# enricobottazzi/zk-fhe

Hardware: AMD Instinct MI355X
Metric: BFV proofs/sec (k=13) (higher is better)
Workload: dtype u32x8 (256-bit Montgomery integers over BN254 Fr/Fq)

## Files before the change

### zk-fhe_amd/csrc/core.hip

```cpp
#include <atomic>
#include <cstdio>
#include <cstdlib>
#include <cstring>

#include <map>
#include <mutex>
#include <utility>

#include "ctx.hpp"
#include "fq29.hip.hpp"
#include "fr29.hip.hpp"
#include "fr9.hip.hpp"

using namespace zk;

static thread_local std::string g_create_err;

int zk_fail(zkfhe_ctx *ctx, int code, const char *what, hipError_t e, const char *file, int line) {
  char buf[512];
  snprintf(buf, sizeof(buf), "%s failed: %s (%s:%d)", what, hipGetErrorString(e), file, line);
  if (ctx) ctx->err = buf; else g_create_err = buf;
  return code;
}
int zk_fail_msg(zkfhe_ctx *ctx, int code, const std::string &msg) {
  if (ctx) ctx->err = msg; else g_create_err = msg;
  return code;
}

int zk_func_max_lds(zkfhe_ctx *ctx, const void *kernel, int bytes) {
  static std::mutex mu;
  static std::map<std::pair<int, const void *>, int> done;
  std::lock_guard<std::mutex> l(mu);
  int &have = done[std::make_pair(ctx->device, kernel)];
  if (have >= bytes) return ZKFHE_OK;
  ZK_HIP(ctx, hipFuncSetAttribute(kernel, hipFuncAttributeMaxDynamicSharedMemorySize, bytes));
  have = bytes;
  return ZKFHE_OK;
}

int zk_scratch(zkfhe_ctx *ctx, int slot, size_t bytes, void **out) {
  if (ctx->scratch_sz[slot] < bytes) {
    if (ctx->scratch[slot]) {
      ZK_HIP(ctx, hipStreamSynchronize(ctx->stream));
      ZK_HIP(ctx, hipFree(ctx->scratch[slot]));
      ctx->scratch[slot] = nullptr;
      ctx->scratch_sz[slot] = 0;
    }
    size_t want = bytes + bytes / 4;
    ZK_HIP(ctx, hipMalloc(&ctx->scratch[slot], want));
    ctx->scratch_sz[slot] = want;
  }
  *out = ctx->scratch[slot];
  return ZKFHE_OK;
}

Fr zk_fr_from_u64(uint64_t v) {
  Fr t = Fr::zero();
  t.l[0] = (u32)v;
  t.l[1] = (u32)(v >> 32);
  return fp_to_mont<FrP>(t);
}

Fr zk_fr_root_of_unity(int log_n) {
  Fr c;
  const u32 w[8] = {0x60c37c9cu, 0xd34f1ed9u, 0xd39329c8u, 0x3215cf6du, 0x3dd31f74u, 0x98865ea9u, 0x166d18b7u, 0x03ddb9f5u};
  for (int i = 0; i < 8; ++i) c.l[i] = w[i];
  Fr r = fp_to_mont<FrP>(c);
  for (int i = 0; i < 28 - log_n; ++i) r = fp_sqr<FrP>(r);
  return r;
}

__global__ void __launch_bounds__(256) k_copy16(const uint4 *__restrict__ src, uint4 *__restrict__ dst, size_t n16) {
  for (size_t i = blockIdx.x * (size_t)blockDim.x + threadIdx.x; i < n16; i += (size_t)gridDim.x * blockDim.x) dst[i] = src[i];
}
int zk_copy_d2d(zkfhe_ctx *ctx, void *dst, const void *src, size_t bytes) {
  if (!bytes) return ZKFHE_OK;
  if (bytes >= ((size_t)1 << 20) && (bytes & 15) == 0 && ((uintptr_t)dst & 15) == 0 && ((uintptr_t)src & 15) == 0) {
    const size_t n16 = bytes / 16;
    size_t blocks = (n16 + 255) / 256;
    const size_t cap = (size_t)ctx->num_cu * 32;
    k_copy16<<<(unsigned)(blocks > cap ? cap : blocks), 256, 0, ctx->stream>>>((const uint4 *)src, (uint4 *)dst, n16);
    ZK_LAUNCH_CHECK(ctx);
    return ZKFHE_OK;
  }
  ZK_HIP(ctx, zk_memcpy_async(ctx, dst, src, bytes, hipMemcpyDeviceToDevice, ctx->stream));
  return ZKFHE_OK;
}

extern "C" {

const char *zkfhe_version(void) { return "zkfhe-mi355x 0.1 (gfx950)"; }

int zkfhe_ctx_create(int device_id, void *hip_stream, zkfhe_ctx **out) {
  setenv("GPU_MAX_HW_QUEUES", "2", 0);
  if (!getenv("ZKFHE_SPIN_WAIT")) {
    (void)hipSetDevice(device_id);
    (void)hipSetDeviceFlags(hipDeviceScheduleBlockingSync);
    (void)hipGetLastError();
  }
  if (!out) return zk_fail_msg(nullptr, ZKFHE_EINVAL, "out is NULL");
  *out = nullptr;
  int count = 0;
  hipError_t e = hipGetDeviceCount(&count);
  if (e != hipSuccess || count == 0)
    return zk_fail_msg(nullptr, ZKFHE_ENODEV, std::string("no HIP device: ") + hipGetErrorString(e));
  if (device_id < 0 || device_id >= count) return zk_fail_msg(nullptr, ZKFHE_EINVAL, "device_id out of range");
  hipDeviceProp_t prop;
  ZK_HIP(nullptr, hipGetDeviceProperties(&prop, device_id));
  if (strncmp(prop.gcnArchName, "gfx950", 6) != 0)
    return zk_fail_msg(nullptr, ZKFHE_ENODEV, std::string("device is ") + prop.gcnArchName + ", this library is built for gfx950 only");
  ZK_HIP(nullptr, hipSetDevice(device_id));
  zkfhe_ctx *ctx = new zkfhe_ctx();
  static std::atomic<uint64_t> next_uid{1};
  ctx->uid = next_uid.fetch_add(1);
  ctx->device = device_id;
  ctx->num_cu = prop.multiProcessorCount;
  if (hip_stream) {
    ctx->stream = (hipStream_t)hip_stream;
  } else {
    e = hipStreamCreateWithFlags(&ctx->stream, hipStreamNonBlocking);
    if (e != hipSuccess) { delete ctx; return zk_fail(nullptr, ZKFHE_EHIP, "hipStreamCreate", e, __FILE__, __LINE__); }
    ctx->own_stream = true;
  }
  if (hipHostMalloc(&ctx->bounce, zkfhe_ctx::BOUNCE_BYTES, hipHostMallocDefault) != hipSuccess) ctx->bounce = nullptr;
  if (hipEventCreateWithFlags(&ctx->wait_ev, hipEventBlockingSync | hipEventDisableTiming) != hipSuccess) ctx->wait_ev = nullptr;
  hipEventCreate(&ctx->ev0);
  hipEventCreate(&ctx->ev1);
  hipEventCreate(&ctx->pe0);
  hipEventCreate(&ctx->pe1);
  *out = ctx;
  return ZKFHE_OK;
}

int zkfhe_ctx_destroy(zkfhe_ctx *ctx) {
  ZK_ENTER(ctx);
  if (!ctx) return ZKFHE_OK;
  hipSetDevice(ctx->device);
  hipStreamSynchronize(ctx->stream);
  if (ctx->bounce) (void)hipHostFree(ctx->bounce);
  for (auto &kv : ctx->domains) {
    hipFree(kv.second.fwd);
    hipFree(kv.second.inv);
    hipFree(kv.second.fwd29);
    hipFree(kv.second.inv29);
    hipFree(kv.second.n_inv29_dev);
  }
  for (auto &kv : ctx->tw13) hipFree(kv.second);
  for (auto &kv : ctx->pre13) hipFree(kv.second);
  for (auto &kv : ctx->dif8) hipFree(kv.second);
  for (int i = 0; i < 4; ++i)
    if (ctx->scratch[i]) hipFree(ctx->scratch[i]);
  if (ctx->tickets) hipFree(ctx->tickets);
  if (ctx->bfv_tw) hipFree(ctx->bfv_tw);
  if (ctx->bfv_work) hipFree(ctx->bfv_work);
  for (auto &kv : ctx->slot_tw) hipFree(kv.second.dev);
  if (ctx->wait_ev) hipEventDestroy(ctx->wait_ev);
  hipEventDestroy(ctx->ev0);
  hipEventDestroy(ctx->ev1);
  if (ctx->own_stream) hipStreamDestroy(ctx->stream);
  delete ctx;
  return ZKFHE_OK;
}

const char *zkfhe_last_error(const zkfhe_ctx *ctx) { return ctx ? ctx->err.c_str() : g_create_err.c_str(); }

int zkfhe_sync(zkfhe_ctx *ctx) {
  ZK_ENTER(ctx);
  ZK_HIP(ctx, zk_wait(ctx));
  return ZKFHE_OK;
}

void *zkfhe_stream(zkfhe_ctx *ctx) { return (void *)ctx->stream; }

int zkfhe_device_info(zkfhe_ctx *ctx, char *arch_name, size_t arch_len, int *num_cu, size_t *hbm_bytes) {
  ZK_ENTER(ctx);
  hipDeviceProp_t prop;
  ZK_HIP(ctx, hipGetDeviceProperties(&prop, ctx->device));
  if (arch_name && arch_len) { strncpy(arch_name, prop.gcnArchName, arch_len - 1); arch_name[arch_len - 1] = 0; }
  if (num_cu) *num_cu = prop.multiProcessorCount;
  if (hbm_bytes) *hbm_bytes = prop.totalGlobalMem;
  return ZKFHE_OK;
}

int zkfhe_dev_alloc(zkfhe_ctx *ctx, size_t bytes, void **dptr) {
  ZK_ENTER(ctx);
  ZK_ARG(ctx, dptr != nullptr);
  ZK_HIP(ctx, hipSetDevice(ctx->device));
  hipError_t e = hipMalloc(dptr, bytes ? bytes : 1);
  if (e == hipErrorOutOfMemory) return zk_fail_msg(ctx, ZKFHE_ENOMEM, "hipMalloc: out of device memory");
  ZK_HIP(ctx, e);
  return ZKFHE_OK;
}
int zkfhe_dev_free(zkfhe_ctx *ctx, void *dptr) {
  ZK_ENTER(ctx);
  if (!dptr) return ZKFHE_OK;
  if (!ctx) {
    (void)hipFree(dptr);
    return ZKFHE_OK;
  }
  ZK_HIP(ctx, hipStreamSynchronize(ctx->stream));
  ZK_HIP(ctx, hipFree(dptr));
  return ZKFHE_OK;
}
int zkfhe_upload(zkfhe_ctx *ctx, void *dst_dev, const void *src_host, size_t bytes) {
  ZK_ENTER(ctx);
  if (!bytes) return ZKFHE_OK;
  if (ctx->bounce && bytes <= zkfhe_ctx::BOUNCE_BYTES) {
    memcpy(ctx->bounce, src_host, bytes);
    ZK_HIP(ctx, zk_memcpy_async(ctx, dst_dev, ctx->bounce, bytes, hipMemcpyHostToDevice, ctx->stream));
  } else {
    ZK_HIP(ctx, zk_memcpy_async(ctx, dst_dev, src_host, bytes, hipMemcpyHostToDevice, ctx->stream));
  }
  ZK_HIP(ctx, zk_wait(ctx));
  return ZKFHE_OK;
}
int zkfhe_download(zkfhe_ctx *ctx, void *dst_host, const void *src_dev, size_t bytes) {
  ZK_ENTER(ctx);
  if (!bytes) return ZKFHE_OK;
  if (ctx->bounce && bytes <= zkfhe_ctx::BOUNCE_BYTES) {
    ZK_HIP(ctx, zk_memcpy_async(ctx, ctx->bounce, src_dev, bytes, hipMemcpyDeviceToHost, ctx->stream));
    ZK_HIP(ctx, zk_wait(ctx));
    memcpy(dst_host, ctx->bounce, bytes);
    return ZKFHE_OK;
  }
  ZK_HIP(ctx, zk_memcpy_async(ctx, dst_host, src_dev, bytes, hipMemcpyDeviceToHost, ctx->stream));
  ZK_HIP(ctx, zk_wait(ctx));
  return ZKFHE_OK;
}
int zkfhe_copy_dev(zkfhe_ctx *ctx, void *dst_dev, const void *src_dev, size_t bytes) {
  ZK_ENTER(ctx);
  return zk_copy_d2d(ctx, dst_dev, src_dev, bytes);
}
int zkfhe_memset_dev(zkfhe_ctx *ctx, void *dst_dev, int byte, size_t bytes) {
  ZK_ENTER(ctx);
  ZK_HIP(ctx, zk_memset_async(ctx, dst_dev, byte, bytes, ctx->stream));
  return ZKFHE_OK;
}

int zkfhe_prof_enable(zkfhe_ctx *ctx, int on) {
  ZK_ENTER(ctx);
  ctx->prof_on = on != 0;
  return ZKFHE_OK;
}
int zkfhe_prof_reset(zkfhe_ctx *ctx) {
  ZK_ENTER(ctx);
  for (int i = 0; i < zkfhe_ctx::PROF_SLOTS; ++i) {
    ctx->prof_ms[i] = ctx->prof_bytes[i] = ctx->prof_ops[i] = 0;
    ctx->prof_launches[i] = 0;
  }
  return ZKFHE_OK;
}
int zkfhe_prof_read(zkfhe_ctx *ctx, int which, double *total_ms, uint64_t *launches, double *algorithmic_bytes) {
  ZK_ENTER(ctx);
  ZK_ARG(ctx, which >= 0 && which < zkfhe_ctx::PROF_SLOTS);
  if (total_ms) *total_ms = ctx->prof_ms[which];
  if (launches) *launches = ctx->prof_launches[which];
  if (algorithmic_bytes) *algorithmic_bytes = ctx->prof_bytes[which];
  return ZKFHE_OK;
}

int zkfhe_prof_read_ops(zkfhe_ctx *ctx, int which, double *ops) {
  ZK_ENTER(ctx);
  ZK_ARG(ctx, which >= 0 && which < zkfhe_ctx::PROF_SLOTS && ops != nullptr);
  *ops = ctx->prof_ops[which];
  return ZKFHE_OK;
}

int zkfhe_ctx_last_proof_marks(zkfhe_ctx *ctx, float marks_ms[3]) {
  ZK_ENTER(ctx);
  ZK_ARG(ctx, marks_ms != nullptr);
  for (int i = 0; i < 3; ++i) marks_ms[i] = ctx->proof_marks[i];
  return ZKFHE_OK;
}

int zkfhe_ctx_last_proof_commands(zkfhe_ctx *ctx, uint64_t counts[3]) {
  ZK_ENTER(ctx);
  ZK_ARG(ctx, counts != nullptr);
  for (int i = 0; i < 3; ++i) counts[i] = ctx->cmd_count[i];
  return ZKFHE_OK;
}

int zkfhe_timer_start(zkfhe_ctx *ctx) {
  ZK_ENTER(ctx);
  ZK_HIP(ctx, hipEventRecord(ctx->ev0, ctx->stream));
  return ZKFHE_OK;
}
int zkfhe_timer_stop_ms(zkfhe_ctx *ctx, float *ms) {
  ZK_ENTER(ctx);
  ZK_HIP(ctx, hipEventRecord(ctx->ev1, ctx->stream));
  ZK_HIP(ctx, hipEventSynchronize(ctx->ev1));
  ZK_HIP(ctx, hipEventElapsedTime(ms, ctx->ev0, ctx->ev1));
  return ZKFHE_OK;
}

}

enum { OP_ADD = 0, OP_SUB = 1, OP_MUL = 2 };

template <int OP>
__global__ void __launch_bounds__(256) k_fr_binop(const Fr *__restrict__ a, const Fr *__restrict__ b, Fr *__restrict__ out, size_t n) {
  for (size_t i = blockIdx.x * (size_t)blockDim.x + threadIdx.x; i < n; i += (size_t)gridDim.x * blockDim.x) {
    Fr x = a[i], y = b[i];
    Fr r = OP == OP_ADD ? x + y : OP == OP_SUB ? x - y : x * y;
    out[i] = r;
  }
}

template <int MODE>
__global__ void __launch_bounds__(256) k_fr_unop(const Fr *__restrict__ a, Fr s, Fr *__restrict__ out, size_t n) {
  for (size_t i = blockIdx.x * (size_t)blockDim.x + threadIdx.x; i < n; i += (size_t)gridDim.x * blockDim.x) {
    Fr x = a[i];
    out[i] = MODE == 0 ? x * s : MODE == 1 ? fr29_to_mont(x) : fp_from_mont<FrP>(x);
  }
}

__global__ void __launch_bounds__(256) k_fr_sqr_chain(const Fr *__restrict__ a, Fr *__restrict__ out, size_t n, int iters) {
  size_t i = blockIdx.x * (size_t)blockDim.x + threadIdx.x;
  if (i >= n) return;
  Fr x = a[i];
  for (int k = 0; k < iters; ++k) x = fp_sqr<FrP>(x);
  out[i] = x;
}

__global__ void __launch_bounds__(256) k_fq29_sqr_chain(const Fq *__restrict__ a, Fq *__restrict__ out, size_t n, int iters) {
  size_t i = blockIdx.x * (size_t)blockDim.x + threadIdx.x;
  if (i >= n) return;
  F29 x = f29_unpack(a[i]);
  for (int k = 0; k < iters; ++k) x = f29_sqr(x);
  out[i] = f29_pack(f29_canonical(x));
}

enum { FR9_MUL = 0, FR9_SQR = 1, FR9_MUL2 = 2, FR9_PERM = 3, FR9_LOOKUP = 4, FR9_CHAIN = 5, FR9_OPS = 6 };
__global__ void __launch_bounds__(256) k_fr9_op(int op, const Fr *__restrict__ in, Fr *__restrict__ out, size_t n) {
  for (size_t i = blockIdx.x * (size_t)blockDim.x + threadIdx.x; i < n; i += (size_t)gridDim.x * blockDim.x) {
    const Fr a = in[i], b = in[n + i], c = in[2 * n + i], d = in[3 * n + i], e = in[4 * n + i];
    Fr r;
    switch (op) {
      case FR9_MUL: r = fr9_store(fr9_mul(fr9_load(a), fr9_load32(b))); break;
      case FR9_SQR: r = fr9_store(fr9_cc(fr9_sqr(fr9_load(a)))); break;
      case FR9_MUL2: r = fr9_store(fr9_mul2(fr9_load(a), fr9_load32(b), fr9_load32(c), fr9_load(d))); break;
      case FR9_PERM: r = fr9_store(fr9_perm_step(fr9_load(a), fr9_perm_factor(fr9_load32(b), fr9_mul(fr9_load(d), fr9_cc(fr9_load32(c))), fr9_load32(e)))); break;
      case FR9_CHAIN: r = fr9_store(fr9_mul(fr9_load(c), fr9_times32(fr9_mul(fr9_load(a), fr9_load32(b))))); break;
      default: r = fr9_store(fr9_lookup_term(fr9_load(a), fr9_load(b), fr9_lookup_sum(fr9_load32(c), fr9_load32(d)))); break;
    }
    out[i] = r;
  }
}

#define BI_CHUNK 8
#define BI_LONG ((size_t)1 << 20)
template <bool NUM>
__global__ void __launch_bounds__(256) k_fr_batch_invert(Fr *__restrict__ a, Fr *__restrict__ num, Fr *__restrict__ tmp, size_t n, size_t T) {
  size_t t = blockIdx.x * (size_t)blockDim.x + threadIdx.x;
  if (t >= T) return;
  Lz<0, 1, 2> acc = lz_widen<0, 1, 2>(fr9_one());
  int cnt = 0;
  for (size_t i = t; i < n; i += T, ++cnt) {
    tmp[i] = fr9_store(acc);
    Fr x = a[i];
    if (!x.is_zero()) acc = fr9_mul(acc, fr9_load32(x));
  }
  acc = lz_widen<0, 1, 2>(fr9_load(fp_inv<FrP>(fr9_store(acc))));
  for (int k = cnt - 1; k >= 0; --k) {
    size_t i = t + (size_t)k * T;
    Fr x = a[i];
    if (x.is_zero()) {
      if (NUM) num[i] = Fr::zero();
      continue;
    }
    const Lz<0, 1, 2> inv = fr9_mul(acc, fr9_load32(tmp[i]));
    acc = fr9_mul(acc, fr9_load32(x));
    if (NUM) num[i] = fr9_store(fr9_mul(inv, fr9_load32(num[i])));
    else a[i] = fr9_store(inv);
  }
}

static unsigned ew_grid(zkfhe_ctx *ctx, size_t n) {
  size_t b = (n + 255) / 256;
  size_t cap = (size_t)ctx->num_cu * 8;
  return (unsigned)(b < 1 ? 1 : (b > cap ? cap : b));
}

extern "C" {

int zkfhe_fr_add(zkfhe_ctx *ctx, const zkfhe_fr *a, const zkfhe_fr *b, zkfhe_fr *out, size_t n) {
  ZK_ENTER(ctx);
  if (!n) return ZKFHE_OK;
  k_fr_binop<OP_ADD><<<ew_grid(ctx, n), 256, 0, ctx->stream>>>((const Fr *)a, (const Fr *)b, (Fr *)out, n);
  ZK_LAUNCH_CHECK(ctx);
  return ZKFHE_OK;
}
int zkfhe_fr_sub(zkfhe_ctx *ctx, const zkfhe_fr *a, const zkfhe_fr *b, zkfhe_fr *out, size_t n) {
  ZK_ENTER(ctx);
  if (!n) return ZKFHE_OK;
  k_fr_binop<OP_SUB><<<ew_grid(ctx, n), 256, 0, ctx->stream>>>((const Fr *)a, (const Fr *)b, (Fr *)out, n);
  ZK_LAUNCH_CHECK(ctx);
  return ZKFHE_OK;
}
int zkfhe_fr_mul(zkfhe_ctx *ctx, const zkfhe_fr *a, const zkfhe_fr *b, zkfhe_fr *out, size_t n) {
  ZK_ENTER(ctx);
  if (!n) return ZKFHE_OK;
  k_fr_binop<OP_MUL><<<ew_grid(ctx, n), 256, 0, ctx->stream>>>((const Fr *)a, (const Fr *)b, (Fr *)out, n);
  ZK_LAUNCH_CHECK(ctx);
  return ZKFHE_OK;
}
int zkfhe_fr_scale(zkfhe_ctx *ctx, const zkfhe_fr *a, const zkfhe_fr *s_host, zkfhe_fr *out, size_t n) {
  ZK_ENTER(ctx);
  if (!n) return ZKFHE_OK;
  ZK_ARG(ctx, s_host != nullptr);
  Fr s;
  memcpy(&s, s_host, 32);
  k_fr_unop<0><<<ew_grid(ctx, n), 256, 0, ctx->stream>>>((const Fr *)a, s, (Fr *)out, n);
  ZK_LAUNCH_CHECK(ctx);
  return ZKFHE_OK;
}
int zkfhe_fr_to_mont(zkfhe_ctx *ctx, const zkfhe_fr *a, zkfhe_fr *out, size_t n) {
  ZK_ENTER(ctx);
  if (!n) return ZKFHE_OK;
  k_fr_unop<1><<<ew_grid(ctx, n), 256, 0, ctx->stream>>>((const Fr *)a, Fr::zero(), (Fr *)out, n);
  ZK_LAUNCH_CHECK(ctx);
  return ZKFHE_OK;
}
int zkfhe_fr_from_mont(zkfhe_ctx *ctx, const zkfhe_fr *a, zkfhe_fr *out, size_t n) {
  ZK_ENTER(ctx);
  if (!n) return ZKFHE_OK;
  k_fr_unop<2><<<ew_grid(ctx, n), 256, 0, ctx->stream>>>((const Fr *)a, Fr::zero(), (Fr *)out, n);
  ZK_LAUNCH_CHECK(ctx);
  return ZKFHE_OK;
}
static int batch_invert(zkfhe_ctx *ctx, Fr *a, Fr *num, size_t n) {
  if (!n) return ZKFHE_OK;
  void *tmp;
  int rc = zk_scratch(ctx, 0, n * sizeof(Fr), &tmp);
  if (rc) return rc;
  static const int forced = getenv("ZKFHE_BI_CHUNK") ? atoi(getenv("ZKFHE_BI_CHUNK")) : 0;
  size_t chunk = forced > 0 ? (size_t)forced : n / ((size_t)ctx->num_cu * 1024);
  if (forced <= 0) chunk = chunk < BI_CHUNK ? BI_CHUNK : (chunk > 32 ? 32 : chunk);
  if (forced <= 0 && n >= BI_LONG && chunk < 16) chunk = 16;
  size_t T = (n + chunk - 1) / chunk;
  if (num)
    k_fr_batch_invert<true><<<zk_blocks(T, 256), 256, 0, ctx->stream>>>(a, num, (Fr *)tmp, n, T);
  else
    k_fr_batch_invert<false><<<zk_blocks(T, 256), 256, 0, ctx->stream>>>(a, nullptr, (Fr *)tmp, n, T);
  ZK_LAUNCH_CHECK(ctx);
  return ZKFHE_OK;
}
int zkfhe_fr_batch_invert(zkfhe_ctx *ctx, zkfhe_fr *a, size_t n) {
  ZK_ENTER(ctx);
  return batch_invert(ctx, (Fr *)a, nullptr, n);
}
int zkfhe_fr_batch_invert_mul(zkfhe_ctx *ctx, const zkfhe_fr *den, zkfhe_fr *num, size_t n) {
  ZK_ENTER(ctx);
  ZK_ARG(ctx, n == 0 || (den != nullptr && num != nullptr && (const void *)den != (const void *)num));
  return batch_invert(ctx, (Fr *)den, (Fr *)num, n);
}
int zkfhe_fr9_op(zkfhe_ctx *ctx, int op, const zkfhe_fr *in, zkfhe_fr *out, size_t n) {
  ZK_ENTER(ctx);
  ZK_ARG(ctx, op >= 0 && op < FR9_OPS);
  if (!n) return ZKFHE_OK;
  ZK_ARG(ctx, in != nullptr && out != nullptr);
  k_fr9_op<<<ew_grid(ctx, n), 256, 0, ctx->stream>>>(op, (const Fr *)in, (Fr *)out, n);
  ZK_LAUNCH_CHECK(ctx);
  return ZKFHE_OK;
}
int zkfhe_fr_sqr_chain(zkfhe_ctx *ctx, const zkfhe_fr *a, zkfhe_fr *out, size_t n, int iters) {
  ZK_ENTER(ctx);
  if (!n) return ZKFHE_OK;
  k_fr_sqr_chain<<<zk_blocks(n, 256), 256, 0, ctx->stream>>>((const Fr *)a, (Fr *)out, n, iters);
  ZK_LAUNCH_CHECK(ctx);
  return ZKFHE_OK;
}

int zkfhe_fq29_sqr_chain(zkfhe_ctx *ctx, const zkfhe_fq *a, zkfhe_fq *out, size_t n, int iters) {
  ZK_ENTER(ctx);
  if (!n) return ZKFHE_OK;
  k_fq29_sqr_chain<<<zk_blocks(n, 256), 256, 0, ctx->stream>>>((const Fq *)a, (Fq *)out, n, iters);
  ZK_LAUNCH_CHECK(ctx);
  return ZKFHE_OK;
}

}
```

### zk-fhe_amd/csrc/ctx.hpp

```cpp
#pragma once
#include <hip/hip_runtime.h>

#include <array>
#include <map>
#include <string>
#include <vector>

#include "../../include/zkfhe.h"
#include "bn254.hip.hpp"

struct NttDomain {
  int log_n = 0;
  zk::Fr *fwd = nullptr;
  zk::Fr *inv = nullptr;
  zk::Fr n_inv;
  zk::Fr omega, omega_inv;
  zk::Fr *fwd29 = nullptr, *inv29 = nullptr;
  zk::Fr n_inv29;
  zk::Fr *n_inv29_dev = nullptr;
};

struct zkfhe_ctx {
  uint64_t uid = 0;
  int device = 0;
  hipStream_t stream = nullptr;
  bool own_stream = false;
  hipEvent_t ev0 = nullptr, ev1 = nullptr;
  std::string err;
  int num_cu = 0;
  std::map<int, NttDomain> domains;
  std::map<const void *, void *> tw13;
  std::map<std::array<uint64_t, 6>, void *> pre13;
  std::map<std::array<uint64_t, 8>, void *> dif8;
  bool prof_on = false;
  hipEvent_t pe0 = nullptr, pe1 = nullptr;
  hipEvent_t wait_ev = nullptr;
  static constexpr int PROF_SLOTS = 26;
  double prof_ms[PROF_SLOTS] = {}, prof_bytes[PROF_SLOTS] = {}, prof_ops[PROF_SLOTS] = {};
  uint64_t prof_launches[PROF_SLOTS] = {};
  void *bounce = nullptr;
  static constexpr size_t BOUNCE_BYTES = (size_t)1 << 20;
  void *scratch[4] = {nullptr, nullptr, nullptr, nullptr};
  size_t scratch_sz[4] = {0, 0, 0, 0};
  float proof_marks[3] = {0, 0, 0};
  uint64_t cmd_count[3] = {0, 0, 0};
  zkfhe_ctx *cmd_owner = nullptr;
  unsigned *tickets = nullptr;
  uint32_t *bfv_tw = nullptr;
  void *bfv_work = nullptr;
  size_t bfv_work_sz = 0;
  struct SlotTables {
    uint32_t *dev = nullptr;
    uint32_t pinv = 0, n_inv = 0;
  };
  std::map<std::pair<uint64_t, uint64_t>, SlotTables> slot_tw;
};

struct zkfhe_basis {
  size_t n = 0;
  int c = 0;
  int windows = 0;
  zk::G1Affine *table = nullptr;
  zk::G1Affine *mult = nullptr;
  int mc = 0, mw = 0;
  size_t mult_bytes = 0;
  bool narrowed = false;
};

int zk_fail(zkfhe_ctx *ctx, int code, const char *what, hipError_t e, const char *file, int line);
int zk_fail_msg(zkfhe_ctx *ctx, int code, const std::string &msg);

#define ZK_HIP(ctx, expr)                                                             \
  do {                                                                                \
    hipError_t _e = (expr);                                                           \
    if (_e != hipSuccess) return zk_fail((ctx), ZKFHE_EHIP, #expr, _e, __FILE__, __LINE__); \
  } while (0)

enum { ZK_CMD_KERNEL = 0, ZK_CMD_COPY = 1, ZK_CMD_FILL = 2 };
static inline void zk_count(zkfhe_ctx *ctx, int which) { ++(ctx->cmd_owner ? ctx->cmd_owner : ctx)->cmd_count[which]; }

#define ZK_LAUNCH_CHECK(ctx)         \
  do {                               \
    zk_count((ctx), ZK_CMD_KERNEL);  \
    ZK_HIP(ctx, hipGetLastError());  \
  } while (0)

static inline hipError_t zk_memcpy_async(zkfhe_ctx *ctx, void *dst, const void *src, size_t bytes, hipMemcpyKind kind, hipStream_t stream) {
  zk_count(ctx, ZK_CMD_COPY);
  return hipMemcpyAsync(dst, src, bytes, kind, stream);
}
static inline hipError_t zk_memset_async(zkfhe_ctx *ctx, void *dst, int value, size_t bytes, hipStream_t stream) {
  zk_count(ctx, ZK_CMD_FILL);
  return hipMemsetAsync(dst, value, bytes, stream);
}

#define ZK_ENTER(ctx)                                   \
  do {                                                  \
    if (ctx) (void)hipSetDevice((ctx)->device);         \
  } while (0)

#define ZK_ARG(ctx, cond)                                                        \
  do {                                                                           \
    if (!(cond)) return zk_fail_msg((ctx), ZKFHE_EINVAL, std::string("bad argument: ") + #cond); \
  } while (0)

inline void zk_prof_begin(zkfhe_ctx *ctx) {
  if (ctx->prof_on) (void)hipEventRecord(ctx->pe0, ctx->stream);
}
inline void zk_prof_end(zkfhe_ctx *ctx, int which, double bytes) {
  if (!ctx->prof_on) return;
  (void)hipEventRecord(ctx->pe1, ctx->stream);
  (void)hipEventSynchronize(ctx->pe1);
  float ms = 0;
  (void)hipEventElapsedTime(&ms, ctx->pe0, ctx->pe1);
  ctx->prof_ms[which] += ms;
  ctx->prof_bytes[which] += bytes;
  ctx->prof_launches[which] += 1;
}

inline hipError_t zk_wait(zkfhe_ctx *ctx) {
  static const bool spin = getenv("ZKFHE_SPIN_WAIT") != nullptr;
  if (spin || !ctx->wait_ev) return hipStreamSynchronize(ctx->stream);
  hipError_t e = hipEventRecord(ctx->wait_ev, ctx->stream);
  if (e != hipSuccess) return e;
  return hipEventSynchronize(ctx->wait_ev);
}

int zk_dif8_pass(zkfhe_ctx *ctx, const zk::Fr *src, zk::Fr *dst, size_t n_cols, int log_n, int S, int inverse, const zk::Fr *shifts_host, unsigned rows);
int zk_msm_batch_strided(zkfhe_ctx *ctx, const zkfhe_basis *basis, const zkfhe_fr *scalars_dev, size_t col_stride, size_t n_cols, zkfhe_g1_affine *out_dev);
int zk_msm_batch_strided_form(zkfhe_ctx *ctx, const zkfhe_basis *basis, const zkfhe_fr *scalars_dev, size_t col_stride, size_t n_cols, void *out_dev, bool xyzz);
#define ZK_CK(x)             \
  do {                       \
    const int rc__ = (x);    \
    if (rc__) return rc__;   \
  } while (0)

int zk_func_max_lds(zkfhe_ctx *ctx, const void *kernel, int bytes);
int zk_scratch(zkfhe_ctx *ctx, int slot, size_t bytes, void **out);
int zk_basis_create_scaled(zkfhe_ctx *ctx, const zkfhe_g1_affine *bases_host, size_t n, int window_bits, double table_budget_scale, zkfhe_basis **out);
int zk_copy_d2d(zkfhe_ctx *ctx, void *dst, const void *src, size_t bytes);
int zk_domain(zkfhe_ctx *ctx, int log_n, const NttDomain **out);
int zk_pre13(zkfhe_ctx *ctx, const zk::Fr &g, int lef, int rows, bool scaled, const void **out);
int zk_coset_ntt_rows(zkfhe_ctx *ctx, const zk::Fr *in_dev, zk::Fr *out_dev, size_t n_cols, int log_n, int lef, const zk::Fr &g, int rows);
int zk_extend_lagrange(zkfhe_ctx *ctx, const zk::Fr *lagr_dev, zk::Fr *tmp_dev, zk::Fr *out_dev, size_t n_cols, int log_n, int lef, const zk::Fr &g, int rows);

zk::Fr zk_fr_from_u64(uint64_t v);
zk::Fr zk_fr_root_of_unity(int log_n);

static inline unsigned zk_blocks(size_t n, unsigned threads) { return (unsigned)((n + threads - 1) / threads); }
```

### zk-fhe_amd/host/keygen.hip

```cpp
#include "prover_internal.hpp"

std::vector<BigInt> GpuPolyMul::mul_u64(const std::vector<uint64_t> &a, const std::vector<uint64_t> &b) {
  const U256 *host = mul_u64_raw(a, b);
  std::vector<BigInt> out(2 * a.size() - 1);
  for (size_t i = 0; i < out.size(); ++i) out[i] = fe::to_bigint(host[i]);
  return out;
}

const U256 *GpuPolyMul::mul_u64_raw(const std::vector<uint64_t> &a, const std::vector<uint64_t> &b) {
  const size_t n = a.size();
  if (ws->polyio.bytes < 2 * n * 8 + 2 * n * 32) throw std::runtime_error("polynomial too long for the prover workspace");
  uint64_t *da = (uint64_t *)ws->polyio.p, *db = da + n;
  Fr *dout = (Fr *)(db + n);
  const U256 *host = ws->host_poly;
  int rc = up(ctx, ws, da, a.data(), n * 8);
  if (!rc) rc = up(ctx, ws, db, b.data(), n * 8);
  if (!rc) rc = zkfhe_witness_poly_mul_u64(ctx, da, db, n, (zkfhe_fr *)dout);
  if (!rc) rc = zkfhe_fr_from_mont(ctx, (const zkfhe_fr *)dout, (zkfhe_fr *)dout, 2 * n - 1);
  if (!rc && ws->host_poly && 2 * n - 1 <= ws->host_poly_len) {
    if (zk_memcpy_async(ctx, ws->host_poly, dout, (2 * n - 1) * 32, hipMemcpyDeviceToHost, ctx->stream) != hipSuccess) rc = ZKFHE_EHIP;
    if (!rc) rc = zkfhe_sync(ctx);
  } else if (!rc) {
    pageable.resize(2 * n - 1);
    host = pageable.data();
    rc = zkfhe_download(ctx, pageable.data(), dout, (2 * n - 1) * 32);
  }
  if (rc) throw std::runtime_error(std::string("GPU poly mul failed: ") + zkfhe_last_error(ctx));
  return host;
}

int up(zkfhe_ctx *ctx, Workspace *ws, void *dst, const void *src, size_t bytes) {
  if (!bytes) return ZKFHE_OK;
  const size_t need = (bytes + 63) & ~(size_t)63;
  if (!ws->ring || ws->ring_off + need > Workspace::RING_BYTES) return zkfhe_upload(ctx, dst, src, bytes);
  uint8_t *slot = ws->ring + ws->ring_off;
  ws->ring_off += need;
  memcpy(slot, src, bytes);
  ZK_HIP(ctx, zk_memcpy_async(ctx, dst, slot, bytes, hipMemcpyHostToDevice, ctx->stream));
  return ZKFHE_OK;
}

int alloc_workspace(zkfhe_ctx *ctx, const CircuitConfig &c, Workspace *ws, int ext_rows) {
  const size_t n = c.n(), ne = (size_t)ext_rows * n, col = n * 32, ecol = ne * 32;
  const size_t n_all = (size_t)c.n_advice() + 3 * c.n_lookup + c.n_chunks() + 1;
  ws->n_all = n_all;
  CK(ws->all_l.alloc(ctx, n_all * col));
  CK(ws->all_ext.alloc(ctx, n_all * ecol));
  {
    size_t o = 0;
    auto take = [&](View &l, View &e, size_t cols) {
      l.p = (char *)ws->all_l.p + o * col;
      e.p = (char *)ws->all_ext.p + o * ecol;
      o += cols;
    };
    take(ws->adv_l, ws->adv_ext, c.n_advice());
    take(ws->la_l, ws->la_ext, c.n_lookup);
    take(ws->ls_l, ws->ls_ext, c.n_lookup);
    take(ws->pz_l, ws->pz_ext, c.n_chunks());
    take(ws->lz_l, ws->lz_ext, c.n_lookup);
    take(ws->inst_l, ws->inst_ext, 1);
  }
  ZK_HIP(ctx, zk_memset_async(ctx, ws->inst_l.p, 0, col, ctx->stream));
  ws->inst_count = 0;
  CK(ws->tmp_c.alloc(ctx, std::max<size_t>(n_all, c.n_perm()) * col));
  {
    const size_t groups = ((size_t)c.n_gate() + 7) / 8 + 1 + 2 + ((size_t)c.n_chunks() + 31) / 32 + ((size_t)c.n_chunks() + 3) / 4 + ((size_t)c.n_lookup + 2) / 3 + 8;
    CK(ws->partials.alloc(ctx, std::max<size_t>(groups * (size_t)ext_rows, 96) * col));
  }
  CK(ws->h_ext.alloc(ctx, 4 * col));
  CK(ws->h_c.alloc(ctx, 4 * col));
  CK(ws->misc.alloc(ctx, 32 * col));
  CK(ws->points.alloc(ctx, std::max<size_t>(n_all, c.n_perm()) * 64 + 64));
  CK(ws->num.alloc(ctx, std::max<size_t>(c.n_chunks(), c.n_lookup) * col));
  CK(ws->den.alloc(ctx, std::max<size_t>(c.n_chunks(), c.n_lookup) * col));
  if ((size_t)c.n_perm() > 4096 || (size_t)c.n_chunks() + c.n_lookup > 4096)
    return zk_fail_msg(ctx, ZKFHE_EINVAL, "configuration too wide for the prover workspace (more than 4096 permutation columns)");
  CK(ws->small.alloc(ctx, 1 << 20));
  const size_t max_items = (size_t)c.n_advice() + c.n_fixed() + 2 + c.n_perm() + c.n_chunks() + 3 * c.n_lookup;
  CK(ws->jobs.alloc(ctx, max_items * sizeof(zkp::EvalJob) + max_items * (sizeof(void *) + 32) + 256));
  CK(ws->evout.alloc(ctx, (max_items + 64) * 4 * 32));
  CK(ws->polyio.alloc(ctx, 4 * c.n() * 32));
  ZK_HIP(ctx, hipHostMalloc((void **)&ws->host_adv, (size_t)c.n_advice() * col, hipHostMallocDefault));
  memset(ws->host_adv, 0, (size_t)c.n_advice() * col);
  ZK_HIP(ctx, hipHostMalloc((void **)&ws->host_blind, std::max<size_t>(2 * c.n_lookup, 2) * col, hipHostMallocDefault));
  return ZKFHE_OK;
}

void free_workspace(Workspace *ws) {
  (void)hipSetDevice(ws->all_l.device);
  for (DevBuf *b : ws->all()) b->release();
  for (void *h : {(void *)ws->host_adv, (void *)ws->host_blind, (void *)ws->host_pool, (void *)ws->host_poly, (void *)ws->host_pts, (void *)ws->ring, (void *)ws->host_rand_pt,
                  (void *)ws->host_early, (void *)ws->host_early_err, (void *)ws->host_out})
    if (h) (void)hipHostFree(h);
  if (ws->ev_pts) (void)hipEventDestroy(ws->ev_pts);
  if (ws->ev_rand) (void)hipEventDestroy(ws->ev_rand);
  if (ws->ev_early) (void)hipEventDestroy(ws->ev_early);
  if (ws->aux) (void)zkfhe_ctx_destroy(ws->aux);
  delete ws;
}

int get_workspace(zkfhe_ctx *ctx, zkfhe_bfv_pk *pk, Workspace **out) {
  std::lock_guard<std::mutex> lock(pk->mu);
  auto it = pk->workspaces.find(ctx->uid);
  if (it == pk->workspaces.end()) {
    Workspace *ws = new Workspace();
    int rc = alloc_workspace(ctx, pk->cfg, ws, pk->ext_rows);
    if (rc) {
      for (DevBuf *b : ws->all()) b->release();
      delete ws;
      return rc;
    }
    it = pk->workspaces.emplace(ctx->uid, ws).first;
  }
  if (it->second->all_l.device != ctx->device) return zk_fail_msg(ctx, ZKFHE_EINVAL, "prover workspace belongs to another device");
  *out = it->second;
  return ZKFHE_OK;
}

int extend_cols(zkfhe_ctx *ctx, zkfhe_bfv_pk *pk, Workspace *ws, const Fr *lagr, size_t count, Fr *ext) {
  if (!count) return ZKFHE_OK;
  const int rows = pk->ext_rows;
  const size_t n = pk->cfg.n();
  const Fr g = mont_u64(COSET_G);
  (void)n;
  return zk_extend_lagrange(ctx, lagr, ws->tmp_c.fr(), ext, count, (int)pk->cfg.k, 2, g, rows);
}

static int build_resident_tables(zkfhe_ctx *ctx, zkfhe_bfv_pk *pk, Workspace *ws) {
  const CircuitConfig &cfg = pk->cfg;
  const size_t n = cfg.n(), cells = (size_t)cfg.n_perm() * n;
  const NttDomain *dom;
  CK(zk_domain(ctx, (int)cfg.k, &dom));
  const size_t R = (size_t)pk->ext_rows;
  CK(pk->fixed_ext.alloc(ctx, (size_t)cfg.n_fixed() * R * n * 32));
  CK(pk->sigma_ext.alloc(ctx, cells * R * 32));
  CK(pk->l_ext.alloc(ctx, 3 * R * n * 32));
  CK(pk->xs_ext.alloc(ctx, R * n * 32));
  CK(extend_cols(ctx, pk, ws, pk->fixed_l.fr(), cfg.n_fixed(), pk->fixed_ext.fr()));
  CK(extend_cols(ctx, pk, ws, pk->sigma_l.fr(), cfg.n_perm(), pk->sigma_ext.fr()));
  {
    std::vector<U256> l(3 * n, fe::zero());
    const size_t u = cfg.u();
    l[0] = fe::one();
    l[n + u] = fe::one();
    for (size_t i = 0; i < u; ++i) l[2 * n + i] = fe::one();
    CK(upload_canon(ctx, ws->misc.fr(), l.data(), 3 * n));
    CK(extend_cols(ctx, pk, ws, ws->misc.fr(), 3, pk->l_ext.fr()));
  }
  {
    const Fr wext = zk_fr_root_of_unity((int)cfg.k + 2);
    Fr shift = mont_u64(COSET_G);
    for (int k1 = 0; k1 < pk->ext_rows; ++k1) {
      zkp::k_powers<<<(unsigned)((n + 255) / 256), 256, 0, ctx->stream>>>(shift, dom->omega, pk->xs_ext.fr() + (size_t)k1 * n, n);
      ZK_LAUNCH_CHECK(ctx);
      shift = shift * wext;
    }
    if (pk->ext_rows == 3) {
      CK(pk->ext3_pw.alloc(ctx, 3 * n * 32));
      Fr gk = mont_u64(COSET_G);
      for (int t = 0; t < 3; ++t) {
        zkp::k_powers<<<(unsigned)((n + 255) / 256), 256, 0, ctx->stream>>>(Fr::one(), fr_inv(gk), pk->ext3_pw.fr() + (size_t)t * n, n);
        ZK_LAUNCH_CHECK(ctx);
        gk = gk * wext;
      }
    }
  }
  return ZKFHE_OK;
}

static U256 vk_digest_of(const zkfhe_bfv_pk *pk) { return vk_digest(pk->cfg, pk->fixed_commit, pk->sigma_commit); }

static int keygen_impl(zkfhe_ctx *ctx, const zkfhe_srs *srs, const char *input_json, const BfvParams &prm, CircuitConfig cfg, bool replay,
                zkfhe_bfv_pk **out) {
  const size_t n = cfg.n();
  ZK_ARG(ctx, srs->k == cfg.k);
  const CircuitInput in = CircuitInput::parse_json(input_json);
  Context ctx0(CTX_PHASE0, false, true), ctx_gate(CTX_GATE1, false, true), ctx_rlc(CTX_RLC1, true, true);
  std::vector<Cell> make_public;
  BfvState st = bfv_phase0(ctx0, in, prm, make_public);
  bfv_phase1(st, prm, ctx_gate, ctx_rlc, fe::zero());
  Assigner as(cfg, true);
  as.place(ctx0, replay);
  as.place(ctx_gate, replay);
  as.place(ctx_rlc, replay);
  as.place_lookups(ctx_gate);
  as.finish_structure(ctx0, ctx_gate, ctx_rlc, make_public);
  cfg.bp_gate0 = as.t.bp_gate0;
  cfg.bp_gate1 = as.t.bp_gate1;
  cfg.bp_rlc = as.t.bp_rlc;
  zkfhe_bfv_pk *pk = new zkfhe_bfv_pk();
  pk->cfg = cfg;
  pk->prm = prm;
  pk->ext_rows = getenv("ZKFHE_CHECK_QUOTIENT") ? 4 : 3;
  {
    pk->gate1_cells = ctx_gate.advice.size();
    pk->n_lookup_cells = ctx_gate.lookup.size();
    pk->n_inv_slots = ctx_gate.inv_slots.size();
    std::vector<uint32_t> lsrc(ctx_gate.lookup.size());
    for (size_t i = 0; i < lsrc.size(); ++i) {
      ZK_ASSERT(ctx_gate.lookup[i].ctx == CTX_GATE1, "lookup cell outside the phase-1 gate context");
      lsrc[i] = ctx_gate.lookup[i].off;
    }
    std::vector<uint32_t> start(cfg.n_gate1, 0), len(cfg.n_gate1, 0);
    size_t s = 0;
    for (unsigned c = 0; c < cfg.n_gate1 && s < pk->gate1_cells; ++c) {
      start[c] = (uint32_t)s;
      if (c < cfg.bp_gate1.size()) {
        len[c] = cfg.bp_gate1[c] + 1;
        s += cfg.bp_gate1[c];
      } else {
        len[c] = (uint32_t)(pk->gate1_cells - s);
        s = pk->gate1_cells;
      }
    }
    CK(pk->lookup_src.alloc(ctx, (lsrc.size() + 1) * 4));
    CK(pk->inv_slots.alloc(ctx, (ctx_gate.inv_slots.size() + 1) * 4));
    CK(pk->place_start.alloc(ctx, (start.size() + 1) * 4));
    CK(pk->place_len.alloc(ctx, (len.size() + 1) * 4));
    if (!lsrc.empty()) CK(zkfhe_upload(ctx, pk->lookup_src.p, lsrc.data(), lsrc.size() * 4));
    if (!ctx_gate.inv_slots.empty()) CK(zkfhe_upload(ctx, pk->inv_slots.p, ctx_gate.inv_slots.data(), ctx_gate.inv_slots.size() * 4));
    CK(zkfhe_upload(ctx, pk->place_start.p, start.data(), start.size() * 4));
    CK(zkfhe_upload(ctx, pk->place_len.p, len.data(), len.size() * 4));
  }
  const size_t cells = (size_t)cfg.n_perm() * n;
  std::vector<uint32_t> parent(cells);
  for (size_t i = 0; i < cells; ++i) parent[i] = (uint32_t)i;
  auto find = [&](uint32_t x) {
    uint32_t root = x;
    while (parent[root] != root) root = parent[root];
    while (parent[x] != root) {
      uint32_t nx = parent[x];
      parent[x] = root;
      x = nx;
    }
    return root;
  };
  for (const auto &cp : as.t.copies) {
    uint32_t ra = find((uint32_t)cp.first), rb = find((uint32_t)cp.second);
    if (ra != rb) {
      if (ra < rb) parent[rb] = ra;
      else parent[ra] = rb;
    }
  }
  std::vector<uint32_t> target(cells), last_of(cells, 0xffffffffu), first_of(cells);
  for (size_t i = 0; i < cells; ++i) target[i] = (uint32_t)i;
  for (size_t i = 0; i < cells; ++i) {
    const uint32_t r = find((uint32_t)i);
    if (last_of[r] == 0xffffffffu) first_of[r] = (uint32_t)i;
    else target[last_of[r]] = (uint32_t)i;
    last_of[r] = (uint32_t)i;
  }
  for (size_t i = 0; i < cells; ++i)
    if (parent[i] == i && last_of[i] != 0xffffffffu) target[last_of[i]] = first_of[i];
  const NttDomain *dom;
  CK(zk_domain(ctx, (int)cfg.k, &dom));
  CK(pk->fixed_l.alloc(ctx, (size_t)cfg.n_fixed() * n * 32));
  CK(pk->sigma_l.alloc(ctx, cells * 32));
  CK(pk->dpow.alloc(ctx, (size_t)cfg.n_perm() * 32));
  for (unsigned c = 0; c < cfg.n_fixed(); ++c) {
    ZK_HIP(ctx, zk_memcpy_async(ctx, pk->fixed_l.fr() + (size_t)c * n, as.t.fixed[c].data(), n * 32, hipMemcpyHostToDevice, ctx->stream));
  }
  CK(zkfhe_fr_to_mont(ctx, (const zkfhe_fr *)pk->fixed_l.p, (zkfhe_fr *)pk->fixed_l.p, (size_t)cfg.n_fixed() * n));
  U256 dcan;
  memcpy(dcan.l, DELTA_CANON, 32);
  zkp::k_powers<<<1, 256, 0, ctx->stream>>>(Fr::one(), mont(dcan), pk->dpow.fr(), cfg.n_perm());
  ZK_LAUNCH_CHECK(ctx);
  DevBuf tgt;
  CK(tgt.alloc(ctx, cells * 4));
  CK(zkfhe_upload(ctx, tgt.p, target.data(), cells * 4));
  zkp::k_sigma_values<<<(unsigned)((cells + 255) / 256), 256, 0, ctx->stream>>>((const uint32_t *)tgt.p, pk->dpow.fr(), dom->fwd, pk->sigma_l.fr(),
                                                                                 cells, (int)cfg.k);
  ZK_LAUNCH_CHECK(ctx);
  Workspace *ws;
  CK(get_workspace(ctx, pk, &ws));
  CK(commit_cols(ctx, srs, srs->g_lagrange, pk->fixed_l.fr(), cfg.n_fixed(), (G1Affine *)ws->points.p, pk->fixed_commit));
  CK(commit_cols(ctx, srs, srs->g_lagrange, pk->sigma_l.fr(), cfg.n_perm(), (G1Affine *)ws->points.p, pk->sigma_commit));
  CK(build_resident_tables(ctx, pk, ws));
  CK(zkfhe_sync(ctx));
  tgt.release();
  pk->vk_digest = vk_digest_of(pk);
  *out = pk;
  return ZKFHE_OK;
}


extern "C" {

int zkfhe_bfv_keygen(zkfhe_ctx *ctx, const zkfhe_srs *srs, const char *input_json, const zkfhe_bfv_params *params,
                     const zkfhe_bfv_config *config, zkfhe_bfv_pk **out) {
  ZK_ENTER(ctx);
  ZK_ARG(ctx, srs && input_json && params && config && out);
  try {
    return keygen_impl(ctx, srs, input_json, params_from_c(params), config_from_c(config), config->replay != 0, out);
  } catch (const std::exception &e) {
    return zk_fail_msg(ctx, ZKFHE_EINVAL, e.what());
  }
}

int zkfhe_bfv_pk_destroy(zkfhe_ctx *ctx, zkfhe_bfv_pk *pk) {
  ZK_ENTER(ctx);
  if (!pk) return ZKFHE_OK;
  zkfhe_sync(ctx);
  DevBuf *bufs[] = {&pk->fixed_l, &pk->sigma_l, &pk->fixed_ext, &pk->sigma_ext, &pk->l_ext, &pk->xs_ext, &pk->dpow, &pk->ext3_pw,
                    &pk->lookup_src, &pk->inv_slots, &pk->place_start, &pk->place_len};
  for (DevBuf *b : bufs) b->release();
  for (auto &kv : pk->workspaces) free_workspace(kv.second);
  delete pk;
  return ZKFHE_OK;
}

int zkfhe_bfv_pk_release_ctx(zkfhe_ctx *ctx, zkfhe_bfv_pk *pk) {
  ZK_ENTER(ctx);
  ZK_ARG(ctx, pk != nullptr);
  zkfhe_sync(ctx);
  std::lock_guard<std::mutex> lock(pk->mu);
  auto it = pk->workspaces.find(ctx->uid);
  if (it != pk->workspaces.end()) {
    free_workspace(it->second);
    pk->workspaces.erase(it);
  }
  return ZKFHE_OK;
}

namespace {
struct FileW {
  FILE *f;
  bool ok = true;
  void raw(const void *p, size_t n) { ok = ok && fwrite(p, 1, n, f) == n; }
  void u32(uint32_t v) { raw(&v, 4); }
  void u64(uint64_t v) { raw(&v, 8); }
  void vec32(const std::vector<uint32_t> &v) {
    u64(v.size());
    if (!v.empty()) raw(v.data(), v.size() * 4);
  }
};
struct FileR {
  FILE *f;
  bool ok = true;
  void raw(void *p, size_t n) { ok = ok && fread(p, 1, n, f) == n; }
  uint32_t u32() {
    uint32_t v = 0;
    raw(&v, 4);
    return v;
  }
  uint64_t u64() {
    uint64_t v = 0;
    raw(&v, 8);
    return v;
  }
  std::vector<uint32_t> vec32(size_t limit) {
    const uint64_t n = u64();
    std::vector<uint32_t> v;
    if (!ok || n > limit) {
      ok = false;
      return v;
    }
    v.resize(n);
    if (n) raw(v.data(), n * 4);
    return v;
  }
};
int download_u32(zkfhe_ctx *ctx, const DevBuf &b, size_t count, std::vector<uint32_t> &out) {
  out.resize(count);
  if (count) CK(zkfhe_download(ctx, out.data(), b.p, count * 4));
  return ZKFHE_OK;
}
int upload_u32(zkfhe_ctx *ctx, DevBuf &b, const std::vector<uint32_t> &v) {
  CK(b.alloc(ctx, (v.size() + 1) * 4));
  if (!v.empty()) CK(zkfhe_upload(ctx, b.p, v.data(), v.size() * 4));
  return ZKFHE_OK;
}
}

int zkfhe_bfv_pk_save(zkfhe_ctx *ctx, const zkfhe_bfv_pk *pk, const char *path) {
  ZK_ENTER(ctx);
  ZK_ARG(ctx, pk != nullptr && path != nullptr);
  const CircuitConfig &cfg = pk->cfg;
  const size_t n = cfg.n();
  std::vector<uint32_t> lookup_src, inv_slots, place_start, place_len;
  CK(download_u32(ctx, pk->lookup_src, pk->n_lookup_cells, lookup_src));
  CK(download_u32(ctx, pk->inv_slots, pk->n_inv_slots, inv_slots));
  CK(download_u32(ctx, pk->place_start, cfg.n_gate1, place_start));
  CK(download_u32(ctx, pk->place_len, cfg.n_gate1, place_len));
  std::vector<uint8_t> cols((size_t)(cfg.n_fixed() + cfg.n_perm()) * n * 32);
  CK(zkfhe_download(ctx, cols.data(), pk->fixed_l.p, (size_t)cfg.n_fixed() * n * 32));
  CK(zkfhe_download(ctx, cols.data() + (size_t)cfg.n_fixed() * n * 32, pk->sigma_l.p, (size_t)cfg.n_perm() * n * 32));
  FILE *f = fopen(path, "wb");
  if (!f) return zk_fail_msg(ctx, ZKFHE_EINVAL, std::string("cannot write ") + path);
  FileW w{f};
  w.raw("ZKFHEPK2", 8);
  const uint32_t hdr[8] = {cfg.k, cfg.n_gate0, cfg.n_gate1, cfg.n_lookup, cfg.n_rlc, cfg.unusable_rows, cfg.lookup_bits, cfg.transcript};
  w.raw(hdr, sizeof(hdr));
  w.vec32(cfg.bp_gate0), w.vec32(cfg.bp_gate1), w.vec32(cfg.bp_rlc);
  w.u64(pk->prm.N), w.u64(pk->prm.Q), w.u64(pk->prm.T), w.u64(pk->prm.B);
  w.u64(pk->gate1_cells);
  w.vec32(lookup_src), w.vec32(inv_slots), w.vec32(place_start), w.vec32(place_len);
  w.u64(pk->fixed_commit.size()), w.u64(pk->sigma_commit.size());
  for (const auto &pt : pk->fixed_commit) w.raw(&pt, sizeof(AffinePoint));
  for (const auto &pt : pk->sigma_commit) w.raw(&pt, sizeof(AffinePoint));
  w.raw(pk->vk_digest.l, 32);
  w.u64(cols.size());
  w.raw(cols.data(), cols.size());
  const bool ok = w.ok && fclose(f) == 0;
  if (!ok) return zk_fail_msg(ctx, ZKFHE_EINVAL, std::string("short write to ") + path);
  return ZKFHE_OK;
}

int zkfhe_bfv_pk_load(zkfhe_ctx *ctx, const zkfhe_srs *srs, const char *path, zkfhe_bfv_pk **out) {
  ZK_ENTER(ctx);
  ZK_ARG(ctx, srs != nullptr && path != nullptr && out != nullptr);
  FILE *f = fopen(path, "rb");
  if (!f) return zk_fail_msg(ctx, ZKFHE_EINVAL, std::string("cannot read ") + path);
  FileR r{f};
  char magic[8];
  r.raw(magic, 8);
  if (!r.ok || memcmp(magic, "ZKFHEPK2", 8) != 0) {
    fclose(f);
    return zk_fail_msg(ctx, ZKFHE_EINVAL, std::string(path) + " is not a ZKFHEPK2 proving key");
  }
  zkfhe_bfv_pk *pk = new zkfhe_bfv_pk();
  pk->ext_rows = getenv("ZKFHE_CHECK_QUOTIENT") ? 4 : 3;
  auto fail = [&](const std::string &why) {
    fclose(f);
    zkfhe_bfv_pk_destroy(ctx, pk);
    return zk_fail_msg(ctx, ZKFHE_EINVAL, std::string(path) + ": " + why);
  };
  try {
    uint32_t hdr[8];
    r.raw(hdr, sizeof(hdr));
    CircuitConfig &cfg = pk->cfg;
    cfg.k = hdr[0], cfg.n_gate0 = hdr[1], cfg.n_gate1 = hdr[2], cfg.n_lookup = hdr[3], cfg.n_rlc = hdr[4], cfg.unusable_rows = hdr[5], cfg.lookup_bits = hdr[6];
    cfg.transcript = hdr[7];
    if (!r.ok || cfg.transcript > TR_BLAKE2B || cfg.k < 3 || cfg.k > 20 || cfg.n_gate0 + cfg.n_gate1 > 4096 || cfg.n_lookup > 4096 || cfg.n_rlc > 4096) return fail("bad header");
    if (cfg.n_gate() == 0 || cfg.unusable_rows < 4 || cfg.unusable_rows >= cfg.n()) return fail("bad header (unusable_rows)");
    if (cfg.lookup_bits == 0 || cfg.lookup_bits > 20 || ((size_t)1 << cfg.lookup_bits) > cfg.max_rows()) return fail("bad header (lookup_bits)");
    if (cfg.k != srs->k) return fail("proving key and SRS have different k");
    cfg.bp_gate0 = r.vec32(1 << 16), cfg.bp_gate1 = r.vec32(1 << 16), cfg.bp_rlc = r.vec32(1 << 16);
    pk->prm.N = r.u64(), pk->prm.Q = r.u64(), pk->prm.T = r.u64(), pk->prm.B = r.u64();
    pk->gate1_cells = r.u64();
    if (!r.ok || pk->prm.N < 2 || (pk->prm.N & (pk->prm.N - 1)) || 5 * (uint64_t)pk->prm.N + 1 > cfg.u() || pk->prm.Q < 2 ||
        pk->prm.Q >= ((uint64_t)1 << 63) || pk->prm.T < 1 || pk->prm.T >= pk->prm.Q || pk->prm.B >= pk->prm.Q)
      return fail("BFV parameters do not fit the recorded layout");
    const size_t n = cfg.n(), max_cells = (size_t)cfg.n_gate1 * n;
    const std::vector<uint32_t> lookup_src = r.vec32(max_cells), inv_slots = r.vec32(max_cells), place_start = r.vec32(cfg.n_gate1), place_len = r.vec32(cfg.n_gate1);
    if (!r.ok || pk->gate1_cells > max_cells || place_start.size() != cfg.n_gate1 || place_len.size() != cfg.n_gate1) return fail("bad structure lists");
    for (uint32_t o : lookup_src)
      if (o >= pk->gate1_cells) return fail("lookup offset outside the gate stream");
    for (uint32_t o : inv_slots)
      if (o >= pk->gate1_cells) return fail("inverse slot outside the gate stream");
    for (unsigned c = 0; c < cfg.n_gate1; ++c)
      if ((size_t)place_start[c] + place_len[c] > pk->gate1_cells || place_len[c] > n) return fail("column range outside the gate stream");
    pk->n_lookup_cells = lookup_src.size();
    pk->n_inv_slots = inv_slots.size();
    const uint64_t nf = r.u64(), ns = r.u64();
    if (!r.ok || nf != cfg.n_fixed() || ns != cfg.n_perm()) return fail("commitment counts do not match the configuration");
    pk->fixed_commit.resize(nf), pk->sigma_commit.resize(ns);
    for (auto &pt : pk->fixed_commit) r.raw(&pt, sizeof(AffinePoint));
    for (auto &pt : pk->sigma_commit) r.raw(&pt, sizeof(AffinePoint));
    r.raw(pk->vk_digest.l, 32);
    const uint64_t col_bytes = r.u64();
    if (!r.ok || col_bytes != (uint64_t)(cfg.n_fixed() + cfg.n_perm()) * n * 32) return fail("column block has the wrong size");
    if (!(vk_digest_of(pk) == pk->vk_digest)) return fail("verifying-key digest does not match the stored commitments");
    std::vector<uint8_t> cols(col_bytes);
    r.raw(cols.data(), cols.size());
    if (!r.ok) return fail("truncated file");
    fclose(f);
    f = nullptr;
    int rc;
    if ((rc = upload_u32(ctx, pk->lookup_src, lookup_src)) || (rc = upload_u32(ctx, pk->inv_slots, inv_slots)) ||
        (rc = upload_u32(ctx, pk->place_start, place_start)) || (rc = upload_u32(ctx, pk->place_len, place_len)) ||
        (rc = pk->fixed_l.alloc(ctx, (size_t)cfg.n_fixed() * n * 32)) || (rc = pk->sigma_l.alloc(ctx, (size_t)cfg.n_perm() * n * 32)) ||
        (rc = pk->dpow.alloc(ctx, (size_t)cfg.n_perm() * 32)) ||
        (rc = zkfhe_upload(ctx, pk->fixed_l.p, cols.data(), (size_t)cfg.n_fixed() * n * 32)) ||
        (rc = zkfhe_upload(ctx, pk->sigma_l.p, cols.data() + (size_t)cfg.n_fixed() * n * 32, (size_t)cfg.n_perm() * n * 32))) {
      zkfhe_bfv_pk_destroy(ctx, pk);
      return rc;
    }
    U256 dcan;
    memcpy(dcan.l, DELTA_CANON, 32);
    zkp::k_powers<<<1, 256, 0, ctx->stream>>>(Fr::one(), mont(dcan), pk->dpow.fr(), cfg.n_perm());
    Workspace *ws;
    if ((rc = get_workspace(ctx, pk, &ws)) || (rc = build_resident_tables(ctx, pk, ws)) || (rc = zkfhe_sync(ctx))) {
      zkfhe_bfv_pk_destroy(ctx, pk);
      return rc;
    }
    std::vector<AffinePoint> chk_f, chk_s;
    if ((rc = commit_cols(ctx, srs, srs->g_lagrange, pk->fixed_l.fr() + (size_t)cfg.fix_table() * n, 1, (G1Affine *)ws->points.p, chk_f)) ||
        (rc = commit_cols(ctx, srs, srs->g_lagrange, pk->sigma_l.fr(), 1, (G1Affine *)ws->points.p, chk_s))) {
      zkfhe_bfv_pk_destroy(ctx, pk);
      return rc;
    }
    if (!(chk_f[0].x == pk->fixed_commit[cfg.fix_table()].x) || !(chk_f[0].y == pk->fixed_commit[cfg.fix_table()].y) ||
        !(chk_s[0].x == pk->sigma_commit[0].x) || !(chk_s[0].y == pk->sigma_commit[0].y)) {
      zkfhe_bfv_pk_destroy(ctx, pk);
      return zk_fail_msg(ctx, ZKFHE_EINVAL, std::string(path) + ": proving key was generated with a different SRS");
    }
  } catch (const std::exception &e) {
    if (f) fclose(f);
    zkfhe_bfv_pk_destroy(ctx, pk);
    return zk_fail_msg(ctx, ZKFHE_EINVAL, e.what());
  }
  *out = pk;
  return ZKFHE_OK;
}

int zkfhe_bfv_pk_info(const zkfhe_bfv_pk *pk, uint8_t vk_digest[32], uint32_t *n_fixed, uint32_t *n_sigma) {
  if (!pk) return ZKFHE_EINVAL;
  if (vk_digest) memcpy(vk_digest, pk->vk_digest.l, 32);
  if (n_fixed) *n_fixed = (uint32_t)pk->fixed_commit.size();
  if (n_sigma) *n_sigma = (uint32_t)pk->sigma_commit.size();
  return ZKFHE_OK;
}

int zkfhe_bfv_pk_prefix_cache(const zkfhe_bfv_pk *pk_c, int capacity, uint64_t *hits, uint64_t *misses, uint64_t *entries) {
  if (!pk_c) return ZKFHE_EINVAL;
  zkfhe_bfv_pk *pk = const_cast<zkfhe_bfv_pk *>(pk_c);
  if (capacity >= 0) pk->prefix.set_capacity((size_t)capacity);
  pk->prefix.stats(hits, misses, entries);
  return ZKFHE_OK;
}

int zkfhe_bfv_pk_commitments(const zkfhe_bfv_pk *pk, uint8_t *fixed_out, uint8_t *sigma_out) {
  if (!pk) return ZKFHE_EINVAL;
  for (size_t i = 0; i < pk->fixed_commit.size() && fixed_out; ++i) {
    memcpy(fixed_out + 64 * i, pk->fixed_commit[i].x.l, 32);
    memcpy(fixed_out + 64 * i + 32, pk->fixed_commit[i].y.l, 32);
  }
  for (size_t i = 0; i < pk->sigma_commit.size() && sigma_out; ++i) {
    memcpy(sigma_out + 64 * i, pk->sigma_commit[i].x.l, 32);
    memcpy(sigma_out + 64 * i + 32, pk->sigma_commit[i].y.l, 32);
  }
  return ZKFHE_OK;
}

int zkfhe_bfv_pk_export_vk(const zkfhe_bfv_pk *pk, uint8_t *out, size_t cap, size_t *len) {
  if (!pk || !len) return ZKFHE_EINVAL;
  const size_t nf = pk->fixed_commit.size(), ns = pk->sigma_commit.size();
  const size_t need = 8 + 40 + 32 + 64 * (nf + ns);
  *len = need;
  if (!out || cap < need) return out ? ZKFHE_EINVAL : ZKFHE_OK;
  memcpy(out, "ZKFHEVK2", 8);
  const uint32_t hdr[10] = {pk->cfg.k, pk->cfg.n_gate0, pk->cfg.n_gate1, pk->cfg.n_lookup, pk->cfg.n_rlc, pk->cfg.unusable_rows,
                            pk->cfg.lookup_bits, pk->cfg.transcript, (uint32_t)nf, (uint32_t)ns};
  memcpy(out + 8, hdr, 40);
  memcpy(out + 48, pk->vk_digest.l, 32);
  uint8_t *p = out + 80;
  for (const auto &c : pk->fixed_commit) {
    memcpy(p, c.x.l, 32);
    memcpy(p + 32, c.y.l, 32);
    p += 64;
  }
  for (const auto &c : pk->sigma_commit) {
    memcpy(p, c.x.l, 32);
    memcpy(p + 32, c.y.l, 32);
    p += 64;
  }
  return ZKFHE_OK;
}

int zkfhe_bfv_pk_break_points(const zkfhe_bfv_pk *pk, int which, uint32_t *out, uint32_t *count) {
  if (!pk || !count) return ZKFHE_EINVAL;
  const auto &v = which == 0 ? pk->cfg.bp_gate0 : which == 1 ? pk->cfg.bp_gate1 : pk->cfg.bp_rlc;
  if (out && *count >= v.size()) memcpy(out, v.data(), v.size() * 4);
  *count = (uint32_t)v.size();
  return ZKFHE_OK;
}

}
```

### zk-fhe_amd/host/prove.hip

```cpp
#include "prover_internal.hpp"

int alloc_witness_buffers(zkfhe_ctx *ctx, const zkfhe_bfv_pk *pk, Workspace *ws) {
  if (ws->stream.p) return ZKFHE_OK;
  const size_t N = pk->prm.N;
  CK(ws->stream.alloc(ctx, (pk->gate1_cells + 8) * 32));
  CK(ws->pool.alloc(ctx, 40 * (2 * N + 8) * 32));
  CK(ws->invtmp.alloc(ctx, (pk->n_inv_slots + 8) * 32));
  ZK_HIP(ctx, hipHostMalloc((void **)&ws->host_pool, 24 * (2 * N + 8) * 32, hipHostMallocDefault));
  ws->host_poly_len = 2 * N + 8;
  ZK_HIP(ctx, hipHostMalloc((void **)&ws->host_poly, ws->host_poly_len * 32, hipHostMallocDefault));
  CK(ws->wblind.alloc(ctx, 256));
  ZK_HIP(ctx, hipHostMalloc((void **)&ws->ring, Workspace::RING_BYTES, hipHostMallocDefault));
  CK(ws->dev_ring.alloc(ctx, Workspace::RING_BYTES));
  {
    const CircuitConfig &c = pk->cfg;
    const size_t max_items = (size_t)c.n_advice() + c.n_fixed() + 2 + c.n_perm() + c.n_chunks() + 3 * c.n_lookup;
    ws->out_pts_cap = std::max<size_t>(ws->n_all, c.n_perm()) + 16;
    ws->out_ev_off = ws->out_pts_cap * PT_SLOT;
    ws->out_ev_cap = max_items * 4;
    ws->out_flag_off = ws->out_ev_off + ws->out_ev_cap * 32;
    ZK_HIP(ctx, hipHostMalloc((void **)&ws->host_out, ws->out_flag_off + 256, hipHostMallocDefault));
    memset(ws->host_out, 0, ws->out_flag_off + 256);
  }
  ZK_HIP(ctx, hipHostMalloc((void **)&ws->host_pts, ((size_t)pk->cfg.n_gate0 + 1) * PT_SLOT, hipHostMallocDefault));
  ZK_HIP(ctx, hipEventCreateWithFlags(&ws->ev_pts, hipEventDisableTiming | hipEventBlockingSync));
  ZK_HIP(ctx, hipEventCreateWithFlags(&ws->ev_rand, hipEventDisableTiming | hipEventBlockingSync));
  ZK_HIP(ctx, hipEventCreateWithFlags(&ws->ev_early, hipEventDisableTiming | hipEventBlockingSync));
  ZK_HIP(ctx, hipHostMalloc((void **)&ws->host_early, ((size_t)pk->cfg.n_advice() + 2 * pk->cfg.n_lookup + 16) * PT_SLOT, hipHostMallocDefault));
  ZK_HIP(ctx, hipHostMalloc((void **)&ws->host_early_err, 64, hipHostMallocDefault));
  ZK_HIP(ctx, hipHostMalloc((void **)&ws->host_rand_pt, PT_SLOT, hipHostMallocDefault));
  if (zkfhe_ctx_create(ctx->device, nullptr, &ws->aux)) return zk_fail_msg(ctx, ZKFHE_EHIP, std::string("auxiliary context: ") + zkfhe_last_error(nullptr));
  return ZKFHE_OK;
}

namespace {

void permute_lookup(const std::vector<U256> &input, size_t u, unsigned table_size, std::vector<U256> &a_perm, std::vector<U256> &s_perm) {
  std::vector<size_t> cnt(table_size, 0);
  for (size_t i = 0; i < u; ++i) {
    const U256 &v = input[i];
    if (v.l[1] | v.l[2] | v.l[3] || v.l[0] >= table_size) throw std::runtime_error("lookup input not in table");
    ++cnt[v.l[0]];
  }
  std::vector<size_t> left(table_size, 1);
  left[0] = u - (table_size - 1);
  a_perm.assign(u, fe::zero());
  s_perm.assign(u, fe::zero());
  std::vector<size_t> holes;
  size_t pos = 0;
  for (unsigned v = 0; v < table_size; ++v)
    for (size_t k = 0; k < cnt[v]; ++k, ++pos) {
      a_perm[pos] = fe::from_u64(v);
      if (k == 0) {
        if (!left[v]) throw std::runtime_error("lookup input not in table");
        --left[v];
        s_perm[pos] = fe::from_u64(v);
      } else {
        holes.push_back(pos);
      }
    }
  size_t hi = 0;
  for (unsigned v = 0; v < table_size; ++v)
    for (size_t k = 0; k < left[v]; ++k) s_perm[holes[hi++]] = fe::from_u64(v);
}

struct DevPoly {
  Fr *d = nullptr;
  size_t len = 0;
  uint64_t bits = 0;
};

class GpuPhase1 {
 public:
  GpuPhase1(zkfhe_ctx *c, const zkfhe_bfv_pk *k, Workspace *w) : ctx(c), pk(k), ws(w) {}

  int launch(const BfvState &st) {
    const uint64_t Q = pk->prm.Q, T = pk->prm.T, B = pk->prm.B;
    stream = ws->stream.fr();
    pool_used = 0;
    off = 0;
    calls.clear();
    call_level.clear();
    produced.clear();
    h_used = 0;
    {
      const PolyChip *ins[14] = {&st.e0, &st.e1, &st.u, &st.m, &st.pk0_u, &st.quotient_0, &st.remainder_0, &st.quotient_0_times_cyclo, &st.expected_c0,
                                 &st.pk1_u, &st.quotient_1, &st.remainder_1, &st.quotient_1_times_cyclo, &st.expected_c1};
      size_t cells = 1 + 16;
      for (const PolyChip *pc : ins) cells += pc->assigned_coefficients.size();
      in_host = ws->host_pool;
      in_dev = ws->pool.fr();
      in_ring = false;
      void *h = nullptr;
      if (cells * 32 <= ((size_t)1 << 20)) {
        void *d = stage_reserve(ws, cells * 32, &h);
        if (d) {
          in_host = (U256 *)h;
          in_dev = (Fr *)d;
          in_ring = true;
        }
      }
    }
    DevPoly e0 = stage(st.e0), e1 = stage(st.e1), u = stage(st.u), m = stage(st.m);
    DevPoly pk0_u = stage(st.pk0_u), q0 = stage(st.quotient_0), r0 = stage(st.remainder_0), q0c = stage(st.quotient_0_times_cyclo), xc0 = stage(st.expected_c0);
    DevPoly pk1_u = stage(st.pk1_u), q1 = stage(st.quotient_1), r1 = stage(st.remainder_1), q1c = stage(st.quotient_1_times_cyclo), xc1 = stage(st.expected_c1);
    in_host[h_used] = st.delta.value;
    const Fr *delta = in_dev + h_used;
    const uint64_t delta_bits = st.delta.value.bits();
    ++h_used;
    mg_slot = h_used;
    n_mg = 0;
    h_used += 16;
    pool_used = h_used;
    if (!in_ring) ZK_HIP(ctx, zk_memcpy_async(ctx, ws->pool.p, ws->host_pool, mg_slot * 32, hipMemcpyHostToDevice, ctx->stream));

    CK(in_range(e0, B, Q));
    CK(in_range(e1, B, Q));
    CK(gadget(zkw::G_CHI_KEY, u, nullptr, nullptr, zkw::cpc_chi_key(), Q - 1, 0, Fr::zero()));
    CK(in_range(m, T / 2, Q));
    const int n_side = 2;
    for (int side = 0; side < n_side; ++side) {
      const DevPoly &pku = side ? pk1_u : pk0_u, &q = side ? q1 : q0, &r = side ? r1 : r0, &qc = side ? q1c : q0c;
      CK(mul_gate());
      DevPoly pku_r;
      CK(reduce_by_modulo(pku, Q, pku_r));
      CK(in_field(q, Q));
      CK(in_field(r, Q));
      CK(mul_gate());
      DevPoly sum, sum_mod;
      CK(add(qc, r, sum));
      CK(reduce_by_modulo(sum, Q, sum_mod));
      if (sum_mod.len < pku_r.len) return zk_fail_msg(ctx, ZKFHE_EINVAL, "degree <= self.degree (src/poly_chip.rs:375)");
      DevPoly trimmed{sum_mod.d + (sum_mod.len - pku_r.len), pku_r.len, sum_mod.bits};
      CK(equal(trimmed, pku_r));
      const size_t N = pk->prm.N;
      if (r.len < N) return zk_fail_msg(ctx, ZKFHE_EINVAL, "degree <= self.degree (src/poly_chip.rs:375)");
      DevPoly acc{r.d + (r.len - N), N, r.bits};
      if (side == 0) {
        DevPoly m_delta, t;
        CK(scalar_mul(m, delta, delta_bits, m_delta));
        CK(add(acc, m_delta, t));
        CK(add(t, e0, acc));
      } else {
        DevPoly t;
        CK(add(acc, e1, t));
        acc = t;
      }
      DevPoly c_red;
      CK(reduce_by_modulo(acc, Q, c_red));
      CK(equal(c_red, side ? xc1 : xc0));
    }
    if (off != pk->gate1_cells) return zk_fail_msg(ctx, ZKFHE_EINVAL, "GPU witness stream length differs from the keygen circuit shape");
    CK(launch_levels());
    if (pk->n_inv_slots) {
      const unsigned g = (unsigned)((pk->n_inv_slots + 255) / 256);
      zkw::k_gather<<<g, 256, 0, ctx->stream>>>(stream, (const unsigned *)pk->inv_slots.p, pk->n_inv_slots, ws->invtmp.fr());
      ZK_LAUNCH_CHECK(ctx);
      CK(zkfhe_fr_batch_invert(ctx, (zkfhe_fr *)ws->invtmp.p, pk->n_inv_slots));
      zkw::k_scatter<<<g, 256, 0, ctx->stream>>>(stream, (const unsigned *)pk->inv_slots.p, pk->n_inv_slots, ws->invtmp.fr());
      ZK_LAUNCH_CHECK(ctx);
    }
    return ZKFHE_OK;
  }

  int place_early(const zkp::RngRows &blind, unsigned zero_cols) {
    zkw::ZeroRuns z{};
    z.count = n_mg;
    for (unsigned i = 0; i < n_mg; ++i) z.at[i] = stream + mg_off[i];
    zkw::k_zero_runs<<<1, 64, 0, ctx->stream>>>(z);
    ZK_LAUNCH_CHECK(ctx);
    return place(blind, zero_cols);
  }
  struct PatchPlan {
    std::vector<unsigned> columns;
    struct Cell {
      unsigned col_slot, row, value;
    };
    std::vector<Cell> cells;
  };
  PatchPlan patch_plan() const {
    PatchPlan p;
    const CircuitConfig &cfg = pk->cfg;
    std::vector<size_t> start(cfg.n_gate1, 0), len(cfg.n_gate1, 0);
    size_t s = 0;
    for (unsigned c = 0; c < cfg.n_gate1 && s < pk->gate1_cells; ++c) {
      start[c] = s;
      if (c < cfg.bp_gate1.size()) {
        len[c] = (size_t)cfg.bp_gate1[c] + 1;
        s += cfg.bp_gate1[c];
      } else {
        len[c] = pk->gate1_cells - s;
        s = pk->gate1_cells;
      }
    }
    for (unsigned i = 0; i < n_mg; ++i)
      for (unsigned j = 0; j < 4; ++j) {
        const size_t o = mg_off[i] + j;
        for (unsigned c = 0; c < cfg.n_gate1; ++c)
          if (len[c] && o >= start[c] && o < start[c] + len[c]) {
            size_t slot = std::find(p.columns.begin(), p.columns.end(), c) - p.columns.begin();
            if (slot == p.columns.size()) p.columns.push_back(c);
            p.cells.push_back({(unsigned)slot, (unsigned)(o - start[c]), 4 * i + j});
          }
      }
    return p;
  }
  int patch(const U256 evals[12], const PatchPlan &plan, Fr *patch_cols, std::vector<zkfhe_sparse_term> *terms = nullptr) {
    const CircuitConfig &cfg = pk->cfg;
    const size_t n = cfg.n();
    Fr mg[16];
    for (int i = 0; i < 4; ++i) {
      mg[4 * i] = Fr::zero();
      for (int j = 0; j < 3; ++j) mg[4 * i + 1 + j] = mont(evals[3 * i + j]);
    }
    if (terms) {
      terms->clear();
      for (const auto &c : plan.cells) {
        if ((c.value & 3) == 0) continue;
        zkfhe_sparse_term t;
        memcpy(&t.scalar, &mg[c.value], 32);
        t.row = c.row;
        t.slot = c.col_slot;
        terms->push_back(t);
      }
    }
    if (plan.cells.size() > 64) return zk_fail_msg(ctx, ZKFHE_EINVAL, "too many challenge-dependent gate cells");
    zkw::PatchList list{};
    for (size_t t = 0; t < plan.cells.size(); ++t) {
      const auto &c = plan.cells[t];
      list.cells[t].dst_adv = ws->adv_l.fr() + ((size_t)cfg.n_gate0 + plan.columns[c.col_slot]) * n + c.row;
      list.cells[t].dst_patch = terms ? nullptr : patch_cols + (size_t)c.col_slot * n + c.row;
      list.cells[t].value = c.value;
    }
    memcpy(list.values, mg, sizeof(mg));
    if (!terms) ZK_HIP(ctx, zk_memset_async(ctx, patch_cols, 0, plan.columns.size() * n * 32, ctx->stream));
    zkw::k_patch_cells<<<1, 64, 0, ctx->stream>>>(list, (unsigned)plan.cells.size());
    ZK_LAUNCH_CHECK(ctx);
    return ZKFHE_OK;
  }

  int finish(const U256 evals[12], const zkp::RngRows &blind) {
    Fr mg[16];
    for (int i = 0; i < 4; ++i) {
      mg[4 * i] = Fr::zero();
      for (int j = 0; j < 3; ++j) mg[4 * i + 1 + j] = mont(evals[3 * i + j]);
    }
    zkw::PatchList list{};
    unsigned nc = 0;
    for (unsigned i = 0; i < n_mg; ++i)
      for (unsigned j = 0; j < 4; ++j) {
        list.cells[nc].dst_adv = stream + mg_off[i] + j;
        list.cells[nc].dst_patch = nullptr;
        list.cells[nc].value = 4 * i + j;
        ++nc;
      }
    memcpy(list.values, mg, sizeof(mg));
    if (nc) {
      zkw::k_patch_cells<<<1, 64, 0, ctx->stream>>>(list, nc);
      ZK_LAUNCH_CHECK(ctx);
    }
    return place(blind, 0);
  }

 private:
  int place(const zkp::RngRows &blind, unsigned zero_cols) {
    const CircuitConfig &cfg = pk->cfg;
    const size_t n = cfg.n();
    const unsigned u = (unsigned)cfg.u();
    const unsigned g_place = grid_for(ctx, (size_t)cfg.n_gate1 * n);
    zkw::k_place<<<g_place + zkp::rng_tail_grid(blind, (size_t)cfg.n_gate1 * (n - u), 256), 256, 0, ctx->stream>>>(
        stream, (const unsigned *)pk->place_start.p, (const unsigned *)pk->place_len.p, cfg.n_gate1, n, ws->adv_l.fr() + (size_t)cfg.n_gate0 * n, blind, u, g_place);
    ZK_LAUNCH_CHECK(ctx);
    if (cfg.n_lookup) {
      if (pk->n_lookup_cells > (size_t)cfg.n_lookup * cfg.max_rows()) return zk_fail_msg(ctx, ZKFHE_EINVAL, "lookup cells do not fit the configured lookup columns");
      zkp::RngRows blind_lk = blind;
      blind_lk.ctr0 += (unsigned long long)(cfg.adv_lookup0() - cfg.n_gate0) * blind.ctr_col_stride;
      const unsigned g_lk = grid_for(ctx, (size_t)(cfg.n_lookup + zero_cols) * n);
      zkw::k_place_lookups<<<g_lk + zkp::rng_tail_grid(blind_lk, (size_t)cfg.n_lookup * (n - u), 256), 256, 0, ctx->stream>>>(
          stream, (const unsigned *)pk->lookup_src.p, pk->n_lookup_cells, (unsigned)cfg.max_rows(), n, cfg.n_lookup, ws->adv_l.fr() + (size_t)cfg.adv_lookup0() * n, blind_lk, u,
          zero_cols, g_lk);
      ZK_LAUNCH_CHECK(ctx);
    } else if (zero_cols) {
      ZK_HIP(ctx, zk_memset_async(ctx, ws->adv_l.fr() + (size_t)cfg.adv_rlc0() * n, 0, (size_t)zero_cols * n * 32, ctx->stream));
    }
    return ZKFHE_OK;
  }

  zkfhe_ctx *ctx;
  const zkfhe_bfv_pk *pk;
  Workspace *ws;
  Fr *stream = nullptr;
  size_t off = 0, pool_used = 0, h_used = 0, mg_slot = 0, mg_off[4] = {0, 0, 0, 0};
  unsigned n_mg = 0;
  U256 *in_host = nullptr;
  Fr *in_dev = nullptr;
  bool in_ring = false;

  DevPoly stage(const PolyChip &p) {
    DevPoly d;
    d.len = p.assigned_coefficients.size();
    d.bits = p.max_num_bits;
    d.d = in_dev + h_used;
    for (size_t i = 0; i < d.len; ++i) in_host[h_used + i] = p.assigned_coefficients[i].value;
    h_used += d.len;
    return d;
  }
  Fr *take(size_t len) {
    Fr *p = ws->pool.fr() + pool_used;
    pool_used += len;
    return p;
  }
  int gadget(int type, const DevPoly &a, const Fr *b, Fr *out, size_t cpc, uint64_t p0, uint64_t p1, const Fr &bound) {
    if (pool_used * 32 > ws->pool.bytes || (off + a.len * cpc) > pk->gate1_cells)
      return zk_fail_msg(ctx, ZKFHE_EINVAL, "GPU witness stream exceeds the keygen circuit shape");
    zkw::GadgetArgs g;
    g.type = type;
    g.a = a.d;
    g.b = b;
    g.out = out;
    g.stream = stream;
    g.base = off;
    g.cpc = cpc;
    g.count = a.len;
    g.p0 = p0;
    g.p1 = p1;
    g.bound = bound;
    calls.push_back(g);
    call_level.push_back(level_of(a.d, a.len, b));
    if (out) produced.push_back({out, out + a.len, call_level.back()});
    off += a.len * cpc;
    return ZKFHE_OK;
  }
  struct Produced {
    const Fr *lo, *hi;
    int level;
  };
  std::vector<zkw::GadgetArgs> calls;
  std::vector<int> call_level;
  std::vector<Produced> produced;
  int level_of(const Fr *a, size_t len, const Fr *b) const {
    int lv = 0;
    for (const Produced &p : produced) {
      if (a < p.hi && a + len > p.lo) lv = std::max(lv, p.level + 1);
      if (b && b < p.hi && b + 1 > p.lo) lv = std::max(lv, p.level + 1);
      if (b && b + len > p.lo && b < p.hi) lv = std::max(lv, p.level + 1);
    }
    return lv;
  }
  int launch_levels() {
    int max_level = 0;
    for (int l : call_level) max_level = std::max(max_level, l);
    std::vector<zkw::GadgetArgs> ordered;
    std::vector<size_t> first(max_level + 2, 0);
    for (int l = 0; l <= max_level; ++l) {
      first[l] = ordered.size();
      for (size_t i = 0; i < calls.size(); ++i)
        if (call_level[i] == l) ordered.push_back(calls[i]);
    }
    first[max_level + 1] = ordered.size();
    STAGE(dev, zkw::GadgetArgs, ws, ordered.data(), ordered.size() * sizeof(zkw::GadgetArgs));
    CK(flush_staged(ctx, ws));
    for (int l = 0; l <= max_level; ++l) {
      size_t longest = 0;
      for (size_t i = first[l]; i < first[l + 1]; ++i) longest = std::max(longest, ordered[i].count);
      if (first[l + 1] == first[l]) continue;
      zkw::k_gadget<<<dim3((unsigned)((longest + 255) / 256), (unsigned)(first[l + 1] - first[l])), 256, 0, ctx->stream>>>(dev + first[l]);
      ZK_LAUNCH_CHECK(ctx);
    }
    return ZKFHE_OK;
  }
  int in_range(const DevPoly &a, uint64_t z, uint64_t y) {
    if (!(z < y)) return zk_fail_msg(ctx, ZKFHE_EINVAL, "z < y (src/poly_chip.rs:278)");
    return gadget(zkw::G_IN_RANGE, a, nullptr, nullptr, zkw::cpc_in_range(z, y), z, y, Fr::zero());
  }
  int in_field(const DevPoly &a, uint64_t q) { return gadget(zkw::G_IN_FIELD, a, nullptr, nullptr, zkw::cpc_in_field(q), q, 0, Fr::zero()); }
  int mul_gate() {
    if (off + 4 > pk->gate1_cells || n_mg >= 4) return zk_fail_msg(ctx, ZKFHE_EINVAL, "GPU witness stream exceeds the keygen circuit shape");
    mg_off[n_mg++] = off;
    off += 4;
    return ZKFHE_OK;
  }
  int reduce_by_modulo(const DevPoly &a, uint64_t q, DevPoly &out) {
    if (a.bits >= 192 || (q >> 63)) return zk_fail_msg(ctx, ZKFHE_EINVAL, "reduce_by_modulo: operands too wide for the device divider (a < 2^192, q < 2^63)");
    Fr bound;
    zkw::u64 rem;
    zkw::c_divmod(zkw::c_pow2((unsigned)a.bits), q, bound, rem);
    bound = zkw::c_add(bound, zkw::c_u64(1));
    out.d = take(a.len);
    out.len = a.len;
    out.bits = bits_u64(q);
    return gadget(zkw::G_DIV_MOD, a, nullptr, out.d, zkw::cpc_div_mod(q, bound), q, 0, bound);
  }
  int add(const DevPoly &a, const DevPoly &b, DevPoly &out) {
    if (b.len < a.len) return zk_fail_msg(ctx, ZKFHE_EINVAL, "add: operand lengths differ");
    out.d = take(a.len);
    out.len = a.len;
    out.bits = std::max(a.bits, b.bits) + 1;
    return gadget(zkw::G_ADD, a, b.d, out.d, 4, 0, 0, Fr::zero());
  }
  int scalar_mul(const DevPoly &a, const Fr *scalar, uint64_t scalar_bits, DevPoly &out) {
    out.d = take(a.len);
    out.len = a.len;
    out.bits = a.bits + scalar_bits;
    return gadget(zkw::G_SCALAR_MUL, a, scalar, out.d, 4, 0, 0, Fr::zero());
  }
  int equal(const DevPoly &a, const DevPoly &b) {
    if (b.len < a.len) return zk_fail_msg(ctx, ZKFHE_EINVAL, "constrain_equality: operand lengths differ");
    return gadget(zkw::G_EQUAL, a, b.d, nullptr, zkw::cpc_equal(), 0, 0, Fr::zero());
  }
};

struct OpenItem {
  zkp::EvalJob job;
  U256 ev[4];
};

class HeavyGate {
 public:
  static HeavyGate &get() {
    static HeavyGate g;
    return g;
  }
  bool enter() {
    std::unique_lock<std::mutex> l(mu);
    if (slots <= 0) return false;
    const uint64_t my = next_ticket++;
    cv.wait(l, [&] { return slots <= 0 || my < serving + (uint64_t)slots; });
    return true;
  }
  void leave() {
    {
      std::lock_guard<std::mutex> l(mu);
      ++serving;
    }
    cv.notify_all();
  }
  int set(int n) {
    int old;
    {
      std::lock_guard<std::mutex> l(mu);
      old = slots;
      if (n >= 0) slots = n;
    }
    cv.notify_all();
    return old;
  }

 private:
  HeavyGate() {
    if (const char *e = getenv("ZKFHE_GATE")) slots = atoi(e);
  }
  std::mutex mu;
  std::condition_variable cv;
  int slots = 0;
  uint64_t next_ticket = 0, serving = 0;
};
struct GateHold {
  bool held = false;
  void enter() { held = HeavyGate::get().enter(); }
  void leave() {
    if (held) HeavyGate::get().leave();
    held = false;
  }
  ~GateHold() { leave(); }
};

struct Trace {
  bool on;
  double t0, last, cpu_last;
  unsigned long tid;
  static double thread_cpu_ms() {
    timespec ts;
    clock_gettime(CLOCK_THREAD_CPUTIME_ID, &ts);
    return ts.tv_sec * 1e3 + ts.tv_nsec * 1e-6;
  }
  Trace() : on(getenv("ZKFHE_TRACE") != nullptr), t0(now_ms()), last(t0), cpu_last(on ? thread_cpu_ms() : 0), tid((unsigned long)std::hash<std::thread::id>()(std::this_thread::get_id()) % 10000) {}
  void mark(const char *what) {
    if (!on) return;
    const double t = now_ms(), c = thread_cpu_ms();
    fprintf(stderr, "[zkfhe trace %04lu] %8.3f ms (+%7.3f, cpu %6.3f) %s @%.3f\n", tid, t - t0, t - last, c - cpu_last, what, t);
    last = t;
    cpu_last = c;
  }
};

struct BackendGuard {
  GpuPolyMul gpu_mul;
  BackendGuard(zkfhe_ctx *ctx, Workspace *ws) : gpu_mul(ctx, ws) { poly_mul_backend() = &gpu_mul; }
  ~BackendGuard() { poly_mul_backend() = nullptr; }
};

zkp::Mat3 vandermonde3_inverse(const Fr c[3]) {
  zkp::Mat3 vinv;
  for (int k1 = 0; k1 < 3; ++k1) {
    const Fr &a = c[(k1 + 1) % 3], &b = c[(k1 + 2) % 3];
    const Fr den = fr_inv((c[k1] - a) * (c[k1] - b));
    vinv.v[0 * 3 + k1] = a * b * den;
    vinv.v[1 * 3 + k1] = (Fr::zero() - (a + b)) * den;
    vinv.v[2 * 3 + k1] = den;
  }
  return vinv;
}

void interpolate4(const Fr *pts, const Fr *vals, size_t np, Fr rc[4]) {
  for (int q = 0; q < 4; ++q) rc[q] = Fr::zero();
  for (size_t i = 0; i < np; ++i) {
    Fr num[4] = {Fr::one(), Fr::zero(), Fr::zero(), Fr::zero()};
    Fr den = Fr::one();
    size_t deg = 0;
    for (size_t t = 0; t < np; ++t) {
      if (t == i) continue;
      for (size_t q = ++deg; q > 0; --q) num[q] = num[q - 1] - pts[t] * num[q];
      num[0] = Fr::zero() - pts[t] * num[0];
      den = den * (pts[i] - pts[t]);
    }
    const Fr scl = vals[i] * fr_inv(den);
    for (size_t q = 0; q <= deg; ++q) rc[q] = rc[q] + num[q] * scl;
  }
}

void split_permuted(std::vector<AffinePoint> &pts, size_t n_adv, std::vector<AffinePoint> &permuted) {
  const size_t nl = (pts.size() - n_adv) / 2;
  permuted.resize(2 * nl);
  for (size_t i = 0; i < nl; ++i) permuted[2 * i] = pts[n_adv + i], permuted[2 * i + 1] = pts[n_adv + nl + i];
  pts.resize(n_adv);
}

struct Proof {
  zkfhe_ctx *const ctx;
  const zkfhe_srs *const srs;
  zkfhe_bfv_pk *const pk;
  const CircuitConfig &cfg;
  std::vector<U256> &instances;
  Trace &trace;
  Workspace *const ws;
  const NttDomain *const dom;
  const size_t n = cfg.n(), u = cfg.u(), nbl = n - u;
  const unsigned k = cfg.k;
  zkp::RngSeed rseed;
  const uint64_t ctr_adv = 0, ctr_lk = (uint64_t)cfg.n_advice() * nbl, ctr_pz = ctr_lk + 2 * (uint64_t)cfg.n_lookup * nbl,
                 ctr_lz = ctr_pz + (uint64_t)cfg.n_chunks() * (nbl - 1), ctr_rand = ctr_lz + (uint64_t)cfg.n_lookup * (nbl - 1);
  Transcript tr{cfg.transcript};
  bool host_witness = false, early_p1 = false, early_rand = false, inst_via_ring = false;
  const unsigned W_sh = srs->sharded() ? (unsigned)zkfhe_comm_world(srs->comm) : 1u, r_sh = srs->sharded() ? (unsigned)zkfhe_comm_rank(srs->comm) : 0u;
  const size_t c_lo = (size_t)cfg.n_chunks() * r_sh / W_sh, c_hi = (size_t)cfg.n_chunks() * (r_sh + 1) / W_sh;
  BfvState st;
  Assigner as{cfg, false, ws->host_adv};
  GpuPhase1 g1{ctx, pk, ws};
  std::vector<AffinePoint> permuted;
  U256 gamma_rlc;
  Fr beta, gamma, y, x;
  Fr *beta_delta_dev = nullptr;
  Fr pts_rot[6];
  std::vector<OpenItem> items;
  size_t idx_H = 0;
  double t_wit = 0;

  int rng_fill(hipStream_t stream, uint64_t ctr0, uint64_t ctr_col_stride, Fr *dst, size_t per_col, size_t col_stride, size_t n_cols) {
    if (!per_col || !n_cols) return ZKFHE_OK;
    zkp::k_rng_fill<<<grid_for(ctx, per_col * n_cols), 256, 0, stream>>>(rseed, ctr0, ctr_col_stride, dst, per_col, col_stride, n_cols);
    ZK_LAUNCH_CHECK(ctx);
    return ZKFHE_OK;
  }
  zkp::RngRows blind_rows(uint64_t ctr0, uint64_t ctr_col_stride) const {
    return zkp::RngRows{rseed, ctr0, ctr_col_stride, 1};
  }
  const zkfhe_basis *small_basis() const { return srs->g_lagrange_small ? srs->g_lagrange_small : srs->g_lagrange; }
  bool owns_chunk(size_t j) const { return j >= c_lo && j < c_hi; }
  bool owns_col(size_t perm_col) const { return owns_chunk(perm_col / cfg.chunk()); }
  int setup() {
    CK(zkfhe_sync(ctx));
    CK(alloc_witness_buffers(ctx, pk, ws));
    ws->aux->cmd_owner = ctx;
    ws->ring_off = ws->ring_flushed = 0;
    ws->inst_pending = false;
    trace.mark("setup (workspace)");
    early_rand = !srs->sharded();
    if (!early_rand) return ZKFHE_OK;
    zkfhe_ctx *aux = ws->aux;
    Fr *rand_c = ws->misc.fr() + 8 * n, *rand_l = ws->misc.fr() + 9 * n;
    CK(rng_fill(aux->stream, ctr_rand, 0, rand_c, n, n, 1));
    if (int rc = zkfhe_msm_batch_xyzz(aux, srs->g, (const zkfhe_fr *)rand_c, 1, (zkfhe_g1_xyzz *)ws->host_rand_pt))
      return zk_fail_msg(ctx, rc, std::string("random polynomial commitment (auxiliary stream): ") + zkfhe_last_error(aux));
    if (int rc = zkfhe_ntt_batch_to(aux, (const zkfhe_fr *)rand_c, (zkfhe_fr *)rand_l, 1, (int)k, 0))
      return zk_fail_msg(ctx, rc, std::string("random polynomial, Lagrange form (auxiliary stream): ") + zkfhe_last_error(aux));
    ZK_HIP(ctx, hipEventRecord(ws->ev_rand, aux->stream));
    return ZKFHE_OK;
  }
  int phase0(const char *input_json, const FastInput *words, std::vector<AffinePoint> &pts) {
    Context ctx0(CTX_PHASE0, false, false);
    std::vector<Cell> make_public;
    instances.clear();
    tr.common_scalar(pk->vk_digest);
    const auto on_public = [&](const std::vector<Cell> &pub) {
      instances.reserve(pub.size());
      for (const Cell &c : pub) instances.push_back(c.value);
      const size_t n_key = std::min<size_t>(instances.size(), 2 * (size_t)pk->prm.N);
      Transcript::State mid;
      if (input_json && pk->prehash.take(input_json, strlen(input_json), instances.data(), instances.size(), mid)) {
        tr.restore(mid);
      } else if (!n_key || !pk->prefix.capacity()) {
        tr.common_scalars_async(instances);
      } else if (pk->prefix.lookup(instances.data(), n_key, mid)) {
        tr.restore(mid);
        tr.common_scalars_async(std::vector<U256>(instances.begin() + (long)n_key, instances.end()));
      } else {
        PrefixCache *cache = &pk->prefix;
        std::vector<U256> key(instances.begin(), instances.begin() + (long)n_key);
        tr.common_scalars_async_marked(instances, n_key, [cache, key](const Transcript::State &st) { cache->insert(key.data(), key.size(), st); });
      }
    };
    std::string rendered;
    if (words ? !bfv_phase0_fast_values(ctx0, *words, pk->prm, make_public, st, on_public)
              : !bfv_phase0_fast(ctx0, input_json, strlen(input_json), pk->prm, make_public, st, on_public)) {
      if (words) {
        rendered = render_input_json(*words);
        input_json = rendered.c_str();
      }
      const CircuitInput in = CircuitInput::parse_json(input_json);
      trace.mark("parse_json");
      st = bfv_phase0(ctx0, in, pk->prm, make_public, on_public);
    }
    trace.mark("bfv_phase0");
    as.place(ctx0, true);
    trace.mark("place phase 0");
    if (instances.size() > n) return zk_fail_msg(ctx, ZKFHE_EINVAL, "more public inputs than rows");
    inst_via_ring = instances.size() * 32 <= ((size_t)1 << 20);
    if (inst_via_ring) {
      STAGE(staged, U256, ws, instances.data(), instances.size() * 32);
      ws->inst_src = (const Fr *)(ws->ring + ((const uint8_t *)staged - (const uint8_t *)ws->dev_ring.p));
      ws->inst_n = instances.size();
      ws->inst_pending = true;
    }
    trace.mark("transcript: instances");
    CK(blind_and_upload(0, cfg.n_gate0));
    trace.mark("blind + upload phase 0");
    const char *witness_env = getenv("ZKFHE_WITNESS");
    host_witness = witness_env && strcmp(witness_env, "host") == 0;
    const char *early_env = getenv("ZKFHE_EARLY_P1");
    const bool early_want = early_env ? early_env[0] == '1' : (cfg.transcript == TR_POSEIDON || k >= 18);
    early_p1 = early_want && !host_witness && cfg.n_lookup > 0 && cfg.lookup_bits == 8;
    if (host_witness) return commit_cols(ctx, srs, small_basis(), ws->adv_l.fr(), cfg.n_gate0, (G1Affine *)ws->points.p, pts);
    CK(srs_msm_pts(ctx, srs, small_basis(), ws->adv_l.fr(), cfg.n_gate0, ws->host_pts));
    CK(srs_record(ctx, srs, ws->ev_pts));
    CK(g1.launch(st));
    if (early_p1) {
      CK(g1.place_early(blind_rows(ctr_adv + (uint64_t)cfg.n_gate0 * nbl, nbl), cfg.n_rlc));
      CK(permute_lookups(ws->host_early_err));
      CK(srs_msm_pts(ctx, srs, small_basis(), ws->adv_l.fr() + (size_t)cfg.n_gate0 * n, cfg.n_advice() - cfg.n_gate0 + 2 * cfg.n_lookup, ws->host_early));
      CK(srs_record(ctx, srs, ws->ev_early));
    }
    ZK_HIP(ctx, hipEventSynchronize(ws->ev_pts));
    pts.resize(cfg.n_gate0);
    points_canon(srs, ws->host_pts, cfg.n_gate0, pts.data());
    return ZKFHE_OK;
  }
  int blind_and_upload(unsigned col_lo, unsigned col_hi) {
    const char *upload_env = getenv("ZKFHE_UPLOAD");
    const bool upload_by_copy = upload_env && !strcmp(upload_env, "copy");
    Fr *dst = ws->adv_l.fr() + (size_t)col_lo * n;
    if (!upload_by_copy) {
      zkp::k_to_mont_blind<<<grid_for(ctx, (size_t)(col_hi - col_lo) * n), 256, 0, ctx->stream>>>((const Fr *)as.t.advice[col_lo], dst, n, (unsigned)u, col_hi - col_lo,
                                                                                                   blind_rows(ctr_adv + (uint64_t)col_lo * nbl, nbl));
      ZK_LAUNCH_CHECK(ctx);
      return ZKFHE_OK;
    }
    ZK_HIP(ctx, zk_memcpy_async(ctx, dst, as.t.advice[col_lo], (size_t)(col_hi - col_lo) * n * 32, hipMemcpyHostToDevice, ctx->stream));
    CK(zkfhe_fr_to_mont(ctx, (const zkfhe_fr *)dst, (zkfhe_fr *)dst, (size_t)(col_hi - col_lo) * n));
    return rng_fill(ctx->stream, ctr_adv + (uint64_t)col_lo * nbl, nbl, dst + u, nbl, n, col_hi - col_lo);
  }
  int permute_lookups(int *err) {
    *err = 0;
    const zkp::RngRows blind_lk = blind_rows(ctr_lk, 2 * nbl);
    return zkw::lookup_permute(ctx, ws->adv_l.fr() + (size_t)cfg.adv_lookup0() * n, n, (unsigned)u, cfg.n_lookup, ws->la_l.fr(), ws->ls_l.fr(), err, nullptr, &blind_lk);
  }
  int phase1_host(std::vector<AffinePoint> &pts) {
    Context ctx_gate(CTX_GATE1, false, false), ctx_rlc(CTX_RLC1, true, false);
    bfv_phase1(st, pk->prm, ctx_gate, ctx_rlc, gamma_rlc);
    as.place(ctx_gate, true);
    as.place(ctx_rlc, true);
    as.place_lookups(ctx_gate);
    t_wit = now_ms();
    CK(blind_and_upload(cfg.n_gate0, cfg.n_advice()));
    trace.mark("blind + upload phase 1");
    return commit_cols_out(ctx, srs, small_basis(), ws->adv_l.fr() + (size_t)cfg.n_gate0 * n, cfg.n_advice() - cfg.n_gate0, ws, pts);
  }
  int phase1_device(std::vector<AffinePoint> &pts) {
    const size_t n_adv1 = cfg.n_advice() - cfg.n_gate0;
    Context ctx_rlc(CTX_RLC1, true, false);
    U256 evals[12];
    bfv_phase1_rlc(st, ctx_rlc, gamma_rlc, evals);
    trace.mark("rlc context");
    as.place(ctx_rlc, true);
    trace.mark("place rlc");
    if (early_p1) return phase1_early_finish(evals, n_adv1, pts);
    CK(g1.finish(evals, blind_rows(ctr_adv + (uint64_t)cfg.n_gate0 * nbl, nbl)));
    trace.mark("gpu phase 1 (enqueue)");
    t_wit = now_ms();
    CK(blind_and_upload(cfg.adv_rlc0(), cfg.n_advice()));
    trace.mark("blind + upload phase 1");
    if (!cfg.n_lookup) return commit_cols_out(ctx, srs, small_basis(), ws->adv_l.fr() + (size_t)cfg.n_gate0 * n, n_adv1, ws, pts);
    if (cfg.lookup_bits != 8) return zk_fail_msg(ctx, ZKFHE_EINVAL, "the device lookup permutation is built for lookup_bits = 8");
    int *lookup_err = ws->out_flags() + 2;
    CK(permute_lookups(lookup_err));
    CK(commit_cols_out(ctx, srs, small_basis(), ws->adv_l.fr() + (size_t)cfg.n_gate0 * n, n_adv1 + 2 * cfg.n_lookup, ws, pts));
    if (*lookup_err) return zk_fail_msg(ctx, ZKFHE_EINVAL, "lookup input not in table: a range check of the witness fails");
    split_permuted(pts, n_adv1, permuted);
    return ZKFHE_OK;
  }
  int phase1_early_finish(const U256 evals[12], size_t n_adv1, std::vector<AffinePoint> &pts) {
    const GpuPhase1::PatchPlan plan = g1.patch_plan();
    const size_t np = plan.columns.size();
    Fr *patch_cols = ws->tmp_c.fr();
    std::vector<zkfhe_sparse_term> terms;
    const bool sparse = !srs->sharded() && zkfhe_basis_has_multiples(srs->g_lagrange);
    CK(g1.patch(evals, plan, patch_cols, sparse ? &terms : nullptr));
    CK(blind_and_upload(cfg.adv_rlc0(), cfg.n_advice()));
    if (np + cfg.n_rlc > ws->out_pts_cap)
      return zk_fail_msg(ctx, ZKFHE_EINVAL, "early phase-1 commitment: correction points do not fit the workspace (set ZKFHE_EARLY_P1=0)");
    uint8_t *fix_dev = ws->out_pts();
    const size_t ps = pt_stride(srs);
    if (np && sparse) {
      STAGE(terms_dev, zkfhe_sparse_term, ws, terms.data(), terms.size() * sizeof(zkfhe_sparse_term));
      CK(flush_staged(ctx, ws));
      CK(zkfhe_msm_sparse_xyzz(ctx, srs->g_lagrange, terms_dev, terms.size(), np, (zkfhe_g1_xyzz *)fix_dev));
    } else if (np) {
      CK(srs_msm_pts(ctx, srs, srs->g_lagrange, patch_cols, np, fix_dev));
    }
    if (cfg.n_rlc) CK(srs_msm_pts(ctx, srs, srs->g_lagrange, ws->adv_l.fr() + (size_t)cfg.adv_rlc0() * n, cfg.n_rlc, fix_dev + np * ps));
    CK(srs_join(ctx, srs, false));
    ZK_HIP(ctx, zk_wait(ctx));
    if (*ws->host_early_err) return zk_fail_msg(ctx, ZKFHE_EINVAL, "lookup input not in table: a range check of the witness fails");
    for (size_t t = 0; t < np; ++t) {
      if (srs->sharded()) {
        G1Affine &e = ((G1Affine *)ws->host_early)[plan.columns[t]];
        zk::G1X acc = zk::g1x_from_affine(e);
        zk::g1x_add_affine(acc, ((const G1Affine *)fix_dev)[t], false);
        e = zk::g1x_to_affine(acc);
      } else {
        zk::g1x_add(((zk::G1X *)ws->host_early)[plan.columns[t]], ((const zk::G1X *)fix_dev)[t]);
      }
    }
    for (unsigned j = 0; j < cfg.n_rlc; ++j) memcpy(ws->host_early + (size_t)(cfg.adv_rlc0() - cfg.n_gate0 + j) * ps, fix_dev + (np + j) * ps, ps);
    trace.mark("gpu phase 1 (enqueue)");
    t_wit = now_ms();
    trace.mark("blind + upload phase 1");
    pts.resize(n_adv1 + 2 * (size_t)cfg.n_lookup);
    points_canon(srs, ws->host_early, pts.size(), pts.data());
    split_permuted(pts, n_adv1, permuted);
    return ZKFHE_OK;
  }
  int lookup_columns() {
    if (!cfg.n_lookup) return ZKFHE_OK;
    if (host_witness) {
      std::vector<U256> input, ap, sp;
      U256 *stA = ws->host_blind, *stS = ws->host_blind + (size_t)cfg.n_lookup * n;
      for (unsigned i = 0; i < cfg.n_lookup; ++i) {
        input.assign(as.t.advice[cfg.adv_lookup0() + i], as.t.advice[cfg.adv_lookup0() + i] + u);
        permute_lookup(input, u, 1u << cfg.lookup_bits, ap, sp);
        U256 *colA = stA + (size_t)i * n, *colS = stS + (size_t)i * n;
        std::copy(ap.begin(), ap.end(), colA);
        std::copy(sp.begin(), sp.end(), colS);
        for (size_t r = u; r < n; ++r) colA[r] = colS[r] = fe::zero();
      }
      ZK_HIP(ctx, zk_memcpy_async(ctx, ws->la_l.p, ws->host_blind, 2 * (size_t)cfg.n_lookup * n * 32, hipMemcpyHostToDevice, ctx->stream));
      CK(zkfhe_fr_to_mont(ctx, (const zkfhe_fr *)ws->la_l.p, (zkfhe_fr *)ws->la_l.p, 2 * (size_t)cfg.n_lookup * n));
      CK(rng_fill(ctx->stream, ctr_lk, 2 * nbl, ws->la_l.fr() + u, nbl, n, cfg.n_lookup));
      CK(rng_fill(ctx->stream, ctr_lk + nbl, 2 * nbl, ws->ls_l.fr() + u, nbl, n, cfg.n_lookup));
      std::vector<AffinePoint> pts;
      CK(commit_cols_out(ctx, srs, small_basis(), ws->la_l.fr(), 2 * cfg.n_lookup, ws, pts));
      split_permuted(pts, 0, permuted);
    }
    tr.write_points(permuted);
    return ZKFHE_OK;
  }
  zkp::PermArgs perm_args() const {
    zkp::PermArgs pa;
    pa.adv = ws->adv_l.fr();
    pa.constcol = pk->fixed_l.fr() + (size_t)cfg.fix_const() * n;
    pa.inst = ws->inst_l.fr();
    pa.sigma = pk->sigma_l.fr();
    pa.wpow = dom->fwd;
    pa.beta_delta = beta_delta_dev;
    pa.beta = beta;
    pa.gamma = gamma;
    pa.n_advice = cfg.n_advice();
    pa.n_perm = cfg.n_perm();
    pa.chunk = cfg.chunk();
    pa.n_chunks = cfg.n_chunks();
    pa.n = n;
    return pa;
  }
  int prefix_products(const Fr *ratio, Fr *z, size_t n_cols, const zkp::RngRows &blind, Fr *totals_dev) {
    const size_t nb_z = nbl - 1;
    if (n <= 65536) {
      zkp::k_prefix_product<<<(unsigned)n_cols + zkp::rng_tail_grid(blind, n_cols * nb_z, 1024), 1024, 0, ctx->stream>>>(ratio, z, totals_dev, n, (unsigned)u, (unsigned)n_cols, blind);
      ZK_LAUNCH_CHECK(ctx);
      return ZKFHE_OK;
    }
    CK(rng_fill(ctx->stream, blind.ctr0, blind.ctr_col_stride, z + (u + 1), nb_z, n, n_cols));
    const unsigned seg_len = 32768, segs = (unsigned)(n / seg_len);
    Fr *seg = ws->den.fr();
    if ((size_t)n_cols * segs * 32 > ws->den.bytes) return zk_fail_msg(ctx, ZKFHE_EINVAL, "prefix products: segment buffer too small");
    zkp::k_prefix_seg_totals<<<dim3(segs, (unsigned)n_cols), 1024, 0, ctx->stream>>>(ratio, seg, n, (unsigned)u, seg_len);
    ZK_LAUNCH_CHECK(ctx);
    zkp::k_prefix_seg_scan<<<(unsigned)((n_cols + 63) / 64), 64, 0, ctx->stream>>>(seg, segs, (unsigned)n_cols, totals_dev);
    ZK_LAUNCH_CHECK(ctx);
    zkp::k_prefix_seg_apply<<<dim3(segs, (unsigned)n_cols), 1024, 0, ctx->stream>>>(ratio, seg, z, n, (unsigned)u, seg_len);
    ZK_LAUNCH_CHECK(ctx);
    return ZKFHE_OK;
  }
  int grand_products() {
    if (inst_via_ring) {
      CK(flush_staged(ctx, ws));
    } else {
      if (instances.size() < ws->inst_count)
        ZK_HIP(ctx, zk_memset_async(ctx, ws->inst_l.fr() + instances.size(), 0, (ws->inst_count - instances.size()) * 32, ctx->stream));
      CK(upload_canon(ctx, ws->inst_l.fr(), instances.data(), instances.size()));
      ws->inst_count = instances.size();
    }
    U256 dcan;
    memcpy(dcan.l, DELTA_CANON, 32);
    beta_delta_dev = (Fr *)ws->small.p;
    zkp::k_powers<<<1, 256, 0, ctx->stream>>>(beta, mont(dcan), beta_delta_dev, cfg.n_perm());
    ZK_LAUNCH_CHECK(ctx);
    const size_t nch = cfg.n_chunks(), nb_z = nbl - 1;
    zkp::k_perm_num_den<<<grid_for(ctx, nch * n), 256, 0, ctx->stream>>>(perm_args(), ws->num.fr(), ws->den.fr());
    ZK_LAUNCH_CHECK(ctx);
    CK(zkfhe_fr_batch_invert_mul(ctx, (const zkfhe_fr *)ws->den.p, (zkfhe_fr *)ws->num.p, nch * n));
    Fr *totals_dev = (Fr *)ws->small.p + 4096;
    CK(prefix_products(ws->num.fr(), ws->pz_l.fr(), nch, blind_rows(ctr_pz, nb_z), totals_dev));
    int *const closes = ws->out_flags();
    closes[0] = closes[1] = 1;
    zkp::k_chunk_carry<<<1, 1024, 0, ctx->stream>>>(totals_dev, (unsigned)nch, 0, closes);
    ZK_LAUNCH_CHECK(ctx);
    zkp::k_scale_rows<<<grid_for(ctx, nch * (u + 1)), 256, 0, ctx->stream>>>(ws->pz_l.fr(), totals_dev, n, (unsigned)(u + 1), (unsigned)nch);
    ZK_LAUNCH_CHECK(ctx);
    if (cfg.n_lookup) {
      const size_t nl = cfg.n_lookup;
      zkp::k_lookup_num_den<<<grid_for(ctx, nl * n), 256, 0, ctx->stream>>>(ws->adv_l.fr() + (size_t)cfg.adv_lookup0() * n,
                                                                            pk->fixed_l.fr() + (size_t)cfg.fix_table() * n, ws->la_l.fr(), ws->ls_l.fr(),
                                                                            beta, gamma, (unsigned)nl, n, ws->num.fr(), ws->den.fr());
      ZK_LAUNCH_CHECK(ctx);
      CK(zkfhe_fr_batch_invert_mul(ctx, (const zkfhe_fr *)ws->den.p, (zkfhe_fr *)ws->num.p, nl * n));
      CK(prefix_products(ws->num.fr(), ws->lz_l.fr(), nl, blind_rows(ctr_lz, nb_z), totals_dev));
      zkp::k_chunk_carry<<<1, 1024, 0, ctx->stream>>>(totals_dev, (unsigned)nl, 1, closes + 1);
      ZK_LAUNCH_CHECK(ctx);
    }
    std::vector<AffinePoint> pz_commit;
    CK(commit_cols_out(ctx, srs, srs->g_lagrange, ws->pz_l.fr(), nch + cfg.n_lookup, ws, pz_commit));
    if (!closes[0]) return zk_fail_msg(ctx, ZKFHE_EINVAL, "permutation argument does not close: a copy constraint is violated");
    if (!closes[1]) return zk_fail_msg(ctx, ZKFHE_EINVAL, "lookup argument does not close");
    tr.write_points(pz_commit);
    return ZKFHE_OK;
  }
  int random_poly() {
    Fr *rand_c = ws->misc.fr() + 8 * n;
    if (early_rand) {
      ZK_HIP(ctx, hipEventSynchronize(ws->ev_rand));
      ZK_HIP(ctx, hipStreamWaitEvent(ctx->stream, ws->ev_rand, 0));
      AffinePoint rp;
      points_canon(srs, ws->host_rand_pt, 1, &rp);
      tr.write_point(rp);
    } else {
      CK(rng_fill(ctx->stream, ctr_rand, 0, rand_c, n, n, 1));
      std::vector<AffinePoint> rand_commit;
      CK(commit_cols_out(ctx, srs, srs->g, rand_c, 1, ws, rand_commit));
      tr.write_point(rand_commit[0]);
    }
    return ZKFHE_OK;
  }
  int grow_qgather(size_t bytes) {
    if (ws->qgather.bytes >= bytes) return ZKFHE_OK;
    CK(zkfhe_sync(ctx));
    ws->qgather.release();
    return ws->qgather.alloc(ctx, bytes);
  }
  int sum_shares(size_t slots, Fr *dst) {
    CK(zkfhe_comm_join(ctx, srs->comm, 0));
    for (size_t j = 0; j < slots; ++j) {
      zkp::k_sum_rows<<<grid_for(ctx, n), 256, 0, ctx->stream>>>(ws->qgather.fr() + j * (size_t)W_sh * n, W_sh, n, dst + j * n);
      ZK_LAUNCH_CHECK(ctx);
    }
    return ZKFHE_OK;
  }
  zkp::QArgs quotient_args(const zkp::QGroup *groups_dev, int q_rows) const {
    zkp::QArgs qa;
    qa.adv = ws->adv_ext.fr();
    qa.fix = pk->fixed_ext.fr();
    qa.sig = pk->sigma_ext.fr();
    qa.pz = ws->pz_ext.fr();
    qa.lz = ws->lz_ext.fr();
    qa.la = ws->la_ext.fr();
    qa.ls = ws->ls_ext.fr();
    qa.inst = ws->inst_ext.fr();
    qa.lext = pk->l_ext.fr();
    qa.xs = pk->xs_ext.fr();
    qa.beta_delta = beta_delta_dev;
    qa.groups = groups_dev;
    qa.partials = ws->partials.fr();
    qa.y = y;
    qa.beta = beta;
    qa.gamma = gamma;
    qa.gamma_rlc = mont(gamma_rlc);
    qa.log_n = k;
    qa.u = (unsigned)u;
    qa.n_gate = cfg.n_gate();
    qa.n_rlc = cfg.n_rlc;
    qa.adv_rlc0 = cfg.adv_rlc0();
    qa.fix_qrlc0 = cfg.fix_qrlc0();
    qa.fix_const = cfg.fix_const();
    qa.fix_table = cfg.fix_table();
    qa.adv_lookup0 = cfg.adv_lookup0();
    qa.n_lookup = cfg.n_lookup;
    qa.n_advice = cfg.n_advice();
    qa.n_perm = cfg.n_perm();
    qa.chunk = cfg.chunk();
    qa.n_chunks = cfg.n_chunks();
    qa.rows = (unsigned)q_rows;
    return qa;
  }
  int launch_quotient(zkp::QArgs &qa, size_t pt0, size_t count, size_t G, const Fr *ypow_dev, const Fr *zinv_dev) {
    qa.pt0 = pt0;
    qa.pt_count = count;
    const unsigned blocks = (unsigned)((count + 255) / 256);
    if (G) {
      zkp::k_quotient_partials<<<dim3(blocks, (unsigned)G), 256, 0, ctx->stream>>>(qa);
      ZK_LAUNCH_CHECK(ctx);
    }
    zkp::k_quotient_combine<<<blocks, 256, 0, ctx->stream>>>(ws->partials.fr(), ypow_dev, (unsigned)G, zinv_dev, k, qa.rows, pt0, count, ws->h_ext.fr());
    ZK_LAUNCH_CHECK(ctx);
    return ZKFHE_OK;
  }
  int quotient(std::vector<AffinePoint> &h_commit) {
    const int q_rows = pk->ext_rows;
    const Fr wext = zk_fr_root_of_unity((int)k + 2);
    if (W_sh == 1) {
      CK(extend_cols(ctx, pk, ws, ws->all_l.fr(), ws->n_all, ws->all_ext.fr()));
    } else {
      const size_t ecol = n * (size_t)q_rows;
      auto ext_range = [&](const View &l, const View &e, size_t lo, size_t hi) -> int {
        if (hi <= lo) return ZKFHE_OK;
        return extend_cols(ctx, pk, ws, l.fr() + lo * n, hi - lo, e.fr() + lo * ecol);
      };
      const size_t a_lo = std::min<size_t>(c_lo * cfg.chunk(), cfg.n_advice()), a_hi = std::min<size_t>(c_hi * cfg.chunk(), cfg.n_advice());
      CK(ext_range(ws->adv_l, ws->adv_ext, a_lo, a_hi));
      const size_t l_lo = a_lo > cfg.adv_lookup0() ? std::min<size_t>(a_lo - cfg.adv_lookup0(), cfg.n_lookup) : 0;
      const size_t l_hi = a_hi > cfg.adv_lookup0() ? std::min<size_t>(a_hi - cfg.adv_lookup0(), cfg.n_lookup) : 0;
      CK(ext_range(ws->la_l, ws->la_ext, l_lo, l_hi));
      CK(ext_range(ws->ls_l, ws->ls_ext, l_lo, l_hi));
      CK(ext_range(ws->lz_l, ws->lz_ext, l_lo, l_hi));
      CK(ext_range(ws->pz_l, ws->pz_ext, c_lo ? c_lo - 1 : 0, c_hi));
      if (owns_col(cfg.perm_inst())) CK(ext_range(ws->inst_l, ws->inst_ext, 0, 1));
    }
    const size_t nch = cfg.n_chunks();
    std::vector<zkp::QGroup> groups;
    std::vector<size_t> last_e;
    size_t e = 0;
    auto run = [&](int type, size_t first, size_t count, size_t max_group, size_t expr_per_unit, const std::function<bool(size_t)> &owned) {
      size_t j = first;
      while (j < first + count) {
        if (!owned(j)) {
          e += expr_per_unit;
          ++j;
          continue;
        }
        size_t len = 0;
        while (j + len < first + count && len < max_group && owned(j + len)) ++len;
        groups.push_back(zkp::QGroup{type, (int)j, (int)len, 0});
        e += len * expr_per_unit;
        last_e.push_back(e - 1);
        j += len;
      }
    };
    run(zkp::QG_GATE, 0, cfg.n_gate(), 8, 1, [&](size_t j) { return owns_col(j); });
    run(zkp::QG_RLC, 0, cfg.n_rlc, cfg.n_rlc ? cfg.n_rlc : 1, 1, [&](size_t j) { return owns_col(cfg.adv_rlc0() + j); });
    run(zkp::QG_PERM_FIRST, 0, 1, 1, 1, [&](size_t) { return owns_chunk(0); });
    run(zkp::QG_PERM_LAST, 0, 1, 1, 1, [&](size_t) { return owns_chunk(nch - 1); });
    run(zkp::QG_PERM_C, 1, nch - 1, 32, 1, [&](size_t j) { return owns_chunk(j); });
    run(zkp::QG_PERM_D, 0, nch, 4, 1, [&](size_t j) { return owns_chunk(j); });
    run(zkp::QG_LOOKUP, 0, cfg.n_lookup, 3, 5, [&](size_t i) { return owns_col(cfg.adv_lookup0() + i); });
    const size_t E = e, G = groups.size();
    if (G > 96 || G * n * (size_t)q_rows * 32 > ws->partials.bytes) return zk_fail_msg(ctx, ZKFHE_EINVAL, "too many quotient groups for the workspace");
    std::vector<Fr> ypow(G);
    for (size_t g = 0; g < G; ++g) ypow[g] = zk::zk_fr_to_29(fr_pow(y, E - 1 - last_e[g]));
    if (groups.empty()) groups.push_back(zkp::QGroup{});
    if (ypow.empty()) ypow.push_back(Fr::zero());
    STAGE(groups_dev, zkp::QGroup, ws, groups.data(), groups.size() * sizeof(zkp::QGroup));
    STAGE(ypow_dev, Fr, ws, ypow.data(), ypow.size() * 32);
    const Fr gn = fr_pow(mont_u64(COSET_G), n), i4 = fr_pow(wext, n);
    Fr zinv[4], cur = gn;
    for (int t = 0; t < 4; ++t) {
      zinv[t] = zk::zk_fr_to_29(fr_inv(cur - Fr::one()));
      cur = cur * i4;
    }
    STAGE(zinv_dev, Fr, ws, zinv, 4 * 32);
    CK(flush_staged(ctx, ws));
    zkp::QArgs qa = quotient_args(groups_dev, q_rows);
    const size_t npts = n * (size_t)q_rows;
    if (W_sh == 1) {
      CK(launch_quotient(qa, 0, npts, G, ypow_dev, zinv_dev));
    } else {
      CK(grow_qgather((size_t)W_sh * npts * 32));
      for (int k1 = 0; k1 < q_rows; ++k1) {
        CK(launch_quotient(qa, (size_t)k1 * n, n, G, ypow_dev, zinv_dev));
        CK(zkfhe_comm_all_gather_async(ctx, srs->comm, ws->h_ext.fr() + (size_t)k1 * n, ws->qgather.fr() + (size_t)k1 * W_sh * n, n * 32));
      }
      CK(sum_shares((size_t)q_rows, ws->h_ext.fr()));
    }
    const Fr g = mont_u64(COSET_G);
    if (q_rows == 4) {
      CK(zkfhe_coset_ntt_batch(ctx, (const zkfhe_fr *)ws->h_ext.p, (zkfhe_fr *)ws->h_c.p, 1, (int)k, 2, (const zkfhe_fr *)&g, 1));
    } else {
      Fr *rows3 = ws->partials.fr();
      const Fr *pw = pk->ext3_pw.fr();
      CK(zkfhe_ntt_batch_to(ctx, (const zkfhe_fr *)ws->h_ext.p, (zkfhe_fr *)rows3, 3, (int)k, 1));
      const Fr c[3] = {fr_pow(g, n), fr_pow(g * wext, n), fr_pow(g * wext * wext, n)};
      zkp::k_ext3_combine<<<(unsigned)((n + 255) / 256), 256, 0, ctx->stream>>>(rows3, pw, vandermonde3_inverse(c), n, ws->h_c.fr());
      ZK_LAUNCH_CHECK(ctx);
    }
    CK(commit_cols_out(ctx, srs, srs->g, ws->h_c.fr(), 3, ws, h_commit));
    if (q_rows == 4) {
      std::vector<U256> top(8);
      CK(zkfhe_download(ctx, top.data(), ws->h_c.fr() + 3 * n, 8 * 32));
      for (const auto &v : top)
        if (!v.is_zero()) return zk_fail_msg(ctx, ZKFHE_EINVAL, "quotient degree too high: a constraint is violated");
    }
    return ZKFHE_OK;
  }
  void add_item(const Fr *lagr, std::initializer_list<int> rots) {
    OpenItem it{{lagr, 0, {0, 0, 0, 0}}};
    for (int r : rots) it.job.rot[it.job.n_rot++] = r;
    items.push_back(it);
  }
  int lincomb(const Fr *const *pp, const Fr *pw, unsigned msz, Fr *dst) {
    const unsigned per = 48, chunks = (msz + per - 1) / per;
    if (chunks > 1 && (size_t)chunks * n * 32 <= ws->partials.bytes) {
      dim3 lg(grid_for(ctx, n), chunks);
      zkp::k_lincomb_ptrs_chunked<<<lg, 256, 0, ctx->stream>>>(pp, pw, msz, per, n, ws->partials.fr());
      ZK_LAUNCH_CHECK(ctx);
      zkp::k_sum_rows<<<grid_for(ctx, n), 256, 0, ctx->stream>>>(ws->partials.fr(), chunks, n, dst);
    } else {
      zkp::k_lincomb_ptrs<<<grid_for(ctx, n), 256, 0, ctx->stream>>>(pp, pw, msz, n, dst);
    }
    ZK_LAUNCH_CHECK(ctx);
    return ZKFHE_OK;
  }
  int evaluations() {
    Fr *rand_c = ws->misc.fr() + 8 * n, *rand_l = ws->misc.fr() + 9 * n, *H_c = ws->misc.fr() + 10 * n, *H_l = ws->misc.fr() + 11 * n;
    const Fr xn = fr_pow(x, n);
    const Fr w = dom->omega;
    pts_rot[0] = x;
    pts_rot[1] = x * w;
    pts_rot[2] = pts_rot[1] * w;
    pts_rot[3] = pts_rot[2] * w;
    pts_rot[4] = x * fr_pow(w, u);
    pts_rot[5] = x * dom->omega_inv;
    const size_t nch = cfg.n_chunks();
    for (unsigned c = 0; c < cfg.n_advice(); ++c) {
      const Fr *p = ws->adv_l.fr() + (size_t)c * n;
      if (c < cfg.n_gate()) add_item(p, {0, 1, 2, 3});
      else if (c < cfg.adv_rlc0()) add_item(p, {0});
      else add_item(p, {0, 1, 2});
    }
    for (unsigned c = 0; c < cfg.n_fixed(); ++c) add_item(pk->fixed_l.fr() + (size_t)c * n, {0});
    idx_H = items.size();
    add_item(H_l, {0});
    add_item(rand_l, {0});
    for (unsigned c = 0; c < cfg.n_perm(); ++c) add_item(pk->sigma_l.fr() + (size_t)c * n, {0});
    for (unsigned j = 0; j < nch; ++j) {
      if (j + 1 != nch) add_item(ws->pz_l.fr() + (size_t)j * n, {0, 1, 4});
      else add_item(ws->pz_l.fr() + (size_t)j * n, {0, 1});
    }
    for (unsigned i = 0; i < cfg.n_lookup; ++i) {
      add_item(ws->lz_l.fr() + (size_t)i * n, {0, 1});
      add_item(ws->la_l.fr() + (size_t)i * n, {0, 5});
      add_item(ws->ls_l.fr() + (size_t)i * n, {0});
    }
    std::vector<zkp::EvalJob> jobs(items.size());
    for (size_t i = 0; i < items.size(); ++i) jobs[i] = items[i].job;
    const Fr sc[3] = {zk::zk_fr_to_29(Fr::one()), zk::zk_fr_to_29(xn), zk::zk_fr_to_29(xn * xn)};
    const Fr *ptrs[3] = {ws->h_c.fr(), ws->h_c.fr() + n, ws->h_c.fr() + 2 * n};
    STAGE(ptrs_dev, const Fr *, ws, ptrs, sizeof(ptrs));
    STAGE(sc_dev, Fr, ws, sc, sizeof(sc));
    STAGE(pts_dev, Fr, ws, pts_rot, sizeof(pts_rot));
    STAGE(jobs_dev, zkp::EvalJob, ws, jobs.data(), jobs.size() * sizeof(zkp::EvalJob));
    CK(flush_staged(ctx, ws));
    CK(lincomb(ptrs_dev, sc_dev, 3, H_c));
    CK(zkfhe_ntt_batch_to(ctx, (const zkfhe_fr *)H_c, (zkfhe_fr *)H_l, 1, (int)k, 0));
    if (!early_rand) CK(zkfhe_ntt_batch_to(ctx, (const zkfhe_fr *)rand_c, (zkfhe_fr *)rand_l, 1, (int)k, 0));
    Fr *bw = ws->misc.fr();
    zkp::k_bary_den<<<grid_for(ctx, 6 * n), 256, 0, ctx->stream>>>(dom->fwd, pts_dev, 6, n, bw);
    ZK_LAUNCH_CHECK(ctx);
    CK(zkfhe_fr_batch_invert(ctx, (zkfhe_fr *)bw, 6 * n));
    const Fr c = zk::zk_fr_to_29((xn - Fr::one()) * dom->n_inv);
    zkp::k_bary_weights<<<grid_for(ctx, 6 * n), 256, 0, ctx->stream>>>(dom->fwd, c, 6 * n, n, bw);
    ZK_LAUNCH_CHECK(ctx);
    DevBuf &od = ws->evout;
    const bool shard_open = W_sh > 1 && k >= 14;
    const size_t per_rank = shard_open ? (jobs.size() + W_sh - 1) / W_sh : jobs.size();
    const size_t j_lo = shard_open ? std::min(jobs.size(), per_rank * r_sh) : 0, j_hi = shard_open ? std::min(jobs.size(), j_lo + per_rank) : jobs.size();
    if (shard_open && (per_rank * W_sh * 4 * 32 > od.bytes || per_rank * (W_sh + 1) * 4 * 32 > ws->h_ext.bytes))
      return zk_fail_msg(ctx, ZKFHE_EINVAL, "too many ranks for the evaluation gather buffers");
    Fr *ev_dst = shard_open ? ws->h_ext.fr() : od.fr();
    const unsigned slices = (n > 32768 && (size_t)16 * jobs.size() * 4 * 32 <= ws->partials.bytes) ? 16u : 1u;
    if (j_hi > j_lo) {
      const zkp::EvalJob *jp = jobs_dev + j_lo;
      const unsigned nj = (unsigned)(j_hi - j_lo);
      if (slices == 1) {
        zkp::k_eval_jobs<<<nj, 256, 0, ctx->stream>>>(jp, bw, n, ev_dst + (shard_open ? 0 : j_lo * 4));
      } else {
        zkp::k_eval_jobs<<<dim3(nj, slices), 256, 0, ctx->stream>>>(jp, bw, n, ws->partials.fr());
        ZK_LAUNCH_CHECK(ctx);
        zkp::k_sum_rows<<<grid_for(ctx, (size_t)nj * 4), 256, 0, ctx->stream>>>(ws->partials.fr(), slices, (size_t)nj * 4, ev_dst + (shard_open ? 0 : j_lo * 4));
      }
      ZK_LAUNCH_CHECK(ctx);
    }
    if (shard_open) CK(zkfhe_comm_all_gather(ctx, srs->comm, ev_dst, od.p, per_rank * 4 * 32));
    if (jobs.size() * 4 > ws->out_ev_cap) return zk_fail_msg(ctx, ZKFHE_EINVAL, "more evaluations than the result block holds");
    CK(zkfhe_fr_from_mont(ctx, (const zkfhe_fr *)od.p, (zkfhe_fr *)ws->out_ev(), jobs.size() * 4));
    ZK_HIP(ctx, zk_wait(ctx));
    trace.mark("evaluations (GPU)");
    const U256 *ev = ws->out_ev();
    for (size_t i = 0; i < items.size(); ++i)
      for (int r = 0; r < items[i].job.n_rot; ++r) items[i].ev[r] = ev[i * 4 + r];
    return ZKFHE_OK;
  }
  int shplonk() {
    const OpenLayout layout(cfg);
    if (items.size() != layout.count || idx_H != layout.H) return zk_fail_msg(ctx, ZKFHE_EINVAL, "opening layout mismatch");
    std::vector<U256> evs;
    evs.reserve(items.size() * 2);
    for (size_t i = 0; i < items.size(); ++i) {
      if (i == idx_H) continue;
      for (int r = 0; r < items[i].job.n_rot; ++r) evs.push_back(items[i].ev[r]);
    }
    tr.write_scalars(evs);
    const Fr yq = mont(tr.squeeze());
    trace.mark("transcript: evaluations");
    std::vector<int> all_rots;
    const std::vector<OpenSet> sets = intermediate_sets(layout, open_queries(cfg, layout), all_rots);
    const size_t ns = sets.size();
    Fr *F = ws->misc.fr() + 12 * n;
    if (ns > 8) return zk_fail_msg(ctx, ZKFHE_EINVAL, "too many rotation sets");
    std::vector<zkp::ShSet> shsets(ns);
    std::vector<const Fr *const *> set_ptrs(ns);
    std::vector<const Fr *> set_pw(ns);
    for (size_t j = 0; j < ns; ++j) {
      const auto &mem = sets[j].members;
      std::vector<const Fr *> ptrs(mem.size());
      std::vector<Fr> pw(mem.size());
      Fr cur = Fr::one();
      const size_t np = sets[j].rots.size();
      if (np > 4) return zk_fail_msg(ctx, ZKFHE_EINVAL, "too many points in a rotation set");
      Fr comb[4] = {Fr::zero(), Fr::zero(), Fr::zero(), Fr::zero()};
      for (size_t m = 0; m < mem.size(); ++m) {
        ptrs[m] = items[mem[m]].job.col;
        pw[m] = zk::zk_fr_to_29(cur);
        for (size_t t = 0; t < np; ++t) comb[t] = comb[t] + cur * mont(items[mem[m]].ev[layout.eval_slot(mem[m], sets[j].rots[t])]);
        cur = cur * yq;
      }
      STAGE(pd, const Fr *, ws, ptrs.data(), mem.size() * sizeof(void *));
      STAGE(sd, Fr, ws, pw.data(), mem.size() * 32);
      set_ptrs[j] = pd;
      set_pw[j] = sd;
      zkp::ShSet &S = shsets[j];
      S.n_pts = (int)np;
      for (size_t t = 0; t < 4; ++t) S.pts[t] = t < np ? pts_rot[sets[j].rots[t]] : Fr::zero();
      interpolate4(S.pts, comb, np, S.rc);
    }
    const Fr v = mont(tr.squeeze());
    Fr vj = Fr::one();
    for (size_t j = 0; j < ns; ++j) {
      shsets[j].vj = vj;
      shsets[j].coef = Fr::zero();
      shsets[j].r_u = Fr::zero();
      vj = vj * v;
    }
    STAGE(sets_dev, zkp::ShSet, ws, shsets.data(), ns * sizeof(zkp::ShSet));
    CK(flush_staged(ctx, ws));
    const bool shard_sets = W_sh > 1 && k >= 14;
    if (shard_sets) CK(grow_qgather((size_t)W_sh * ns * n * 32));
    for (size_t j = 0; j < ns; ++j) {
      const size_t all = sets[j].members.size();
      const size_t m_lo = shard_sets ? all * r_sh / W_sh : 0, m_hi = shard_sets ? all * (r_sh + 1) / W_sh : all;
      CK(lincomb(set_ptrs[j] + m_lo, set_pw[j] + m_lo, (unsigned)(m_hi - m_lo), F + j * n));
      if (shard_sets) CK(zkfhe_comm_all_gather_async(ctx, srs->comm, F + j * n, ws->qgather.fr() + j * (size_t)W_sh * n, n * 32));
    }
    if (shard_sets) CK(sum_shares(ns, F));
    Fr *zs = ws->misc.fr() + 20 * n;
    Fr *hq = ws->misc.fr() + 28 * n;
    Fr *Wq = ws->misc.fr() + 29 * n;
    Fr *dinv = ws->misc.fr() + 30 * n;
    zkp::k_sh_zs<<<grid_for(ctx, ns * n), 256, 0, ctx->stream>>>(sets_dev, (unsigned)ns, dom->fwd, n, zs);
    ZK_LAUNCH_CHECK(ctx);
    CK(zkfhe_fr_batch_invert(ctx, (zkfhe_fr *)zs, ns * n));
    zkp::k_sh_h<<<grid_for(ctx, n), 256, 0, ctx->stream>>>(sets_dev, (unsigned)ns, F, zs, dom->fwd, n, hq);
    ZK_LAUNCH_CHECK(ctx);
    std::vector<AffinePoint> hq_commit, w_commit;
    CK(commit_cols_out(ctx, srs, srs->g_lagrange, hq, 1, ws, hq_commit));
    tr.write_point(hq_commit[0]);
    const Fr uu = mont(tr.squeeze());
    trace.mark("shplonk h (GPU)");
    Fr ztu = Fr::one();
    for (int r : all_rots) ztu = ztu * (uu - pts_rot[r]);
    Fr z0_diff_inv = Fr::one();
    zkp::ShW shw{};
    for (size_t j = 0; j < ns; ++j) {
      Fr zdiff = Fr::one();
      for (int r : all_rots)
        if (std::find(sets[j].rots.begin(), sets[j].rots.end(), r) == sets[j].rots.end()) zdiff = zdiff * (uu - pts_rot[r]);
      if (j == 0) z0_diff_inv = fr_inv(zdiff);
      shsets[j].coef = shsets[j].vj * zdiff * z0_diff_inv;
      Fr ru = shsets[j].rc[3];
      for (int q = 2; q >= 0; --q) ru = ru * uu + shsets[j].rc[q];
      shsets[j].r_u = ru;
      shw.coef[j] = shsets[j].coef;
      shw.r_u[j] = ru;
    }
    ztu = ztu * z0_diff_inv;
    zkp::k_sh_den<<<(unsigned)((n + 255) / 256), 256, 0, ctx->stream>>>(dom->fwd, uu, n, dinv);
    ZK_LAUNCH_CHECK(ctx);
    CK(zkfhe_fr_batch_invert(ctx, (zkfhe_fr *)dinv, n));
    zkp::k_sh_w<<<grid_for(ctx, n), 256, 0, ctx->stream>>>(shw, (unsigned)ns, F, hq, ztu, dinv, n, Wq);
    ZK_LAUNCH_CHECK(ctx);
    CK(commit_cols_out(ctx, srs, srs->g_lagrange, Wq, 1, ws, w_commit));
    tr.write_point(w_commit[0]);
    return ZKFHE_OK;
  }
};

int prove_impl(zkfhe_ctx *ctx, const zkfhe_srs *srs, zkfhe_bfv_pk *pk, const char *input_json, const FastInput *words, const uint8_t seed[32],
               std::vector<uint8_t> &proof, std::vector<U256> &instances, float *timings) {
  const double t_start = now_ms();
  ctx->cmd_count[ZK_CMD_KERNEL] = ctx->cmd_count[ZK_CMD_COPY] = ctx->cmd_count[ZK_CMD_FILL] = 0;
  Trace trace;
  const NttDomain *dom;
  CK(zk_domain(ctx, (int)pk->cfg.k, &dom));
  Workspace *ws;
  CK(get_workspace(ctx, pk, &ws));
  BackendGuard guard(ctx, ws);
  Proof P{ctx, srs, pk, pk->cfg, instances, trace, ws, dom};
  memcpy(P.rseed.w, seed, 32);
  CK(P.setup());
  std::vector<AffinePoint> pts;
  CK(P.phase0(input_json, words, pts));
  trace.mark("commit phase 0 (GPU)");
  ctx->proof_marks[0] = (float)(now_ms() - t_start);
  for (const auto &p : pts) P.tr.write_point(p);
  P.gamma_rlc = P.tr.squeeze();
  ctx->proof_marks[1] = (float)(now_ms() - t_start);
  CK(P.host_witness ? P.phase1_host(pts) : P.phase1_device(pts));
  trace.mark("commit phase 1 (GPU)");
  P.tr.write_points(pts);
  P.tr.squeeze();
  CK(P.lookup_columns());
  trace.mark("lookup permute + commit");
  P.beta = mont(P.tr.squeeze());
  P.gamma = mont(P.tr.squeeze());
  GateHold gate;
  if (!srs->sharded()) gate.enter();
  CK(P.grand_products());
  CK(P.random_poly());
  P.y = mont(P.tr.squeeze());
  const double t_commit = now_ms();
  trace.mark("grand products + commits");
  CK(P.quotient(pts));
  gate.leave();
  for (const auto &p : pts) P.tr.write_point(p);
  P.x = mont(P.tr.squeeze());
  const double t_quot = now_ms();
  trace.mark("quotient");
  CK(P.evaluations());
  CK(P.shplonk());
  proof = P.tr.out;
  const double t_end = now_ms();
  trace.mark("evaluations + shplonk");
  ctx->proof_marks[2] = (float)(t_end - t_start);
  if (timings) {
    timings[0] = (float)(P.t_wit - t_start);
    timings[1] = (float)(t_commit - P.t_wit);
    timings[2] = (float)(t_quot - t_commit);
    timings[3] = (float)(t_end - t_quot);
    timings[4] = (float)(t_end - t_start);
  }
  return ZKFHE_OK;
}

int prove_out(zkfhe_ctx *ctx, const zkfhe_srs *srs, const zkfhe_bfv_pk *pk, const char *input_json, const FastInput *words, const uint8_t seed[32],
              uint8_t *proof_out, size_t proof_cap, size_t *proof_len, uint8_t *instances_out, size_t *n_instances, float *timings_ms) {
  std::vector<uint8_t> proof;
  std::vector<U256> inst;
  CK(prove_impl(ctx, srs, const_cast<zkfhe_bfv_pk *>(pk), input_json, words, seed, proof, inst, timings_ms));
  if (proof.size() > proof_cap) return zk_fail_msg(ctx, ZKFHE_EINVAL, "proof buffer too small");
  memcpy(proof_out, proof.data(), proof.size());
  *proof_len = proof.size();
  if (n_instances) {
    const size_t have = *n_instances;
    *n_instances = inst.size();
    if (instances_out) {
      if (have < inst.size()) return zk_fail_msg(ctx, ZKFHE_EINVAL, "instance buffer too small (the required count is returned in *n_instances)");
      memcpy(instances_out, inst.data(), inst.size() * 32);
    }
  }
  return ZKFHE_OK;
}

}

extern "C" {

int zkfhe_bfv_prove(zkfhe_ctx *ctx, const zkfhe_srs *srs, const zkfhe_bfv_pk *pk, const char *input_json, const uint8_t seed[32],
                    uint8_t *proof_out, size_t proof_cap, size_t *proof_len, uint8_t *instances_out, size_t *n_instances, float *timings_ms) {
  ZK_ENTER(ctx);
  ZK_ARG(ctx, srs && pk && input_json && seed && proof_out && proof_len);
  try {
    pos::BulkClientScope in_flight;
    return prove_out(ctx, srs, pk, input_json, nullptr, seed, proof_out, proof_cap, proof_len, instances_out, n_instances, timings_ms);
  } catch (const std::exception &e) {
    return zk_fail_msg(ctx, ZKFHE_EINVAL, e.what());
  }
}

int zkfhe_bfv_prove_words(zkfhe_ctx *ctx, const zkfhe_srs *srs, const zkfhe_bfv_pk *pk, const zkfhe_bfv_words *words, const uint8_t seed[32],
                          uint8_t *proof_out, size_t proof_cap, size_t *proof_len, uint8_t *instances_out, size_t *n_instances, float *timings_ms) {
  ZK_ENTER(ctx);
  ZK_ARG(ctx, srs && pk && words && seed && proof_out && proof_len);
  const uint64_t *src[8] = {words->pk0, words->pk1, words->m, words->u, words->e0, words->e1, words->c0, words->c1};
  for (const uint64_t *p : src) ZK_ARG(ctx, p != nullptr);
  try {
    pos::BulkClientScope in_flight;
    const size_t N = pk->prm.N;
    FastInput in;
    for (int k = 0; k < 8; ++k) in.a[k].assign(src[k], src[k] + N);
    in.a[8].assign(N + 1, 0);
    in.a[8][0] = in.a[8][N] = 1;
    return prove_out(ctx, srs, pk, nullptr, &in, seed, proof_out, proof_cap, proof_len, instances_out, n_instances, timings_ms);
  } catch (const std::exception &e) {
    return zk_fail_msg(ctx, ZKFHE_EINVAL, e.what());
  }
}

int zkfhe_prover_gate(int n) { return HeavyGate::get().set(n); }

int zkfhe_lookup_permute(zkfhe_ctx *ctx, const zkfhe_fr *cols_dev, size_t n_cols, size_t n, uint32_t usable_rows, zkfhe_fr *a_dev, zkfhe_fr *s_dev, int *not_in_table) {
  ZK_ENTER(ctx);
  ZK_ARG(ctx, cols_dev && a_dev && s_dev && not_in_table && n_cols > 0 && n_cols < 65536 && usable_rows <= n && usable_rows >= 256);
  void *flag;
  CK(zk_scratch(ctx, 3, 64 + n_cols * 256 * sizeof(unsigned), &flag));
  ZK_HIP(ctx, zk_memset_async(ctx, flag, 0, 4, ctx->stream));
  CK(zkw::lookup_permute(ctx, (const Fr *)cols_dev, n, usable_rows, (unsigned)n_cols, (Fr *)a_dev, (Fr *)s_dev, (int *)flag, (unsigned *)((char *)flag + 64)));
  return zkfhe_download(ctx, not_in_table, flag, 4);
}

int zkfhe_bfv_pk_prehash(const zkfhe_bfv_pk *pk_c, const char *input_json, uint64_t *started, uint64_t *taken, uint64_t *pending) {
  if (!pk_c) return ZKFHE_EINVAL;
  zkfhe_bfv_pk *pk = const_cast<zkfhe_bfv_pk *>(pk_c);
  int rc = ZKFHE_OK;
  if (input_json) {
    const uint32_t kind = pk->cfg.transcript;
    const U256 digest = pk->vk_digest;
    const BfvParams prm = pk->prm;
    PrefixCache *cache = &pk->prefix;
    const bool ok = pk->prehash.start(input_json, strlen(input_json), [kind, digest, prm, cache](const std::string &text, std::vector<U256> &inst, Transcript::State &out) {
      struct PublicInputsKnown {};
      try {
        Context ctx0(CTX_PHASE0, false, false);
        std::vector<Cell> make_public;
        BfvState st;
        const auto on_public = [&](const std::vector<Cell> &pub) {
          inst.reserve(pub.size());
          for (const Cell &c : pub) inst.push_back(c.value);
          throw PublicInputsKnown{};
        };
        if (!bfv_phase0_fast(ctx0, text.c_str(), text.size(), prm, make_public, st, on_public))
          (void)bfv_phase0(ctx0, CircuitInput::parse_json(text.c_str()), prm, make_public, on_public);
        throw std::runtime_error("phase 0 ended without public inputs");
      } catch (const PublicInputsKnown &) {
      }
      const size_t n_key = std::min<size_t>(inst.size(), 2 * (size_t)prm.N);
      Transcript tr(kind);
      tr.common_scalar(digest);
      Transcript::State mid;
      size_t from = 0;
      if (n_key && cache->capacity()) {
        if (cache->lookup(inst.data(), n_key, mid)) {
          tr.restore(mid);
        } else {
          tr.common_scalars_async(std::vector<U256>(inst.begin(), inst.begin() + (long)n_key));
          mid = tr.snapshot();
          cache->insert(inst.data(), n_key, mid);
        }
        from = n_key;
      }
      tr.common_scalars_async(std::vector<U256>(inst.begin() + (long)from, inst.end()));
      out = tr.snapshot();
    });
    if (!ok) rc = ZKFHE_EINVAL;
  }
  pk->prehash.stats(started, taken, pending);
  return rc;
}

int zkfhe_bfv_witness_stream(zkfhe_ctx *ctx, const zkfhe_bfv_pk *pk_c, const char *input_json, const uint8_t gamma_le[32], uint8_t *cells_out,
                             size_t cap_cells, size_t *n_cells) {
  ZK_ENTER(ctx);
  ZK_ARG(ctx, pk_c && input_json && gamma_le && n_cells);
  zkfhe_bfv_pk *pk = const_cast<zkfhe_bfv_pk *>(pk_c);
  *n_cells = pk->gate1_cells;
  if (!cells_out) return ZKFHE_OK;
  ZK_ARG(ctx, cap_cells >= pk->gate1_cells);
  try {
    Workspace *ws;
    CK(get_workspace(ctx, pk, &ws));
    CK(zkfhe_sync(ctx));
    BackendGuard guard(ctx, ws);
    Context ctx0(CTX_PHASE0, false, false), ctx_rlc(CTX_RLC1, true, false);
    std::vector<Cell> make_public;
    BfvState st;
    if (!bfv_phase0_fast(ctx0, input_json, strlen(input_json), pk->prm, make_public, st)) st = bfv_phase0(ctx0, CircuitInput::parse_json(input_json), pk->prm, make_public);
    U256 gamma, evals[12];
    memcpy(gamma.l, gamma_le, 32);
    if (!(gamma < fe::MOD)) return zk_fail_msg(ctx, ZKFHE_EINVAL, "gamma is not a canonical Fr value");
    CK(alloc_witness_buffers(ctx, pk, ws));
    ws->ring_off = ws->ring_flushed = 0;
    GpuPhase1 g1(ctx, pk, ws);
    CK(g1.launch(st));
    bfv_phase1_rlc(st, ctx_rlc, gamma, evals);
    CK(g1.finish(evals, zkp::RngRows{}));
    CK(zkfhe_fr_from_mont(ctx, (const zkfhe_fr *)ws->stream.p, (zkfhe_fr *)ws->stream.p, pk->gate1_cells));
    ZK_HIP(ctx, zk_memcpy_async(ctx, cells_out, ws->stream.p, pk->gate1_cells * 32, hipMemcpyDeviceToHost, ctx->stream));
    CK(zkfhe_sync(ctx));
    return ZKFHE_OK;
  } catch (const std::exception &e) {
    return zk_fail_msg(ctx, ZKFHE_EINVAL, e.what());
  }
}

}
```

### zk-fhe_amd/host/prover_kernels.hip.hpp

```cpp
#pragma once
#include "../csrc/ctx.hpp"
#include "../csrc/fr9.hip.hpp"

namespace zkp {

using zk::Fr;

static __global__ void __launch_bounds__(256) k_powers(Fr start, Fr base, Fr *__restrict__ out, size_t n) {
  for (size_t i = blockIdx.x * (size_t)blockDim.x + threadIdx.x; i < n; i += (size_t)gridDim.x * blockDim.x) {
    Fr r = start, b = base;
    for (size_t e = i; e; e >>= 1) {
      if (e & 1) r = r * b;
      b = zk::fp_sqr<zk::FrP>(b);
    }
    out[i] = r;
  }
}

__device__ __forceinline__ unsigned long long rotr64(unsigned long long x, int n) { return (x >> n) | (x << (64 - n)); }
__device__ __forceinline__ Fr rng_draw(const unsigned long long seed[4], unsigned long long ctr) {
  typedef unsigned long long u64;
  const u64 IV[8] = {0x6a09e667f3bcc908ULL, 0xbb67ae8584caa73bULL, 0x3c6ef372fe94f82bULL, 0xa54ff53a5f1d36f1ULL,
                     0x510e527fade682d1ULL, 0x9b05688c2b3e6c1fULL, 0x1f83d9abfb41bd6bULL, 0x5be0cd19137e2179ULL};
  const unsigned char S[12][16] = {
      {0, 1, 2, 3, 4, 5, 6, 7, 8, 9, 10, 11, 12, 13, 14, 15}, {14, 10, 4, 8, 9, 15, 13, 6, 1, 12, 0, 2, 11, 7, 5, 3},
      {11, 8, 12, 0, 5, 2, 15, 13, 10, 14, 3, 6, 7, 1, 9, 4}, {7, 9, 3, 1, 13, 12, 11, 14, 2, 6, 5, 10, 4, 0, 15, 8},
      {9, 0, 5, 7, 2, 4, 10, 15, 14, 1, 11, 12, 6, 8, 3, 13}, {2, 12, 6, 10, 0, 11, 8, 3, 4, 13, 7, 5, 15, 14, 1, 9},
      {12, 5, 1, 15, 14, 13, 4, 10, 0, 7, 6, 3, 9, 2, 8, 11}, {13, 11, 7, 14, 12, 1, 3, 9, 5, 0, 15, 4, 8, 6, 2, 10},
      {6, 15, 14, 9, 11, 3, 0, 8, 12, 2, 13, 7, 1, 4, 10, 5}, {10, 2, 8, 4, 7, 6, 1, 5, 15, 11, 9, 14, 3, 12, 13, 0},
      {0, 1, 2, 3, 4, 5, 6, 7, 8, 9, 10, 11, 12, 13, 14, 15}, {14, 10, 4, 8, 9, 15, 13, 6, 1, 12, 0, 2, 11, 7, 5, 3}};
  u64 h[8], m[16], v[16];
#pragma unroll
  for (int i = 0; i < 8; ++i) h[i] = IV[i];
  h[0] ^= 0x01010040ULL;
  h[6] ^= 0x6e722d6568666b7aULL;
  h[7] ^= 0x0000000000000067ULL;
#pragma unroll
  for (int i = 0; i < 16; ++i) m[i] = 0;
  m[0] = seed[0], m[1] = seed[1], m[2] = seed[2], m[3] = seed[3], m[4] = ctr;
#pragma unroll
  for (int i = 0; i < 8; ++i) {
    v[i] = h[i];
    v[i + 8] = IV[i];
  }
  v[12] ^= 40;
  v[14] = ~v[14];
#define ZK_B2G(a, b, c, d, x, y)          \
  v[a] = v[a] + v[b] + (x);               \
  v[d] = rotr64(v[d] ^ v[a], 32);         \
  v[c] = v[c] + v[d];                     \
  v[b] = rotr64(v[b] ^ v[c], 24);         \
  v[a] = v[a] + v[b] + (y);               \
  v[d] = rotr64(v[d] ^ v[a], 16);         \
  v[c] = v[c] + v[d];                     \
  v[b] = rotr64(v[b] ^ v[c], 63);
#pragma unroll
  for (int r = 0; r < 12; ++r) {
    ZK_B2G(0, 4, 8, 12, m[S[r][0]], m[S[r][1]])
    ZK_B2G(1, 5, 9, 13, m[S[r][2]], m[S[r][3]])
    ZK_B2G(2, 6, 10, 14, m[S[r][4]], m[S[r][5]])
    ZK_B2G(3, 7, 11, 15, m[S[r][6]], m[S[r][7]])
    ZK_B2G(0, 5, 10, 15, m[S[r][8]], m[S[r][9]])
    ZK_B2G(1, 6, 11, 12, m[S[r][10]], m[S[r][11]])
    ZK_B2G(2, 7, 8, 13, m[S[r][12]], m[S[r][13]])
    ZK_B2G(3, 4, 9, 14, m[S[r][14]], m[S[r][15]])
  }
#undef ZK_B2G
#pragma unroll
  for (int i = 0; i < 8; ++i) h[i] ^= v[i] ^ v[i + 8];
  Fr lo, hi;
#pragma unroll
  for (int i = 0; i < 4; ++i) {
    lo.l[2 * i] = (zk::u32)h[i];
    lo.l[2 * i + 1] = (zk::u32)(h[i] >> 32);
    hi.l[2 * i] = (zk::u32)h[4 + i];
    hi.l[2 * i + 1] = (zk::u32)(h[4 + i] >> 32);
  }
#pragma unroll
  for (int k = 0; k < 5; ++k) {
    zk::fp_reduce_once<zk::FrP>(lo.l);
    zk::fp_reduce_once<zk::FrP>(hi.l);
  }
  const Fr r2 = Fr::r2();
  const Fr lom = zk::fp_mul<zk::FrP>(lo, r2);
  const Fr him = zk::fp_mul<zk::FrP>(zk::fp_mul<zk::FrP>(hi, r2), r2);
  return zk::fp_add<zk::FrP>(lom, him);
}
struct RngSeed {
  unsigned long long w[4];
};
struct RngRows {
  RngSeed seed;
  unsigned long long ctr0, ctr_col_stride;
  int on;
};
__device__ __forceinline__ Fr rng_row(const RngRows &b, size_t col, size_t j) { return rng_draw(b.seed.w, b.ctr0 + col * b.ctr_col_stride + j); }
__device__ __forceinline__ void rng_tail_blocks(const RngRows &b, unsigned first_block, Fr *__restrict__ dst, size_t per_col, size_t col_stride, size_t n_cols) {
  const size_t total = per_col * n_cols, T = (size_t)(gridDim.x - first_block) * blockDim.x;
  for (size_t g = (size_t)(blockIdx.x - first_block) * blockDim.x + threadIdx.x; g < total; g += T) {
    const size_t c = g / per_col, j = g - c * per_col;
    dst[c * col_stride + j] = rng_row(b, c, j);
  }
}
static inline unsigned rng_tail_grid(const RngRows &b, size_t draws, unsigned threads) { return b.on ? (unsigned)((draws + threads - 1) / threads) : 0u; }
static __global__ void __launch_bounds__(256) k_rng_fill(RngSeed seed, unsigned long long ctr0, unsigned long long ctr_col_stride, Fr *__restrict__ dst,
                                                  size_t per_col, size_t col_stride, size_t n_cols) {
  const size_t total = per_col * n_cols;
  for (size_t g = blockIdx.x * (size_t)blockDim.x + threadIdx.x; g < total; g += (size_t)gridDim.x * blockDim.x) {
    const size_t c = g / per_col, j = g - c * per_col;
    dst[c * col_stride + j] = rng_draw(seed.w, ctr0 + c * ctr_col_stride + j);
  }
}

static __global__ void __launch_bounds__(256) k_to_mont_blind(const Fr *__restrict__ src, Fr *__restrict__ dst, size_t n, unsigned u, size_t n_cols, RngRows blind) {
  const size_t total = n_cols * n;
  for (size_t g = blockIdx.x * (size_t)blockDim.x + threadIdx.x; g < total; g += (size_t)gridDim.x * blockDim.x) {
    const size_t c = g / n, r = g - c * n;
    dst[g] = r >= u ? rng_row(blind, c, r - u) : zk::fr29_to_mont(src[g]);
  }
}
static __global__ void __launch_bounds__(256) k_ring_flush(const uint4 *__restrict__ src, uint4 *__restrict__ dst, size_t n16, const Fr *__restrict__ inst_src,
                                                    Fr *__restrict__ inst_dst, size_t inst_n, size_t inst_zero) {
  const size_t total = n16 + inst_n + inst_zero;
  for (size_t g = blockIdx.x * (size_t)blockDim.x + threadIdx.x; g < total; g += (size_t)gridDim.x * blockDim.x) {
    if (g < n16) dst[g] = src[g];
    else if (g < n16 + inst_n) inst_dst[g - n16] = zk::fr29_to_mont(inst_src[g - n16]);
    else inst_dst[g - n16] = Fr::zero();
  }
}

static __global__ void __launch_bounds__(256) k_srs_den(const Fr *__restrict__ wpow, Fr s, Fr nn, Fr *__restrict__ out, size_t n) {
  size_t i = blockIdx.x * (size_t)blockDim.x + threadIdx.x;
  if (i < n) out[i] = (s - wpow[i]) * nn;
}
static __global__ void __launch_bounds__(256) k_srs_li(const Fr *__restrict__ wpow, Fr snm1, Fr *__restrict__ inv_inout, size_t n) {
  size_t i = blockIdx.x * (size_t)blockDim.x + threadIdx.x;
  if (i < n) inv_inout[i] = wpow[i] * snm1 * inv_inout[i];
}
static __global__ void __launch_bounds__(256) k_fill_point(zk::G1Affine p, zk::G1Affine *__restrict__ out, size_t n) {
  size_t i = blockIdx.x * (size_t)blockDim.x + threadIdx.x;
  if (i < n) out[i] = p;
}

static __global__ void __launch_bounds__(256) k_sigma_values(const uint32_t *__restrict__ target, const Fr *__restrict__ dpow,
                                                      const Fr *__restrict__ wpow, Fr *__restrict__ out, size_t cells, int log_n) {
  size_t i = blockIdx.x * (size_t)blockDim.x + threadIdx.x;
  if (i >= cells) return;
  const uint32_t t = target[i];
  out[i] = dpow[t >> log_n] * wpow[t & ((1u << log_n) - 1)];
}

struct PermArgs {
  const Fr *adv;
  const Fr *constcol;
  const Fr *inst;
  const Fr *sigma;
  const Fr *wpow;
  const Fr *beta_delta;
  Fr beta, gamma;
  unsigned n_advice, n_perm, chunk, n_chunks;
  size_t n;
};
__device__ __forceinline__ const Fr *perm_col(const PermArgs &a, unsigned c) {
  return c < a.n_advice ? a.adv + (size_t)c * a.n : (c == a.n_advice ? a.constcol : a.inst);
}
static __global__ void __launch_bounds__(256) k_perm_num_den(PermArgs a, Fr *__restrict__ num, Fr *__restrict__ den) {
  const size_t total = (size_t)a.n_chunks * a.n;
  for (size_t g = blockIdx.x * (size_t)blockDim.x + threadIdx.x; g < total; g += (size_t)gridDim.x * blockDim.x) {
    const unsigned j = (unsigned)(g / a.n);
    const size_t i = g - (size_t)j * a.n;
    Fr nu = Fr::one(), de = Fr::one();
    const Fr w = a.wpow[i];
    for (unsigned c = j * a.chunk; c < (j + 1) * a.chunk && c < a.n_perm; ++c) {
      const Fr v = perm_col(a, c)[i];
      nu = nu * (v + a.beta_delta[c] * w + a.gamma);
      de = de * (v + a.beta * a.sigma[(size_t)c * a.n + i] + a.gamma);
    }
    num[g] = nu;
    den[g] = de;
  }
}
static __global__ void __launch_bounds__(256) k_lookup_num_den(const Fr *__restrict__ a_cols, const Fr *__restrict__ table, const Fr *__restrict__ la,
                                                        const Fr *__restrict__ ls, Fr beta, Fr gamma, unsigned n_lookup, size_t n,
                                                        Fr *__restrict__ num, Fr *__restrict__ den) {
  const size_t total = (size_t)n_lookup * n;
  const zk::Fr9S beta9 = zk::fr9_load(beta);
  const zk::Fr9C gamma9 = zk::fr9_load32(gamma);
  for (size_t g = blockIdx.x * (size_t)blockDim.x + threadIdx.x; g < total; g += (size_t)gridDim.x * blockDim.x) {
    const size_t i = g % n;
    num[g] = zk::fr9_store(zk::fr9_lookup_term(zk::fr9_load(a_cols[g]), beta9, zk::fr9_lookup_sum(zk::fr9_load32(table[i]), gamma9)));
    den[g] = zk::fr9_store(zk::fr9_lookup_term(zk::fr9_load(la[g]), beta9, zk::fr9_lookup_sum(zk::fr9_load32(ls[g]), gamma9)));
  }
}

static __global__ void __launch_bounds__(1024) k_prefix_product(const Fr *__restrict__ ratio, Fr *__restrict__ z, Fr *__restrict__ total, size_t n,
                                                         unsigned u, unsigned n_cols, RngRows blind) {
  __shared__ Fr sh[1024];
  if (blockIdx.x >= n_cols) {
    rng_tail_blocks(blind, n_cols, z + u + 1, n - u - 1, n, n_cols);
    return;
  }
  const size_t col = blockIdx.x;
  const Fr *r = ratio + col * n;
  Fr *o = z + col * n;
  const unsigned per = (unsigned)((n + 1023) / 1024);
  const unsigned lo = threadIdx.x * per;
  zk::Lz<0, 1, 2> local = zk::lz_widen<0, 1, 2>(zk::fr9_one());
  for (unsigned k = 0; k < per; ++k) {
    const unsigned i = lo + k;
    if (i < u) local = zk::fr9_mul(local, zk::fr9_load32(r[i]));
  }
  sh[threadIdx.x] = zk::fr9_store(local);
  __syncthreads();
  for (unsigned d = 1; d < 1024; d <<= 1) {
    if (threadIdx.x >= d) local = zk::fr9_mul(local, zk::fr9_load32(sh[threadIdx.x - d]));
    __syncthreads();
    if (threadIdx.x >= d) sh[threadIdx.x] = zk::fr9_store(local);
    __syncthreads();
  }
  zk::Lz<0, 1, 2> acc = zk::lz_widen<0, 1, 2>(threadIdx.x ? zk::fr9_load(sh[threadIdx.x - 1]) : zk::fr9_one());
  for (unsigned k = 0; k < per; ++k) {
    const unsigned i = lo + k;
    if (i <= u) o[i] = zk::fr9_store(acc);
    if (i < u) acc = zk::fr9_mul(acc, zk::fr9_load32(r[i]));
  }
  if (threadIdx.x == 1023) total[col] = sh[1023];
}
static __global__ void __launch_bounds__(1024) k_prefix_seg_totals(const Fr *__restrict__ ratio, Fr *__restrict__ seg_total, size_t n, unsigned u, unsigned seg_len) {
  __shared__ Fr sh[1024];
  const size_t col = blockIdx.y;
  const unsigned seg = blockIdx.x, base = seg * seg_len;
  const Fr *r = ratio + col * n;
  const unsigned per = (seg_len + 1023) / 1024, lo = base + threadIdx.x * per;
  Fr local = Fr::one();
  for (unsigned k = 0; k < per; ++k) {
    const unsigned i = lo + k;
    if (i < u && i < base + seg_len) local = local * r[i];
  }
  sh[threadIdx.x] = local;
  __syncthreads();
  for (unsigned d = 512; d > 0; d >>= 1) {
    if (threadIdx.x < d) sh[threadIdx.x] = sh[threadIdx.x] * sh[threadIdx.x + d];
    __syncthreads();
  }
  if (threadIdx.x == 0) seg_total[col * gridDim.x + seg] = sh[0];
}
static __global__ void __launch_bounds__(64) k_prefix_seg_scan(Fr *__restrict__ seg_total, unsigned segs, unsigned n_cols, Fr *__restrict__ total) {
  const unsigned col = blockIdx.x * blockDim.x + threadIdx.x;
  if (col >= n_cols) return;
  Fr acc = Fr::one();
  for (unsigned s = 0; s < segs; ++s) {
    const Fr t = seg_total[(size_t)col * segs + s];
    seg_total[(size_t)col * segs + s] = acc;
    acc = acc * t;
  }
  total[col] = acc;
}
static __global__ void __launch_bounds__(1024) k_prefix_seg_apply(const Fr *__restrict__ ratio, const Fr *__restrict__ seg_carry, Fr *__restrict__ z, size_t n, unsigned u,
                                                            unsigned seg_len) {
  __shared__ Fr sh[1024];
  const size_t col = blockIdx.y;
  const unsigned seg = blockIdx.x, base = seg * seg_len, end = base + seg_len;
  const Fr *r = ratio + col * n;
  Fr *o = z + col * n;
  const unsigned per = (seg_len + 1023) / 1024, lo = base + threadIdx.x * per;
  Fr local = Fr::one();
  for (unsigned k = 0; k < per; ++k) {
    const unsigned i = lo + k;
    if (i < u && i < end) local = local * r[i];
  }
  sh[threadIdx.x] = local;
  __syncthreads();
  for (unsigned d = 1; d < 1024; d <<= 1) {
    Fr v = sh[threadIdx.x];
    Fr other = threadIdx.x >= d ? sh[threadIdx.x - d] : Fr::one();
    __syncthreads();
    if (threadIdx.x >= d) sh[threadIdx.x] = other * v;
    __syncthreads();
  }
  Fr acc = seg_carry[col * gridDim.x + seg];
  if (threadIdx.x) acc = acc * sh[threadIdx.x - 1];
  for (unsigned k = 0; k < per; ++k) {
    const unsigned i = lo + k;
    if (i >= end) break;
    if (i <= u) o[i] = acc;
    if (i < u) acc = acc * r[i];
  }
}
static __global__ void __launch_bounds__(1024) k_chunk_carry(Fr *__restrict__ total, unsigned count, int check_ones, int *__restrict__ closes) {
  __shared__ Fr sh[1024];
  __shared__ int bad;
  const unsigned t = threadIdx.x;
  if (t == 0) bad = 0;
  __syncthreads();
  const unsigned per = (count + 1023) / 1024, lo = t * per;
  if (check_ones) {
    const Fr one = Fr::one();
    for (unsigned k = 0; k < per; ++k)
      if (lo + k < count && !(total[lo + k] == one)) bad = 1;
    __syncthreads();
    if (t == 0) *closes = bad ? 0 : 1;
    return;
  }
  Fr vals[4];
  Fr local = Fr::one();
#pragma unroll
  for (unsigned k = 0; k < 4; ++k) {
    vals[k] = k < per && lo + k < count ? total[lo + k] : Fr::one();
    local = local * vals[k];
  }
  sh[t] = local;
  __syncthreads();
  const unsigned active = (count + per - 1) / per;
  for (unsigned d = 1; d < active; d <<= 1) {
    const Fr v = sh[t];
    const Fr other = t >= d ? sh[t - d] : Fr::one();
    __syncthreads();
    if (t >= d) sh[t] = other * v;
    __syncthreads();
  }
  Fr acc = t ? sh[t - 1] : Fr::one();
#pragma unroll
  for (unsigned k = 0; k < 4; ++k) {
    if (k < per && lo + k < count) total[lo + k] = acc;
    acc = acc * vals[k];
  }
  if (active == 0 ? t == 0 : t == active - 1) *closes = (active == 0 || sh[t] == Fr::one()) ? 1 : 0;
}
static __global__ void __launch_bounds__(256) k_scale_rows(Fr *__restrict__ z, const Fr *__restrict__ carry, size_t n, unsigned rows, unsigned n_cols) {
  const size_t total = (size_t)n_cols * rows;
  for (size_t g = blockIdx.x * (size_t)blockDim.x + threadIdx.x; g < total; g += (size_t)gridDim.x * blockDim.x) {
    const unsigned col = (unsigned)(g / rows);
    const unsigned i = (unsigned)(g - (size_t)col * rows);
    Fr *p = z + (size_t)col * n + i;
    *p = *p * carry[col];
  }
}

enum { QG_GATE = 0, QG_RLC = 1, QG_PERM_HEAD = 2, QG_PERM_C = 3, QG_PERM_D = 4, QG_LOOKUP = 5, QG_PERM_FIRST = 6, QG_PERM_LAST = 7 };
struct QGroup {
  int type, first, count, pad;
};
struct QArgs {
  const Fr *adv, *fix, *sig, *pz, *lz, *la, *ls, *inst, *lext, *xs;
  const Fr *beta_delta;
  const QGroup *groups;
  Fr *partials;
  Fr y, beta, gamma, gamma_rlc;
  unsigned log_n, u, n_gate, n_rlc, adv_rlc0, fix_qrlc0, fix_const, fix_table, adv_lookup0, n_lookup, n_advice, n_perm, chunk, n_chunks;
  unsigned rows;
  size_t pt0, pt_count;
};

static __global__ void __launch_bounds__(256) k_quotient_partials(QArgs a) {
  const size_t n = (size_t)1 << a.log_n, ne = n * a.rows;
  const size_t p = a.pt0 + blockIdx.x * (size_t)blockDim.x + threadIdx.x;
  if (p >= a.pt0 + a.pt_count || p >= ne) return;
  const QGroup g = a.groups[blockIdx.y];
  const size_t row0 = p & ~(n - 1);
  const size_t k2 = p & (n - 1);
  auto at = [&](const Fr *base, unsigned col, unsigned rot) -> Fr { return base[(size_t)col * ne + row0 + ((k2 + rot) & (n - 1))]; };
  auto ld = [&](const Fr *base, unsigned col, unsigned rot) { return zk::fr9_load(at(base, col, rot)); };
  auto ld32 = [&](const Fr *base, unsigned col, unsigned rot) { return zk::fr9_load32(at(base, col, rot)); };
  const zk::Fr9C y = zk::fr9_load32(a.y);
  zk::Lz<0, 1, 3> acc = zk::lz_widen<0, 1, 3>(zk::lz_zero());
  auto horner = [&](const zk::Fr9C &u, const auto &v) { acc = zk::lz_widen<0, 1, 3>(zk::fr9_mul2(acc, y, u, v)); };
  switch (g.type) {
    case QG_GATE:
      for (int j = g.first; j < g.first + g.count; ++j) {
        const Fr q = at(a.fix, j, 0);
        if (!q.is_zero())
          horner(zk::fr9_load32(q), zk::fr9_norm(zk::lz_sub(zk::lz_add(ld(a.adv, j, 0), zk::fr9_mul(ld(a.adv, j, 1), ld32(a.adv, j, 2))), ld(a.adv, j, 3))));
        else acc = zk::lz_widen<0, 1, 3>(zk::fr9_mul(acc, y));
      }
      break;
    case QG_RLC: {
      const zk::Fr9C gamma_rlc = zk::fr9_load32(a.gamma_rlc);
      for (int j = g.first; j < g.first + g.count; ++j) {
        const unsigned col = a.adv_rlc0 + j;
        horner(ld32(a.fix, a.fix_qrlc0 + j, 0), zk::fr9_norm(zk::lz_sub(zk::lz_add(zk::fr9_mul(ld(a.adv, col, 0), gamma_rlc), ld(a.adv, col, 1)), ld(a.adv, col, 2))));
      }
      break;
    }
    case QG_PERM_HEAD: {
      const Fr zm = at(a.pz, a.n_chunks - 1, 0);
      acc = zk::lz_widen<0, 1, 3>(zk::fr9_mul(zk::fr9_load32(a.lext[p]), zk::lz_sub(zk::fr9_one(), ld(a.pz, 0, 0))));
      horner(zk::fr9_load32(a.lext[ne + p]), zk::lz_sub(zk::fr9_mul(zk::fr9_load(zm), zk::fr9_load32(zm)), zk::fr9_load(zm)));
      break;
    }
    case QG_PERM_FIRST:
      acc = zk::lz_widen<0, 1, 3>(zk::fr9_mul(zk::fr9_load32(a.lext[p]), zk::lz_sub(zk::fr9_one(), ld(a.pz, 0, 0))));
      break;
    case QG_PERM_LAST: {
      const Fr zm = at(a.pz, a.n_chunks - 1, 0);
      acc = zk::lz_widen<0, 1, 3>(zk::fr9_mul(zk::fr9_load32(a.lext[ne + p]), zk::lz_sub(zk::fr9_mul(zk::fr9_load(zm), zk::fr9_load32(zm)), zk::fr9_load(zm))));
      break;
    }
    case QG_PERM_C: {
      const zk::Fr9C l0 = zk::fr9_load32(a.lext[p]);
      for (int j = g.first; j < g.first + g.count; ++j) horner(l0, zk::lz_sub(ld(a.pz, j, 0), ld(a.pz, j - 1, a.u)));
      break;
    }
    case QG_PERM_D: {
      const zk::Fr9C lact = zk::fr9_load32(a.lext[2 * ne + p]), gamma = zk::fr9_load32(a.gamma);
      const zk::Lz<0, 1, 2> beta = zk::fr9_cc(zk::fr9_load32(a.beta)), x = zk::fr9_cc(zk::fr9_load32(a.xs[p]));
      for (int j = g.first; j < g.first + g.count; ++j) {
        zk::Lz<0, 1, 3> left = zk::lz_widen<0, 1, 3>(ld(a.pz, j, 1)), right = zk::lz_widen<0, 1, 3>(ld(a.pz, j, 0));
        for (unsigned c = j * a.chunk; c < (j + 1) * a.chunk && c < a.n_perm; ++c) {
          const zk::Fr9C v = zk::fr9_load32(c < a.n_advice ? at(a.adv, c, 0) : (c == a.n_advice ? at(a.fix, a.fix_const, 0) : a.inst[p]));
          left = zk::fr9_perm_step(left, zk::fr9_perm_factor(v, zk::fr9_mul(ld(a.sig, c, 0), beta), gamma));
          right = zk::fr9_perm_step(right, zk::fr9_perm_factor(v, zk::fr9_mul(zk::fr9_load(a.beta_delta[c]), x), gamma));
        }
        horner(lact, zk::lz_sub(left, right));
      }
      break;
    }
    case QG_LOOKUP: {
      const zk::Fr9C l0 = zk::fr9_load32(a.lext[p]), ll = zk::fr9_load32(a.lext[ne + p]), lact = zk::fr9_load32(a.lext[2 * ne + p]);
      const zk::Fr9C gamma = zk::fr9_load32(a.gamma);
      const zk::Fr9S beta = zk::fr9_load(a.beta), one = zk::fr9_one();
      const zk::Lz<0, 1, 64> s_gamma = zk::fr9_lookup_sum(ld32(a.fix, a.fix_table, 0), gamma);
      for (int i = g.first; i < g.first + g.count; ++i) {
        const Fr z0 = at(a.lz, i, 0), ap = at(a.la, i, 0), sp = at(a.ls, i, 0);
        const auto d = zk::lz_sub(zk::fr9_load(ap), zk::fr9_load(sp));
        horner(l0, zk::lz_sub(one, zk::fr9_load(z0)));
        horner(ll, zk::lz_sub(zk::fr9_mul(zk::fr9_load(z0), zk::fr9_load32(z0)), zk::fr9_load(z0)));
        horner(lact, zk::fr9_mul2(ld32(a.lz, i, 1), zk::fr9_lookup_term(zk::fr9_load(ap), beta, zk::fr9_lookup_sum(zk::fr9_load32(sp), gamma)), zk::fr9_load32(z0),
                                  zk::lz_neg(zk::fr9_lookup_term(ld(a.adv, a.adv_lookup0 + i, 0), beta, s_gamma))));
        horner(l0, d);
        horner(lact, zk::fr9_mul(zk::lz_sub(zk::fr9_load32(ap), ld32(a.la, i, (unsigned)(n - 1))), d));
      }
      break;
    }
  }
  a.partials[(size_t)blockIdx.y * ne + p] = zk::fr9_store(acc);
}

static __global__ void __launch_bounds__(256) k_quotient_combine(const Fr *__restrict__ partials, const Fr *__restrict__ ypow, unsigned n_groups,
                                                          const Fr *__restrict__ zinv, unsigned log_n, unsigned rows, size_t pt0, size_t pt_count, Fr *__restrict__ h_ext) {
  const size_t n = (size_t)1 << log_n, ne = n * rows;
  const size_t p = pt0 + blockIdx.x * (size_t)blockDim.x + threadIdx.x;
  if (p >= pt0 + pt_count || p >= ne) return;
  zk::F29 acc;
#pragma unroll
  for (int l = 0; l < 9; ++l) acc.l[l] = 0;
  unsigned g = 0;
  for (; g + 1 < n_groups; g += 2)
    acc = zk::fr29_weak_reduce(zk::f29_add(acc, zk::fr29_mul2(zk::fr29_unpack(partials[(size_t)g * ne + p]), zk::fr29_unpack(ypow[g]),
                                                             zk::fr29_unpack(partials[(size_t)(g + 1) * ne + p]), zk::fr29_unpack(ypow[g + 1]))));
  if (g < n_groups) acc = zk::fr29_weak_reduce(zk::f29_add(acc, zk::fr29_mul(zk::fr29_unpack(partials[(size_t)g * ne + p]), zk::fr29_unpack(ypow[g]))));
  h_ext[p] = zk::fr29_pack(zk::fr29_canonical(zk::fr29_mul(acc, zk::fr29_unpack(zinv[p >> log_n]))));
}

struct Mat3 {
  Fr v[9];
};
static __global__ void __launch_bounds__(256) k_ext3_combine(const Fr *__restrict__ rows3, const Fr *__restrict__ pw, Mat3 vinv, size_t n, Fr *__restrict__ h_c) {
  const size_t i = blockIdx.x * (size_t)blockDim.x + threadIdx.x;
  if (i >= n) return;
  Fr t[3];
#pragma unroll
  for (int k1 = 0; k1 < 3; ++k1) t[k1] = rows3[(size_t)k1 * n + i] * pw[(size_t)k1 * n + i];
#pragma unroll
  for (int m = 0; m < 3; ++m) h_c[(size_t)m * n + i] = vinv.v[3 * m] * t[0] + vinv.v[3 * m + 1] * t[1] + vinv.v[3 * m + 2] * t[2];
  h_c[3 * n + i] = Fr::zero();
}

static __global__ void __launch_bounds__(256) k_bary_den(const Fr *__restrict__ wpow, const Fr *__restrict__ pts, unsigned n_pts, size_t n,
                                                  Fr *__restrict__ out) {
  const size_t total = (size_t)n_pts * n;
  for (size_t g = blockIdx.x * (size_t)blockDim.x + threadIdx.x; g < total; g += (size_t)gridDim.x * blockDim.x)
    out[g] = pts[g / n] - wpow[g % n];
}
static __global__ void __launch_bounds__(256) k_bary_weights(const Fr *__restrict__ wpow, Fr c, size_t total, size_t n, Fr *__restrict__ inout) {
  for (size_t g = blockIdx.x * (size_t)blockDim.x + threadIdx.x; g < total; g += (size_t)gridDim.x * blockDim.x)
    inout[g] = inout[g] * wpow[g % n] * c;
}
struct EvalJob {
  const Fr *col;
  int n_rot;
  int rot[4];
};
static __global__ void __launch_bounds__(256) k_eval_jobs(const EvalJob *__restrict__ jobs, const Fr *__restrict__ bw ,
                                                          size_t n, Fr *__restrict__ out) {
  __shared__ Fr sh[256];
  const EvalJob job = jobs[blockIdx.x];
  zk::F29 acc[4];
#pragma unroll
  for (int r = 0; r < 4; ++r)
#pragma unroll
    for (int l = 0; l < 9; ++l) acc[r].l[l] = 0;
  const size_t lo = (n / gridDim.y) * blockIdx.y, hi = blockIdx.y + 1 == gridDim.y ? n : lo + n / gridDim.y;
  size_t i = lo + threadIdx.x;
  for (; i + 256 < hi; i += 512) {
    const zk::F29 v0 = zk::fr29_unpack(job.col[i]), v1 = zk::fr29_unpack(job.col[i + 256]);
#pragma unroll
    for (int r = 0; r < 4; ++r)
      if (r < job.n_rot) {
        const Fr *w = bw + (size_t)job.rot[r] * n + i;
        acc[r] = zk::fr29_weak_reduce(zk::f29_add(acc[r], zk::fr29_mul2(v0, zk::fr29_unpack(w[0]), v1, zk::fr29_unpack(w[256]))));
      }
  }
  if (i < hi) {
    const zk::F29 v0 = zk::fr29_unpack(job.col[i]);
#pragma unroll
    for (int r = 0; r < 4; ++r)
      if (r < job.n_rot) acc[r] = zk::fr29_weak_reduce(zk::f29_add(acc[r], zk::fr29_mul(v0, zk::fr29_unpack(bw[(size_t)job.rot[r] * n + i]))));
  }
#pragma unroll
  for (int r = 0; r < 4; ++r) {
    if (r >= job.n_rot) break;
    sh[threadIdx.x] = zk::fr29_pack(zk::fr29_canonical(acc[r]));
    __syncthreads();
    for (int s = 128; s > 0; s >>= 1) {
      if ((int)threadIdx.x < s) sh[threadIdx.x] = sh[threadIdx.x] + sh[threadIdx.x + s];
      __syncthreads();
    }
    if (threadIdx.x == 0) out[((size_t)blockIdx.y * gridDim.x + blockIdx.x) * 4 + r] = sh[0];
    __syncthreads();
  }
}

static __device__ __forceinline__ Fr lincomb29(const Fr *const *__restrict__ ptrs, const Fr *__restrict__ s29, unsigned k0, unsigned k1, size_t i) {
  zk::F29 acc;
#pragma unroll
  for (int l = 0; l < 9; ++l) acc.l[l] = 0;
  unsigned k = k0;
  for (; k + 1 < k1; k += 2)
    acc = zk::fr29_weak_reduce(zk::f29_add(acc, zk::fr29_mul2(zk::fr29_unpack(ptrs[k][i]), zk::fr29_unpack(s29[k]), zk::fr29_unpack(ptrs[k + 1][i]), zk::fr29_unpack(s29[k + 1]))));
  if (k < k1) acc = zk::fr29_weak_reduce(zk::f29_add(acc, zk::fr29_mul(zk::fr29_unpack(ptrs[k][i]), zk::fr29_unpack(s29[k]))));
  return zk::fr29_pack(zk::fr29_canonical(acc));
}
static __global__ void __launch_bounds__(256) k_lincomb_ptrs(const Fr *const *__restrict__ ptrs, const Fr *__restrict__ s29, unsigned m, size_t n,
                                                      Fr *__restrict__ out) {
  for (size_t i = blockIdx.x * (size_t)blockDim.x + threadIdx.x; i < n; i += (size_t)gridDim.x * blockDim.x) out[i] = lincomb29(ptrs, s29, 0, m, i);
}
static __global__ void __launch_bounds__(256) k_lincomb_ptrs_chunked(const Fr *const *__restrict__ ptrs, const Fr *__restrict__ s29, unsigned m, unsigned per, size_t n,
                                                              Fr *__restrict__ partial) {
  const unsigned k0 = blockIdx.y * per, k1 = min(k0 + per, m);
  for (size_t i = blockIdx.x * (size_t)blockDim.x + threadIdx.x; i < n; i += (size_t)gridDim.x * blockDim.x)
    partial[(size_t)blockIdx.y * n + i] = lincomb29(ptrs, s29, k0, k1, i);
}
static __global__ void __launch_bounds__(256) k_sum_rows(const Fr *__restrict__ partial, unsigned rows, size_t n, Fr *__restrict__ out) {
  for (size_t i = blockIdx.x * (size_t)blockDim.x + threadIdx.x; i < n; i += (size_t)gridDim.x * blockDim.x) {
    Fr acc = partial[i];
    for (unsigned r = 1; r < rows; ++r) acc = acc + partial[(size_t)r * n + i];
    out[i] = acc;
  }
}
struct ShSet {
  Fr rc[4];
  Fr pts[4];
  Fr vj;
  Fr coef;
  Fr r_u;
  int n_pts, pad[3];
};
static __global__ void __launch_bounds__(256) k_sh_zs(const ShSet *__restrict__ sets, unsigned n_sets, const Fr *__restrict__ wpow, size_t n,
                                               Fr *__restrict__ zs) {
  const size_t total = (size_t)n_sets * n;
  for (size_t g = blockIdx.x * (size_t)blockDim.x + threadIdx.x; g < total; g += (size_t)gridDim.x * blockDim.x) {
    const ShSet &s = sets[g / n];
    const Fr w = wpow[g % n];
    Fr acc = Fr::one();
    for (int t = 0; t < s.n_pts; ++t) acc = acc * (w - s.pts[t]);
    zs[g] = acc;
  }
}
static __global__ void __launch_bounds__(256) k_sh_h(const ShSet *__restrict__ sets, unsigned n_sets, const Fr *__restrict__ F, const Fr *__restrict__ zs_inv,
                                              const Fr *__restrict__ wpow, size_t n, Fr *__restrict__ hq) {
  for (size_t i = blockIdx.x * (size_t)blockDim.x + threadIdx.x; i < n; i += (size_t)gridDim.x * blockDim.x) {
    const Fr w = wpow[i];
    Fr acc = Fr::zero();
    for (unsigned j = 0; j < n_sets; ++j) {
      const ShSet &s = sets[j];
      Fr r = s.rc[3];
      r = r * w + s.rc[2];
      r = r * w + s.rc[1];
      r = r * w + s.rc[0];
      acc = acc + s.vj * (F[(size_t)j * n + i] - r) * zs_inv[(size_t)j * n + i];
    }
    hq[i] = acc;
  }
}
static __global__ void __launch_bounds__(256) k_sh_den(const Fr *__restrict__ wpow, Fr u, size_t n, Fr *__restrict__ out) {
  size_t i = blockIdx.x * (size_t)blockDim.x + threadIdx.x;
  if (i < n) out[i] = wpow[i] - u;
}
struct ShW {
  Fr coef[8], r_u[8];
};
static __global__ void __launch_bounds__(256) k_sh_w(ShW sets, unsigned n_sets, const Fr *__restrict__ F, const Fr *__restrict__ hq,
                                              Fr ztu, const Fr *__restrict__ inv, size_t n, Fr *__restrict__ W) {
  for (size_t i = blockIdx.x * (size_t)blockDim.x + threadIdx.x; i < n; i += (size_t)gridDim.x * blockDim.x) {
    Fr acc = Fr::zero();
#pragma unroll
    for (unsigned j = 0; j < 8; ++j)
      if (j < n_sets) acc = acc + sets.coef[j] * (F[(size_t)j * n + i] - sets.r_u[j]);
    W[i] = (acc - ztu * hq[i]) * inv[i];
  }
}

}
```

Before: 265.0.

## Run independent prover kernels side by side in shared launches for small circuits

For domains up to 65536 rows, independent small kernels are merged into single launches. The lookup num/den and beta-delta powers share one grid. Permutation and lookup ratios are inverted in one joined batch inversion, and the two chunk-carry checks run as two blocks of one kernel. The SHPLONK per-set linear combinations become one job-list kernel with chunked partials, carrying the zs or barycentric-denominator work as a tail. This cuts launch count and fills the GPU better at k=13, at the cost of larger num/den buffers, more code paths, and an env switch (ZKFHE_CHAIN=serial) to fall back.

```diff
diff --git a/zk-fhe_amd/csrc/core.hip b/zk-fhe_amd/csrc/core.hip
--- a/zk-fhe_amd/csrc/core.hip
+++ b/zk-fhe_amd/csrc/core.hip
@@ -115,6 +115,8 @@
   ctx->uid = next_uid.fetch_add(1);
   ctx->device = device_id;
   ctx->num_cu = prop.multiProcessorCount;
+  const char *chain_env = getenv("ZKFHE_CHAIN");
+  ctx->chain_serial = chain_env && !strcmp(chain_env, "serial");
   if (hip_stream) {
     ctx->stream = (hipStream_t)hip_stream;
   } else {
@@ -428,7 +430,7 @@
   ZK_LAUNCH_CHECK(ctx);
   return ZKFHE_OK;
 }
-static int batch_invert(zkfhe_ctx *ctx, Fr *a, Fr *num, size_t n) {
+static int batch_invert(zkfhe_ctx *ctx, Fr *a, Fr *num, size_t n, bool joined = false) {
   if (!n) return ZKFHE_OK;
   void *tmp;
   int rc = zk_scratch(ctx, 0, n * sizeof(Fr), &tmp);
@@ -436,7 +438,7 @@
   static const int forced = getenv("ZKFHE_BI_CHUNK") ? atoi(getenv("ZKFHE_BI_CHUNK")) : 0;
   size_t chunk = forced > 0 ? (size_t)forced : n / ((size_t)ctx->num_cu * 1024);
   if (forced <= 0) chunk = chunk < BI_CHUNK ? BI_CHUNK : (chunk > 32 ? 32 : chunk);
-  if (forced <= 0 && n >= BI_LONG && chunk < 16) chunk = 16;
+  if (forced <= 0 && n >= BI_LONG && chunk < 16 && !joined) chunk = 16;
   size_t T = (n + chunk - 1) / chunk;
   if (num)
     k_fr_batch_invert<true><<<zk_blocks(T, 256), 256, 0, ctx->stream>>>(a, num, (Fr *)tmp, n, T);
@@ -454,6 +456,13 @@
   ZK_ARG(ctx, n == 0 || (den != nullptr && num != nullptr && (const void *)den != (const void *)num));
   return batch_invert(ctx, (Fr *)den, (Fr *)num, n);
 }
+}
+int zk_fr_batch_invert_mul_joined(zkfhe_ctx *ctx, const zk::Fr *den, zk::Fr *num, size_t n) {
+  ZK_ENTER(ctx);
+  ZK_ARG(ctx, n == 0 || (den != nullptr && num != nullptr && (const void *)den != (const void *)num));
+  return batch_invert(ctx, (Fr *)den, num, n, true);
+}
+extern "C" {
 int zkfhe_fr9_op(zkfhe_ctx *ctx, int op, const zkfhe_fr *in, zkfhe_fr *out, size_t n) {
   ZK_ENTER(ctx);
   ZK_ARG(ctx, op >= 0 && op < FR9_OPS);
diff --git a/zk-fhe_amd/csrc/ctx.hpp b/zk-fhe_amd/csrc/ctx.hpp
--- a/zk-fhe_amd/csrc/ctx.hpp
+++ b/zk-fhe_amd/csrc/ctx.hpp
@@ -45,6 +45,7 @@
   float proof_marks[3] = {0, 0, 0};
   uint64_t cmd_count[3] = {0, 0, 0};
   zkfhe_ctx *cmd_owner = nullptr;
+  bool chain_serial = false;
   unsigned *tickets = nullptr;
   uint32_t *bfv_tw = nullptr;
   void *bfv_work = nullptr;
@@ -138,6 +139,7 @@
 int zk_func_max_lds(zkfhe_ctx *ctx, const void *kernel, int bytes);
 int zk_scratch(zkfhe_ctx *ctx, int slot, size_t bytes, void **out);
 int zk_basis_create_scaled(zkfhe_ctx *ctx, const zkfhe_g1_affine *bases_host, size_t n, int window_bits, double table_budget_scale, zkfhe_basis **out);
+int zk_fr_batch_invert_mul_joined(zkfhe_ctx *ctx, const zk::Fr *den, zk::Fr *num, size_t n);
 int zk_copy_d2d(zkfhe_ctx *ctx, void *dst, const void *src, size_t bytes);
 int zk_domain(zkfhe_ctx *ctx, int log_n, const NttDomain **out);
 int zk_pre13(zkfhe_ctx *ctx, const zk::Fr &g, int lef, int rows, bool scaled, const void **out);
diff --git a/zk-fhe_amd/host/chain_jobs.hpp b/zk-fhe_amd/host/chain_jobs.hpp
--- /dev/null
+++ b/zk-fhe_amd/host/chain_jobs.hpp
@@ -0,0 +1,43 @@
+#pragma once
+#include <cstddef>
+#include <cstdint>
+#include <vector>
+
+namespace chain {
+
+constexpr unsigned PER = 48;
+
+struct Job {
+  uint32_t first;
+  uint32_t m;
+  uint32_t set;
+  int32_t slot;
+};
+struct Sum {
+  uint32_t set, slot0, chunks;
+  uint32_t pad;
+};
+struct Plan {
+  std::vector<Job> jobs;
+  std::vector<Sum> sums;
+  std::vector<uint32_t> first;
+  uint32_t members = 0;
+  uint32_t slots = 0;
+};
+
+inline Plan plan(const std::vector<size_t> &sizes) {
+  Plan p;
+  for (size_t j = 0; j < sizes.size(); ++j) {
+    const uint32_t m = (uint32_t)sizes[j], chunks = m ? (m + PER - 1) / PER : 1;
+    p.first.push_back(p.members);
+    if (chunks > 1) p.sums.push_back(Sum{(uint32_t)j, p.slots, chunks, 0});
+    for (uint32_t c = 0; c < chunks; ++c) {
+      const uint32_t lo = c * PER, hi = lo + PER < m ? lo + PER : m;
+      p.jobs.push_back(Job{p.members + lo, hi - lo, (uint32_t)j, chunks > 1 ? (int32_t)p.slots++ : -1});
+    }
+    p.members += m;
+  }
+  return p;
+}
+
+}
diff --git a/zk-fhe_amd/host/keygen.hip b/zk-fhe_amd/host/keygen.hip
--- a/zk-fhe_amd/host/keygen.hip
+++ b/zk-fhe_amd/host/keygen.hip
@@ -71,8 +71,8 @@
   CK(ws->h_c.alloc(ctx, 4 * col));
   CK(ws->misc.alloc(ctx, 32 * col));
   CK(ws->points.alloc(ctx, std::max<size_t>(n_all, c.n_perm()) * 64 + 64));
-  CK(ws->num.alloc(ctx, std::max<size_t>(c.n_chunks(), c.n_lookup) * col));
-  CK(ws->den.alloc(ctx, std::max<size_t>(c.n_chunks(), c.n_lookup) * col));
+  CK(ws->num.alloc(ctx, ((size_t)c.n_chunks() + c.n_lookup) * col));
+  CK(ws->den.alloc(ctx, ((size_t)c.n_chunks() + c.n_lookup) * col));
   if ((size_t)c.n_perm() > 4096 || (size_t)c.n_chunks() + c.n_lookup > 4096)
     return zk_fail_msg(ctx, ZKFHE_EINVAL, "configuration too wide for the prover workspace (more than 4096 permutation columns)");
   CK(ws->small.alloc(ctx, 1 << 20));
diff --git a/zk-fhe_amd/host/prove.hip b/zk-fhe_amd/host/prove.hip
--- a/zk-fhe_amd/host/prove.hip
+++ b/zk-fhe_amd/host/prove.hip
@@ -822,9 +822,10 @@
     U256 dcan;
     memcpy(dcan.l, DELTA_CANON, 32);
     beta_delta_dev = (Fr *)ws->small.p;
+    const size_t nch = cfg.n_chunks(), nb_z = nbl - 1;
+    if (n <= 65536 && !ctx->chain_serial) return grand_products_side_by_side(mont(dcan));
     zkp::k_powers<<<1, 256, 0, ctx->stream>>>(beta, mont(dcan), beta_delta_dev, cfg.n_perm());
     ZK_LAUNCH_CHECK(ctx);
-    const size_t nch = cfg.n_chunks(), nb_z = nbl - 1;
     zkp::k_perm_num_den<<<grid_for(ctx, nch * n), 256, 0, ctx->stream>>>(perm_args(), ws->num.fr(), ws->den.fr());
     ZK_LAUNCH_CHECK(ctx);
     CK(zkfhe_fr_batch_invert_mul(ctx, (const zkfhe_fr *)ws->den.p, (zkfhe_fr *)ws->num.p, nch * n));
@@ -847,6 +848,32 @@
       zkp::k_chunk_carry<<<1, 1024, 0, ctx->stream>>>(totals_dev, (unsigned)nl, 1, closes + 1);
       ZK_LAUNCH_CHECK(ctx);
     }
+    return commit_products();
+  }
+  int grand_products_side_by_side(const Fr &delta) {
+    const size_t nch = cfg.n_chunks(), nl = cfg.n_lookup, nb_z = nbl - 1;
+    if ((nch + nl) * n * 32 > ws->num.bytes || (nch + nl) * n * 32 > ws->den.bytes) return zk_fail_msg(ctx, ZKFHE_EINVAL, "grand products: ratio buffers too small");
+    Fr *const num_lk = ws->num.fr() + nch * n, *const den_lk = ws->den.fr() + nch * n;
+    zkp::k_lookup_num_den_powers<<<(nl ? grid_for(ctx, nl * n) : 0u) + 1u, 256, 0, ctx->stream>>>(
+        ws->adv_l.fr() + (size_t)cfg.adv_lookup0() * n, pk->fixed_l.fr() + (size_t)cfg.fix_table() * n, ws->la_l.fr(), ws->ls_l.fr(), beta, gamma, (unsigned)nl, n, num_lk, den_lk,
+        beta, delta, beta_delta_dev, cfg.n_perm());
+    ZK_LAUNCH_CHECK(ctx);
+    zkp::k_perm_num_den<<<grid_for(ctx, nch * n), 256, 0, ctx->stream>>>(perm_args(), ws->num.fr(), ws->den.fr());
+    ZK_LAUNCH_CHECK(ctx);
+    CK(zk_fr_batch_invert_mul_joined(ctx, ws->den.fr(), ws->num.fr(), (nch + nl) * n));
+    Fr *totals_dev = (Fr *)ws->small.p + 4096;
+    CK(prefix_products(ws->num.fr(), ws->pz_l.fr(), nch + nl, blind_rows(ctr_pz, nb_z), totals_dev));
+    int *const closes = ws->out_flags();
+    closes[0] = closes[1] = 1;
+    zkp::k_chunk_carry_both<<<nl ? 2 : 1, 1024, 0, ctx->stream>>>(totals_dev, (unsigned)nch, (unsigned)nl, closes);
+    ZK_LAUNCH_CHECK(ctx);
+    zkp::k_scale_rows<<<grid_for(ctx, nch * (u + 1)), 256, 0, ctx->stream>>>(ws->pz_l.fr(), totals_dev, n, (unsigned)(u + 1), (unsigned)nch);
+    ZK_LAUNCH_CHECK(ctx);
+    return commit_products();
+  }
+  int commit_products() {
+    const size_t nch = cfg.n_chunks();
+    int *const closes = ws->out_flags();
     std::vector<AffinePoint> pz_commit;
     CK(commit_cols_out(ctx, srs, srs->g_lagrange, ws->pz_l.fr(), nch + cfg.n_lookup, ws, pz_commit));
     if (!closes[0]) return zk_fail_msg(ctx, ZKFHE_EINVAL, "permutation argument does not close: a copy constraint is violated");
@@ -1085,13 +1112,25 @@
     STAGE(sc_dev, Fr, ws, sc, sizeof(sc));
     STAGE(pts_dev, Fr, ws, pts_rot, sizeof(pts_rot));
     STAGE(jobs_dev, zkp::EvalJob, ws, jobs.data(), jobs.size() * sizeof(zkp::EvalJob));
-    CK(flush_staged(ctx, ws));
-    CK(lincomb(ptrs_dev, sc_dev, 3, H_c));
+    Fr *bw = ws->misc.fr();
+    const bool side_by_side = n <= 65536 && !ctx->chain_serial;
+    if (side_by_side) {
+      const chain::Job hjob{0, 3, 0, -1};
+      STAGE(hjob_dev, chain::Job, ws, &hjob, sizeof(hjob));
+      CK(flush_staged(ctx, ws));
+      const unsigned gx = grid_for(ctx, n), tail_rows = (grid_for(ctx, 6 * n) + gx - 1) / gx;
+      zkp::k_chain_jobs<zkp::TAIL_BARY><<<dim3(gx, 1 + tail_rows), 256, 0, ctx->stream>>>(hjob_dev, 1, ptrs_dev, sc_dev, n, H_c, nullptr, pts_dev, 6, dom->fwd, bw);
+      ZK_LAUNCH_CHECK(ctx);
+    } else {
+      CK(flush_staged(ctx, ws));
+      CK(lincomb(ptrs_dev, sc_dev, 3, H_c));
+    }
     CK(zkfhe_ntt_batch_to(ctx, (const zkfhe_fr *)H_c, (zkfhe_fr *)H_l, 1, (int)k, 0));
     if (!early_rand) CK(zkfhe_ntt_batch_to(ctx, (const zkfhe_fr *)rand_c, (zkfhe_fr *)rand_l, 1, (int)k, 0));
-    Fr *bw = ws->misc.fr();
-    zkp::k_bary_den<<<grid_for(ctx, 6 * n), 256, 0, ctx->stream>>>(dom->fwd, pts_dev, 6, n, bw);
-    ZK_LAUNCH_CHECK(ctx);
+    if (!side_by_side) {
+      zkp::k_bary_den<<<grid_for(ctx, 6 * n), 256, 0, ctx->stream>>>(dom->fwd, pts_dev, 6, n, bw);
+      ZK_LAUNCH_CHECK(ctx);
+    }
     CK(zkfhe_fr_batch_invert(ctx, (zkfhe_fr *)bw, 6 * n));
     const Fr c = zk::zk_fr_to_29((xn - Fr::one()) * dom->n_inv);
     zkp::k_bary_weights<<<grid_for(ctx, 6 * n), 256, 0, ctx->stream>>>(dom->fwd, c, 6 * n, n, bw);
@@ -1146,6 +1185,14 @@
     std::vector<zkp::ShSet> shsets(ns);
     std::vector<const Fr *const *> set_ptrs(ns);
     std::vector<const Fr *> set_pw(ns);
+    const bool side_by_side = n <= 65536 && !ctx->chain_serial && !(W_sh > 1 && k >= 14);
+    std::vector<size_t> set_sizes(ns);
+    for (size_t j = 0; j < ns; ++j) set_sizes[j] = sets[j].members.size();
+    const chain::Plan plan = chain::plan(set_sizes);
+    std::vector<const Fr *> all_ptrs;
+    std::vector<Fr> all_pw;
+    all_ptrs.reserve(plan.members);
+    all_pw.reserve(plan.members);
     for (size_t j = 0; j < ns; ++j) {
       const auto &mem = sets[j].members;
       std::vector<const Fr *> ptrs(mem.size());
@@ -1160,10 +1207,15 @@
         for (size_t t = 0; t < np; ++t) comb[t] = comb[t] + cur * mont(items[mem[m]].ev[layout.eval_slot(mem[m], sets[j].rots[t])]);
         cur = cur * yq;
       }
-      STAGE(pd, const Fr *, ws, ptrs.data(), mem.size() * sizeof(void *));
-      STAGE(sd, Fr, ws, pw.data(), mem.size() * 32);
-      set_ptrs[j] = pd;
-      set_pw[j] = sd;
+      if (side_by_side) {
+        all_ptrs.insert(all_ptrs.end(), ptrs.begin(), ptrs.end());
+        all_pw.insert(all_pw.end(), pw.begin(), pw.end());
+      } else {
+        STAGE(pd, const Fr *, ws, ptrs.data(), mem.size() * sizeof(void *));
+        STAGE(sd, Fr, ws, pw.data(), mem.size() * 32);
+        set_ptrs[j] = pd;
+        set_pw[j] = sd;
+      }
       zkp::ShSet &S = shsets[j];
       S.n_pts = (int)np;
       for (size_t t = 0; t < 4; ++t) S.pts[t] = t < np ? pts_rot[sets[j].rots[t]] : Fr::zero();
@@ -1178,22 +1230,46 @@
       vj = vj * v;
     }
     STAGE(sets_dev, zkp::ShSet, ws, shsets.data(), ns * sizeof(zkp::ShSet));
-    CK(flush_staged(ctx, ws));
-    const bool shard_sets = W_sh > 1 && k >= 14;
-    if (shard_sets) CK(grow_qgather((size_t)W_sh * ns * n * 32));
-    for (size_t j = 0; j < ns; ++j) {
-      const size_t all = sets[j].members.size();
-      const size_t m_lo = shard_sets ? all * r_sh / W_sh : 0, m_hi = shard_sets ? all * (r_sh + 1) / W_sh : all;
-      CK(lincomb(set_ptrs[j] + m_lo, set_pw[j] + m_lo, (unsigned)(m_hi - m_lo), F + j * n));
-      if (shard_sets) CK(zkfhe_comm_all_gather_async(ctx, srs->comm, F + j * n, ws->qgather.fr() + j * (size_t)W_sh * n, n * 32));
-    }
-    if (shard_sets) CK(sum_shares(ns, F));
     Fr *zs = ws->misc.fr() + 20 * n;
     Fr *hq = ws->misc.fr() + 28 * n;
     Fr *Wq = ws->misc.fr() + 29 * n;
     Fr *dinv = ws->misc.fr() + 30 * n;
-    zkp::k_sh_zs<<<grid_for(ctx, ns * n), 256, 0, ctx->stream>>>(sets_dev, (unsigned)ns, dom->fwd, n, zs);
-    ZK_LAUNCH_CHECK(ctx);
+    if (side_by_side) {
+      if ((size_t)plan.slots * n * 32 > ws->partials.bytes) return zk_fail_msg(ctx, ZKFHE_EINVAL, "SHPLONK: partial sums do not fit the quotient buffer");
+      STAGE(ptrs_dev, const Fr *, ws, all_ptrs.data(), all_ptrs.size() * sizeof(void *));
+      STAGE(pw_dev, Fr, ws, all_pw.data(), all_pw.size() * 32);
+      STAGE(jobs_dev, chain::Job, ws, plan.jobs.data(), plan.jobs.size() * sizeof(chain::Job));
+      const chain::Sum no_sum{};
+      STAGE(sums_dev, chain::Sum, ws, plan.sums.empty() ? &no_sum : plan.sums.data(), plan.sums.size() * sizeof(chain::Sum));
+      CK(flush_staged(ctx, ws));
+      const unsigned gx = grid_for(ctx, n), nj = (unsigned)plan.jobs.size(), tail_rows = (grid_for(ctx, ns * n) + gx - 1) / gx;
+      if ((size_t)gx * (nj + tail_rows) <= (size_t)7 * ctx->num_cu) {
+        zkp::k_chain_jobs<zkp::TAIL_ZS><<<dim3(gx, nj + tail_rows), 256, 0, ctx->stream>>>(jobs_dev, nj, ptrs_dev, pw_dev, n, F, ws->partials.fr(), sets_dev, (unsigned)ns, dom->fwd, zs);
+        ZK_LAUNCH_CHECK(ctx);
+      } else {
+        zkp::k_chain_jobs<zkp::TAIL_NONE><<<dim3(gx, nj), 256, 0, ctx->stream>>>(jobs_dev, nj, ptrs_dev, pw_dev, n, F, ws->partials.fr(), nullptr, 0, nullptr, nullptr);
+        ZK_LAUNCH_CHECK(ctx);
+        zkp::k_sh_zs<<<grid_for(ctx, ns * n), 256, 0, ctx->stream>>>(sets_dev, (unsigned)ns, dom->fwd, n, zs);
+        ZK_LAUNCH_CHECK(ctx);
+      }
+      if (!plan.sums.empty()) {
+        zkp::k_chain_sums<<<dim3(gx, (unsigned)plan.sums.size()), 256, 0, ctx->stream>>>(sums_dev, ws->partials.fr(), n, F);
+        ZK_LAUNCH_CHECK(ctx);
+      }
+    } else {
+      CK(flush_staged(ctx, ws));
+      const bool shard_sets = W_sh > 1 && k >= 14;
+      if (shard_sets) CK(grow_qgather((size_t)W_sh * ns * n * 32));
+      for (size_t j = 0; j < ns; ++j) {
+        const size_t all = sets[j].members.size();
+        const size_t m_lo = shard_sets ? all * r_sh / W_sh : 0, m_hi = shard_sets ? all * (r_sh + 1) / W_sh : all;
+        CK(lincomb(set_ptrs[j] + m_lo, set_pw[j] + m_lo, (unsigned)(m_hi - m_lo), F + j * n));
+        if (shard_sets) CK(zkfhe_comm_all_gather_async(ctx, srs->comm, F + j * n, ws->qgather.fr() + j * (size_t)W_sh * n, n * 32));
+      }
+      if (shard_sets) CK(sum_shares(ns, F));
+      zkp::k_sh_zs<<<grid_for(ctx, ns * n), 256, 0, ctx->stream>>>(sets_dev, (unsigned)ns, dom->fwd, n, zs);
+      ZK_LAUNCH_CHECK(ctx);
+    }
     CK(zkfhe_fr_batch_invert(ctx, (zkfhe_fr *)zs, ns * n));
     zkp::k_sh_h<<<grid_for(ctx, n), 256, 0, ctx->stream>>>(sets_dev, (unsigned)ns, F, zs, dom->fwd, n, hq);
     ZK_LAUNCH_CHECK(ctx);
diff --git a/zk-fhe_amd/host/prover_kernels.hip.hpp b/zk-fhe_amd/host/prover_kernels.hip.hpp
--- a/zk-fhe_amd/host/prover_kernels.hip.hpp
+++ b/zk-fhe_amd/host/prover_kernels.hip.hpp
@@ -1,13 +1,14 @@
 #pragma once
 #include "../csrc/ctx.hpp"
 #include "../csrc/fr9.hip.hpp"
+#include "chain_jobs.hpp"
 
 namespace zkp {
 
 using zk::Fr;
 
-static __global__ void __launch_bounds__(256) k_powers(Fr start, Fr base, Fr *__restrict__ out, size_t n) {
-  for (size_t i = blockIdx.x * (size_t)blockDim.x + threadIdx.x; i < n; i += (size_t)gridDim.x * blockDim.x) {
+__device__ __forceinline__ void powers_body(Fr start, Fr base, Fr *__restrict__ out, size_t n, unsigned blk, unsigned nblk) {
+  for (size_t i = blk * (size_t)blockDim.x + threadIdx.x; i < n; i += (size_t)nblk * blockDim.x) {
     Fr r = start, b = base;
     for (size_t e = i; e; e >>= 1) {
       if (e & 1) r = r * b;
@@ -16,6 +17,7 @@
     out[i] = r;
   }
 }
+static __global__ void __launch_bounds__(256) k_powers(Fr start, Fr base, Fr *__restrict__ out, size_t n) { powers_body(start, base, out, n, blockIdx.x, gridDim.x); }
 
 __device__ __forceinline__ unsigned long long rotr64(unsigned long long x, int n) { return (x >> n) | (x << (64 - n)); }
 __device__ __forceinline__ Fr rng_draw(const unsigned long long seed[4], unsigned long long ctr) {
@@ -180,17 +182,28 @@
     den[g] = de;
   }
 }
+__device__ __forceinline__ void lookup_num_den_body(const Fr *__restrict__ a_cols, const Fr *__restrict__ table, const Fr *__restrict__ la, const Fr *__restrict__ ls,
+                                                    const Fr &beta, const Fr &gamma, unsigned n_lookup, size_t n, Fr *__restrict__ num, Fr *__restrict__ den, unsigned blk,
+                                                    unsigned nblk) {
+  const size_t total = (size_t)n_lookup * n;
+  const zk::Fr9S beta9 = zk::fr9_load(beta);
+  const zk::Fr9C gamma9 = zk::fr9_load32(gamma);
+  for (size_t g = blk * (size_t)blockDim.x + threadIdx.x; g < total; g += (size_t)nblk * blockDim.x) {
+    const size_t i = g % n;
+    num[g] = zk::fr9_store(zk::fr9_lookup_term(zk::fr9_load(a_cols[g]), beta9, zk::fr9_lookup_sum(zk::fr9_load32(table[i]), gamma9)));
+    den[g] = zk::fr9_store(zk::fr9_lookup_term(zk::fr9_load(la[g]), beta9, zk::fr9_lookup_sum(zk::fr9_load32(ls[g]), gamma9)));
+  }
+}
 static __global__ void __launch_bounds__(256) k_lookup_num_den(const Fr *__restrict__ a_cols, const Fr *__restrict__ table, const Fr *__restrict__ la,
                                                         const Fr *__restrict__ ls, Fr beta, Fr gamma, unsigned n_lookup, size_t n,
                                                         Fr *__restrict__ num, Fr *__restrict__ den) {
-  const size_t total = (size_t)n_lookup * n;
-  const zk::Fr9S beta9 = zk::fr9_load(beta);
-  const zk::Fr9C gamma9 = zk::fr9_load32(gamma);
-  for (size_t g = blockIdx.x * (size_t)blockDim.x + threadIdx.x; g < total; g += (size_t)gridDim.x * blockDim.x) {
-    const size_t i = g % n;
-    num[g] = zk::fr9_store(zk::fr9_lookup_term(zk::fr9_load(a_cols[g]), beta9, zk::fr9_lookup_sum(zk::fr9_load32(table[i]), gamma9)));
-    den[g] = zk::fr9_store(zk::fr9_lookup_term(zk::fr9_load(la[g]), beta9, zk::fr9_lookup_sum(zk::fr9_load32(ls[g]), gamma9)));
-  }
+  lookup_num_den_body(a_cols, table, la, ls, beta, gamma, n_lookup, n, num, den, blockIdx.x, gridDim.x);
+}
+static __global__ void __launch_bounds__(256) k_lookup_num_den_powers(const Fr *__restrict__ a_cols, const Fr *__restrict__ table, const Fr *__restrict__ la,
+                                                               const Fr *__restrict__ ls, Fr beta, Fr gamma, unsigned n_lookup, size_t n, Fr *__restrict__ num,
+                                                               Fr *__restrict__ den, Fr pstart, Fr pbase, Fr *__restrict__ pout, size_t pn) {
+  if (blockIdx.x + 1 == gridDim.x) powers_body(pstart, pbase, pout, pn, 0, 1);
+  else lookup_num_den_body(a_cols, table, la, ls, beta, gamma, n_lookup, n, num, den, blockIdx.x, gridDim.x - 1);
 }
 
 static __global__ void __launch_bounds__(1024) k_prefix_product(const Fr *__restrict__ ratio, Fr *__restrict__ z, Fr *__restrict__ total, size_t n,
@@ -287,7 +300,7 @@
     if (i < u) acc = acc * r[i];
   }
 }
-static __global__ void __launch_bounds__(1024) k_chunk_carry(Fr *__restrict__ total, unsigned count, int check_ones, int *__restrict__ closes) {
+__device__ __forceinline__ void chunk_carry_body(Fr *__restrict__ total, unsigned count, int check_ones, int *__restrict__ closes) {
   __shared__ Fr sh[1024];
   __shared__ int bad;
   const unsigned t = threadIdx.x;
@@ -326,6 +339,13 @@
     acc = acc * vals[k];
   }
   if (active == 0 ? t == 0 : t == active - 1) *closes = (active == 0 || sh[t] == Fr::one()) ? 1 : 0;
+}
+static __global__ void __launch_bounds__(1024) k_chunk_carry(Fr *__restrict__ total, unsigned count, int check_ones, int *__restrict__ closes) {
+  chunk_carry_body(total, count, check_ones, closes);
+}
+static __global__ void __launch_bounds__(1024) k_chunk_carry_both(Fr *__restrict__ total, unsigned n_carry, unsigned n_ones, int *__restrict__ closes) {
+  if (blockIdx.x == 0) chunk_carry_body(total, n_carry, 0, closes);
+  else chunk_carry_body(total + n_carry, n_ones, 1, closes + 1);
 }
 static __global__ void __launch_bounds__(256) k_scale_rows(Fr *__restrict__ z, const Fr *__restrict__ carry, size_t n, unsigned rows, unsigned n_cols) {
   const size_t total = (size_t)n_cols * rows;
@@ -466,11 +486,15 @@
   h_c[3 * n + i] = Fr::zero();
 }
 
+__device__ __forceinline__ void bary_den_body(const Fr *__restrict__ wpow, const Fr *__restrict__ pts, unsigned n_pts, size_t n, Fr *__restrict__ out, unsigned blk,
+                                              unsigned nblk) {
+  const size_t total = (size_t)n_pts * n;
+  for (size_t g = blk * (size_t)blockDim.x + threadIdx.x; g < total; g += (size_t)nblk * blockDim.x)
+    out[g] = pts[g / n] - wpow[g % n];
+}
 static __global__ void __launch_bounds__(256) k_bary_den(const Fr *__restrict__ wpow, const Fr *__restrict__ pts, unsigned n_pts, size_t n,
                                                   Fr *__restrict__ out) {
-  const size_t total = (size_t)n_pts * n;
-  for (size_t g = blockIdx.x * (size_t)blockDim.x + threadIdx.x; g < total; g += (size_t)gridDim.x * blockDim.x)
-    out[g] = pts[g / n] - wpow[g % n];
+  bary_den_body(wpow, pts, n_pts, n, out, blockIdx.x, gridDim.x);
 }
 static __global__ void __launch_bounds__(256) k_bary_weights(const Fr *__restrict__ wpow, Fr c, size_t total, size_t n, Fr *__restrict__ inout) {
   for (size_t g = blockIdx.x * (size_t)blockDim.x + threadIdx.x; g < total; g += (size_t)gridDim.x * blockDim.x)
@@ -531,22 +555,28 @@
   if (k < k1) acc = zk::fr29_weak_reduce(zk::f29_add(acc, zk::fr29_mul(zk::fr29_unpack(ptrs[k][i]), zk::fr29_unpack(s29[k]))));
   return zk::fr29_pack(zk::fr29_canonical(acc));
 }
+__device__ __forceinline__ void lincomb_body(const Fr *const *__restrict__ ptrs, const Fr *__restrict__ s29, unsigned k0, unsigned k1, size_t n, Fr *__restrict__ out,
+                                             unsigned blk, unsigned nblk) {
+  for (size_t i = blk * (size_t)blockDim.x + threadIdx.x; i < n; i += (size_t)nblk * blockDim.x) out[i] = lincomb29(ptrs, s29, k0, k1, i);
+}
 static __global__ void __launch_bounds__(256) k_lincomb_ptrs(const Fr *const *__restrict__ ptrs, const Fr *__restrict__ s29, unsigned m, size_t n,
                                                       Fr *__restrict__ out) {
-  for (size_t i = blockIdx.x * (size_t)blockDim.x + threadIdx.x; i < n; i += (size_t)gridDim.x * blockDim.x) out[i] = lincomb29(ptrs, s29, 0, m, i);
+  lincomb_body(ptrs, s29, 0, m, n, out, blockIdx.x, gridDim.x);
 }
 static __global__ void __launch_bounds__(256) k_lincomb_ptrs_chunked(const Fr *const *__restrict__ ptrs, const Fr *__restrict__ s29, unsigned m, unsigned per, size_t n,
                                                               Fr *__restrict__ partial) {
   const unsigned k0 = blockIdx.y * per, k1 = min(k0 + per, m);
-  for (size_t i = blockIdx.x * (size_t)blockDim.x + threadIdx.x; i < n; i += (size_t)gridDim.x * blockDim.x)
-    partial[(size_t)blockIdx.y * n + i] = lincomb29(ptrs, s29, k0, k1, i);
-}
-static __global__ void __launch_bounds__(256) k_sum_rows(const Fr *__restrict__ partial, unsigned rows, size_t n, Fr *__restrict__ out) {
-  for (size_t i = blockIdx.x * (size_t)blockDim.x + threadIdx.x; i < n; i += (size_t)gridDim.x * blockDim.x) {
+  lincomb_body(ptrs, s29, k0, k1, n, partial + (size_t)blockIdx.y * n, blockIdx.x, gridDim.x);
+}
+__device__ __forceinline__ void sum_rows_body(const Fr *__restrict__ partial, unsigned rows, size_t n, Fr *__restrict__ out, unsigned blk, unsigned nblk) {
+  for (size_t i = blk * (size_t)blockDim.x + threadIdx.x; i < n; i += (size_t)nblk * blockDim.x) {
     Fr acc = partial[i];
     for (unsigned r = 1; r < rows; ++r) acc = acc + partial[(size_t)r * n + i];
     out[i] = acc;
   }
+}
+static __global__ void __launch_bounds__(256) k_sum_rows(const Fr *__restrict__ partial, unsigned rows, size_t n, Fr *__restrict__ out) {
+  sum_rows_body(partial, rows, n, out, blockIdx.x, gridDim.x);
 }
 struct ShSet {
   Fr rc[4];
@@ -556,16 +586,38 @@
   Fr r_u;
   int n_pts, pad[3];
 };
-static __global__ void __launch_bounds__(256) k_sh_zs(const ShSet *__restrict__ sets, unsigned n_sets, const Fr *__restrict__ wpow, size_t n,
-                                               Fr *__restrict__ zs) {
+__device__ __forceinline__ void sh_zs_body(const ShSet *__restrict__ sets, unsigned n_sets, const Fr *__restrict__ wpow, size_t n, Fr *__restrict__ zs, unsigned blk,
+                                           unsigned nblk) {
   const size_t total = (size_t)n_sets * n;
-  for (size_t g = blockIdx.x * (size_t)blockDim.x + threadIdx.x; g < total; g += (size_t)gridDim.x * blockDim.x) {
+  for (size_t g = blk * (size_t)blockDim.x + threadIdx.x; g < total; g += (size_t)nblk * blockDim.x) {
     const ShSet &s = sets[g / n];
     const Fr w = wpow[g % n];
     Fr acc = Fr::one();
     for (int t = 0; t < s.n_pts; ++t) acc = acc * (w - s.pts[t]);
     zs[g] = acc;
   }
+}
+static __global__ void __launch_bounds__(256) k_sh_zs(const ShSet *__restrict__ sets, unsigned n_sets, const Fr *__restrict__ wpow, size_t n,
+                                               Fr *__restrict__ zs) {
+  sh_zs_body(sets, n_sets, wpow, n, zs, blockIdx.x, gridDim.x);
+}
+enum { TAIL_ZS = 0, TAIL_BARY = 1, TAIL_NONE = 2 };
+template <int TAIL>
+static __global__ void __launch_bounds__(256) k_chain_jobs(const chain::Job *__restrict__ jobs, unsigned n_jobs, const Fr *const *__restrict__ ptrs, const Fr *__restrict__ s29,
+                                                    size_t n, Fr *__restrict__ direct, Fr *__restrict__ partial, const void *__restrict__ tab, unsigned count,
+                                                    const Fr *__restrict__ wpow, Fr *__restrict__ tail_out) {
+  if (blockIdx.y < n_jobs) {
+    const chain::Job j = jobs[blockIdx.y];
+    lincomb_body(ptrs, s29, j.first, j.first + j.m, n, j.slot < 0 ? direct + (size_t)j.set * n : partial + (size_t)j.slot * n, blockIdx.x, gridDim.x);
+    return;
+  }
+  const unsigned blk = (blockIdx.y - n_jobs) * gridDim.x + blockIdx.x, nblk = (gridDim.y - n_jobs) * gridDim.x;
+  if (TAIL == TAIL_ZS) sh_zs_body((const ShSet *)tab, count, wpow, n, tail_out, blk, nblk);
+  else if (TAIL == TAIL_BARY) bary_den_body(wpow, (const Fr *)tab, count, n, tail_out, blk, nblk);
+}
+static __global__ void __launch_bounds__(256) k_chain_sums(const chain::Sum *__restrict__ sums, const Fr *__restrict__ partial, size_t n, Fr *__restrict__ direct) {
+  const chain::Sum s = sums[blockIdx.y];
+  sum_rows_body(partial + (size_t)s.slot0 * n, s.chunks, n, direct + (size_t)s.set * n, blockIdx.x, gridDim.x);
 }
 static __global__ void __launch_bounds__(256) k_sh_h(const ShSet *__restrict__ sets, unsigned n_sets, const Fr *__restrict__ F, const Fr *__restrict__ zs_inv,
                                               const Fr *__restrict__ wpow, size_t n, Fr *__restrict__ hq) {
```

Result: faster. 273.3, median of 6 (+3.1%).
